# castorini/howl

Measured on AMD Instinct MI355X. Metric: utterances/sec/node (res8 end-to-end training step, 1s@16kHz, 40-mel), higher is better.
Workload: dtype f32; 1 GPU; res8 training step (frontend+fwd+xent+bwd+AdamW), 512 x 1 s utterances per GPU, 12 labels -- BASELINE configs[2] per-GPU share: res8 GSC-12, 512 x 1 s per GPU (4096 over 8); global_batch=512, samples_per_utterance=16000, labels=12, parallelism=single, frontend=eval

## Files before the change

### howl_amd/csrc/howl_common.hip.h

```cpp
#pragma once
#include <hip/hip_runtime.h>
#include <math.h>
#include <stdint.h>
#include <stdio.h>

typedef float f32x4 __attribute__((ext_vector_type(4)));
typedef __attribute__((address_space(3))) float lds_f32;

#if defined(HIPEMU)
#define HOWL_OPAQUE_V(x) ((void)(x))
#else
#define HOWL_OPAQUE_V(x) asm volatile("" : "+v"(x))
#endif
#define HOWL_OPAQUE_LDS(p) HOWL_OPAQUE_V(p)

#define HOWL_OK 0
#define HOWL_E_ARG (-1)
#define HOWL_E_LAUNCH (-2)
#define HOWL_E_WORKSPACE (-3)

void howl_set_error(const char* fmt, ...);
int howl_num_cus();
bool howl_prof_begin(const char* tag, hipStream_t stream, size_t* slot, double work);
void howl_prof_end(size_t slot, hipStream_t stream);

struct HowlSideLane {
    hipStream_t stream;
    hipEvent_t fork_ev, join_ev;
};
HowlSideLane* howl_side_lane();
bool howl_raise_lds(const void* kernel, size_t lds, size_t* granted, const char* what);
bool howl_take_pending_error();
inline void howl_lane_fork(HowlSideLane* l, hipStream_t main) {
    hipEventRecord(l->fork_ev, main);
    hipStreamWaitEvent(l->stream, l->fork_ev, 0);
}
inline void howl_lane_join(HowlSideLane* l, hipStream_t main) {
    hipEventRecord(l->join_ev, l->stream);
    hipStreamWaitEvent(main, l->join_ev, 0);
}

struct HowlProfScope {
    size_t slot = 0;
    bool on;
    hipStream_t stream;
    HowlProfScope(const char* tag, hipStream_t s, double work = 0.0) : stream(s) { on = howl_prof_begin(tag, s, &slot, work); }
    ~HowlProfScope() {
        if (on) howl_prof_end(slot, stream);
    }
};

struct HowlAdamWCoef {
    float lr, b1, b2, eps, wd, bc1, bc2_sqrt, gscale;
};
inline HowlAdamWCoef howl_adamw_coef(float lr, float beta1, float beta2, float eps, float weight_decay, int step, float grad_scale) {
    const double bc1 = 1.0 - pow((double)beta1, (double)step);
    const double bc2 = 1.0 - pow((double)beta2, (double)step);
    return HowlAdamWCoef{lr, beta1, beta2, eps, weight_decay, (float)bc1, (float)sqrt(bc2), grad_scale};
}
__device__ __forceinline__ void howl_adamw_element(float* __restrict__ p, float* __restrict__ m, float* __restrict__ v, size_t i, float g,
                                                   const HowlAdamWCoef& c) {
#pragma clang fp contract(off)
    const float gi = g * c.gscale;
    float pi = p[i] * (1.0f - c.lr * c.wd);
    const float mi = m[i] + (gi - m[i]) * (1.0f - c.b1);
    const float vi = c.b2 * v[i] + (1.0f - c.b2) * gi * gi;
    const float denom = sqrtf(vi) / c.bc2_sqrt + c.eps;
    pi -= (c.lr / c.bc1) * (mi / denom);
    p[i] = pi;
    m[i] = mi;
    v[i] = vi;
}

#define HOWL_REQUIRE(cond, ...)                 \
    do {                                        \
        if (!(cond)) {                          \
            howl_set_error(__VA_ARGS__);        \
            return HOWL_E_ARG;                  \
        }                                       \
    } while (0)

#define HOWL_CHECK_LAUNCH(name)                                                     \
    do {                                                                            \
        hipError_t e_ = hipGetLastError();                                          \
        if (howl_take_pending_error()) return HOWL_E_LAUNCH;   \
        if (e_ != hipSuccess) {                                                     \
            howl_set_error("%s: launch failed: %s", name, hipGetErrorString(e_));   \
            return HOWL_E_LAUNCH;                                                   \
        }                                                                           \
    } while (0)

__device__ __forceinline__ void wave_lds_sync() {
    __builtin_amdgcn_fence(__ATOMIC_RELEASE, "wavefront");
    __builtin_amdgcn_wave_barrier();
    __builtin_amdgcn_fence(__ATOMIC_ACQUIRE, "wavefront");
}

__device__ __forceinline__ float wave_sum(float v) {
    for (int m = 32; m >= 1; m >>= 1) v += __shfl_xor(v, m);
    return v;
}
__device__ __forceinline__ float wave_sum_rows(float v) {
    v += __int_as_float(__builtin_amdgcn_update_dpp(0, __float_as_int(v), 0xB1, 0xf, 0xf, true));
    v += __int_as_float(__builtin_amdgcn_update_dpp(0, __float_as_int(v), 0x4E, 0xf, 0xf, true));
    v += __int_as_float(__builtin_amdgcn_update_dpp(0, __float_as_int(v), 0x141, 0xf, 0xf, true));
    v += __int_as_float(__builtin_amdgcn_update_dpp(0, __float_as_int(v), 0x140, 0xf, 0xf, true));
    v += __shfl_xor(v, 16);
    v += __shfl_xor(v, 32);
    return v;
}
__device__ __forceinline__ double wave_sum_d(double v) {
    for (int m = 32; m >= 1; m >>= 1) v += __shfl_xor(v, m);
    return v;
}
```

### howl_amd/csrc/res8.hip

```cpp
#include "howl_common.hip.h"
#include "../../include/howl_hip.h"

namespace {

struct HowlPtrs6 {
    float* p[6];
};
constexpr int MAX_WINDOWS = 64;
struct HowlWinRows {
    int lo[MAX_WINDOWS], hi[MAX_WINDOWS];
};
struct HowlBnBuffers {
    float* running_mean;
    float* running_var;
    long long* num_batches;
};
struct BnFold {
    const float* part;
    int nparts;
    double count;
    float* stats_out;
    HowlBnBuffers bn;
};

// ... 18 lines not shown
__host__ __device__ inline int tile_floats(int H, bool own_rows = false) { return CP * chan_stride(H, own_rows) + 32; }
constexpr int WPW = 13;
constexpr int WNCOL = 16 * 26;
constexpr int WTAPS = 9 * NMAP;
__host__ __device__ inline int wgrad_rounds(int H) { return (H + 3) / 4; }

constexpr int PACK_ELEMS = 3 * KSTEPS * 64;
__device__ __forceinline__ void pack_weights_one(const HowlPtrs6& w, float* __restrict__ wp_fwd, float* __restrict__ wp_bwd,
                                                 int layer, int mode, int idx) {
    const int lane = idx & 63;
    const int ks = (idx >> 6) % KSTEPS;
    const int nt = idx / (64 * KSTEPS);
    int kk, tap;
    if (ks < 9 * KFULL) {
        const int c0 = ks / 9;
        tap = ks - 9 * c0;
        kk = 4 * c0 + (lane >> 4);
    } else {
        tap = 4 * (ks - 9 * KFULL) + (lane >> 4);
        kk = 4 * KFULL;
    }
    const int n = 16 * nt + (lane & 15);
    float v = 0.0f;
    if (kk < NMAP && n < NMAP && tap < 9) {
        const float* wl = w.p[layer];
        v = (mode == 0) ? wl[(n * NMAP + kk) * 9 + tap] : wl[(kk * NMAP + n) * 9 + (8 - tap)];
    }
    float* dst = (mode == 0 ? wp_fwd : wp_bwd) + (size_t)layer * (3 * KSTEPS * 64);
    dst[idx] = v;
}

__device__ __forceinline__ void zero_lds(float* p, int n, int tid, int nthreads) {
    const int n4 = n >> 2;
    for (int i = tid; i < n4; i += nthreads) reinterpret_cast<float4*>(p)[i] = make_float4(0.0f, 0.0f, 0.0f, 0.0f);
    for (int i = 4 * n4 + tid; i < n; i += nthreads) p[i] = 0.0f;
}

__host__ __device__ inline int part_stride(int nparts) { return (nparts + 3) & ~3; }
__device__ __forceinline__ double fold_part_column(const float* __restrict__ part, int nps, int nparts, int column, int lane) {
    const int slice = lane & 7;
    const float* src = part + (size_t)column * nps;
    double acc = 0.0;
    for (int r0 = 4 * slice; r0 < nparts; r0 += 8 * 32) {
        float4 v[8];
#pragma unroll
        for (int j = 0; j < 8; ++j) {
            const int r = r0 + 32 * j;
            v[j] = *reinterpret_cast<const float4*>(src + (r < nps ? r : 0));
        }
#pragma unroll
        for (int j = 0; j < 8; ++j) {
            const int r = r0 + 32 * j;
            acc += (r + 0 < nparts) ? (double)v[j].x : 0.0;
            acc += (r + 1 < nparts) ? (double)v[j].y : 0.0;
            acc += (r + 2 < nparts) ? (double)v[j].z : 0.0;
            acc += (r + 3 < nparts) ? (double)v[j].w : 0.0;
        }
    }
    acc += __shfl_xor(acc, 1);
    acc += __shfl_xor(acc, 2);
    acc += __shfl_xor(acc, 4);
    return acc;
}

template <int NTW>
struct KCursor {
    const lds_f32* ap[NTW];
    const lds_f32* bp;
    float a[NTW], b;
};

template <int NTW>
__device__ __forceinline__ void k_prime(KCursor<NTW>& k) {
#pragma unroll
    for (int i = 0; i < NTW; ++i) k.a[i] = k.ap[i][0];
    k.b = k.bp[0];
}

template <int NTW, int TS>
__device__ __forceinline__ void k_begin(KCursor<NTW>& k, f32x4 (&acc)[NTW], const lds_f32* tile, const lds_f32* wl,
                                        int CS, int P, int t0, int lane) {
    constexpr int ts = TS;
#pragma unroll
    for (int i = 0; i < NTW; ++i) {
        int m = 16 * (t0 + ts * i) + (lane & 15);
        m = m < P ? m : P - 1;
        const int h = m / PW;
        k.ap[i] = tile + (lane >> 4) * CS + h * WP + (m - h * PW);
        HOWL_OPAQUE_LDS(k.ap[i]);
        acc[i] = {0.0f, 0.0f, 0.0f, 0.0f};
    }
    k.bp = wl + lane;
    HOWL_OPAQUE_LDS(k.bp);
}

template <int NTW>
__device__ __forceinline__ void k_run(KCursor<NTW>& k, f32x4 (&acc)[NTW], int CS, int groups) {
#pragma unroll 2
    for (int g = 0; g < groups; ++g) {
#pragma unroll
        for (int tap = 0; tap < 9; ++tap) {
            float na[NTW], nb;
            if (tap < 8) {
                const int off = ((tap + 1) / 3) * WP + ((tap + 1) % 3);
#pragma unroll
                for (int i = 0; i < NTW; ++i) na[i] = k.ap[i][off];
                nb = k.bp[(tap + 1) * 64];
            } else {
                k.bp += 9 * 64;
#pragma unroll
                for (int i = 0; i < NTW; ++i) k.ap[i] += 4 * CS;
#pragma unroll
                for (int i = 0; i < NTW; ++i) na[i] = k.ap[i][0];
                nb = k.bp[0];
            }
#pragma unroll
            for (int i = 0; i < NTW; ++i) acc[i] = __builtin_amdgcn_mfma_f32_16x16x4f32(k.a[i], k.b, acc[i], 0, 0, 0);
#pragma unroll
            for (int i = 0; i < NTW; ++i) k.a[i] = na[i];
            k.b = nb;
        }
    }
}

template <int NTW>
__device__ __forceinline__ void k_tail(KCursor<NTW>& k, f32x4 (&acc)[NTW], const int (&dl)[3]) {
#pragma unroll
    for (int s3 = 0; s3 < 3; ++s3) {
        const float b = k.bp[s3 * 64];
#pragma unroll
        for (int i = 0; i < NTW; ++i) acc[i] = __builtin_amdgcn_mfma_f32_16x16x4f32(k.ap[i][dl[s3]], b, acc[i], 0, 0, 0);
    }
}

constexpr int SPLIT_C = 24;
constexpr int KG_A = SPLIT_C / 4;
constexpr int KG_B = KFULL - KG_A;
constexpr int NS0 = 5, NS1 = 4;
static_assert(CONV_THREADS * NS0 >= SPLIT_C * MAX_H * PW / 2 && CONV_THREADS * NS1 >= (NMAP - SPLIT_C) * MAX_H * PW / 2, "slots");
static_assert(KG_A == 6 && KG_B == 5, "the segment schedule of conv_loop is written for 6 + 5 K groups");

#define HOWL_STAIR(p_) __builtin_amdgcn_s_setprio(p_)

struct StageCfg {
    const float* a;
    const float* s;
    const float* k;
    float* ds;
    const float* dpool;
    float invP;
    bool fused;
    bool even;
    bool affine;
};

struct SlotVal {
    float2 a, s, k;
};

template <int NSL>
__device__ __forceinline__ void region_slots(int (&pk)[NSL], int c0, int nch, int P, int CS, int tid) {
    const float invP = 1.0f / (float)P;
#pragma unroll
    for (int j = 0; j < NSL; ++j) {
        const int e = 2 * (tid + j * CONV_THREADS);
        const int c = (int)(((float)e + 0.5f) * invP);
        const int p = e - c * P;
        const int h = (int)(((float)p + 0.5f) * 0.1f);
        const int w = p - h * PW;
        pk[j] = (e < nch * P) ? (((c0 + c) * CS + (h + 1) * WP + (w + 1)) | ((c0 + c) << 20)) : -1;
    }
}
template <int NSL>
__device__ __forceinline__ void region_slots_pad(int (&pk)[NSL], int c0, int nch, int P, int CS, int tid, int hv, unsigned& padbits) {
    region_slots<NSL>(pk, c0, nch, P, CS, tid);
#pragma unroll
    for (int j = 0; j < NSL; ++j) {
        const int e = 2 * (tid + j * CONV_THREADS);
        const int p = e % P;
        if (pk[j] >= 0 && p / PW >= hv) padbits |= 1u << j;
    }
}

template <int MODE, int HALO = 0>
__device__ __forceinline__ void slot_load(SlotVal& v, const StageCfg& cfg, size_t base, int i2, int pkj, int b) {
    HOWL_OPAQUE_V(pkj);
    const unsigned off = pkj >= 0 ? 8u * (unsigned)i2 : 0u;
    if (MODE == 1 && cfg.fused) {
        if (cfg.a != nullptr) {
            v.a = *reinterpret_cast<const float2*>(reinterpret_cast<const char*>(cfg.a + base) + off);
        } else {
            const unsigned c4 = pkj >= 0 ? 4u * (unsigned)(pkj >> 20) : 0u;
            const float g = *reinterpret_cast<const float*>(reinterpret_cast<const char*>(cfg.dpool + (size_t)(HALO == 1 ? b >> 1 : b) * CP) + c4) * cfg.invP;
            v.a = make_float2(g, g);
        }
        v.s = *reinterpret_cast<const float2*>(reinterpret_cast<const char*>(cfg.s + base) + off);
        v.k = cfg.k != nullptr ? *reinterpret_cast<const float2*>(reinterpret_cast<const char*>(cfg.k + base) + off)
                               : make_float2(0.0f, 0.0f);
    } else {
        v.a = *reinterpret_cast<const float2*>(reinterpret_cast<const char*>(cfg.a + base) + off);
    }
}

__device__ __forceinline__ void bn_relu_bwd_pair(const SlotVal& v, const float* lmc, bool even, float2& ds, float2& dz) {
    const float A = lmc[0], Bc = lmc[CP], Cc = lmc[2 * CP];
    ds.x = fmaf(A, v.a.x, fmaf(Bc, fabsf(v.s.x), Cc)) + v.k.x;
    ds.y = fmaf(A, v.a.y, fmaf(Bc, fabsf(v.s.y), Cc)) + v.k.y;
    const float t0 = even ? -v.s.x : v.s.x, t1 = even ? -v.s.y : v.s.y;
    dz.x = t0 > 0.0f ? ds.x : 0.0f;
    dz.y = t1 > 0.0f ? ds.y : 0.0f;
}

template <int MODE>
__device__ __forceinline__ void slot_write(const SlotVal& v, const StageCfg& cfg, size_t base, int i2, int pkj, float* tile,
                                           const float* lm, bool zero = false ) {
    HOWL_OPAQUE_V(pkj);
    if (pkj < 0) return;
    const int c = pkj >> 20;
    float v0 = v.a.x, v1 = v.a.y;
    if (MODE == 0) {
        v0 = fabsf(v0);
        v1 = fabsf(v1);
        if (cfg.affine) {
            const float sh = lm[c], r = lm[CP + c];
            v0 = fmaf(v0, r, sh);
            v1 = fmaf(v1, r, sh);
        }
    } else if (cfg.fused) {
        float2 ds, dz;
        bn_relu_bwd_pair(v, lm + c, cfg.even, ds, dz);
        if (cfg.ds != nullptr)
            *reinterpret_cast<float2*>(reinterpret_cast<char*>(cfg.ds + base) + 8u * (unsigned)i2) = ds;
        v0 = dz.x;
        v1 = dz.y;
    }
    if (zero) v0 = v1 = 0.0f;
    float* d = tile + (pkj & 0xFFFFF);
    d[0] = v0;
    d[1] = v1;
}

struct HaloSlot {
    int pk;
    int g;
};
__device__ __forceinline__ HaloSlot halo_slot(int c0, int nch, int H, int P, int CS, int tid) {
    const int c = tid / H, h = tid - c * H;
    HaloSlot hs;
    hs.pk = (tid < nch * H) ? (((c0 + c) * CS + (h + 1) * WP) | ((c0 + c) << 20)) : -1;
    hs.g = (tid < nch * H) ? (c0 + c) * P + h * PW : 0;
    return hs;
}
template <int MODE>
__device__ __forceinline__ void halo_load(SlotVal& v, const StageCfg& cfg, size_t nbase, const HaloSlot& hs, int gcol, int b) {
    const unsigned off = hs.pk >= 0 ? 4u * (unsigned)(hs.g + gcol) : 0u;
    v.s = v.k = make_float2(0.0f, 0.0f);
    if (MODE == 1 && cfg.fused) {
        if (cfg.a != nullptr) {
            v.a.x = *reinterpret_cast<const float*>(reinterpret_cast<const char*>(cfg.a + nbase) + off);
        } else {
            const unsigned c4 = hs.pk >= 0 ? 4u * (unsigned)(hs.pk >> 20) : 0u;
            v.a.x = *reinterpret_cast<const float*>(reinterpret_cast<const char*>(cfg.dpool + (size_t)(b >> 1) * CP) + c4) * cfg.invP;
        }
        v.s.x = *reinterpret_cast<const float*>(reinterpret_cast<const char*>(cfg.s + nbase) + off);
        if (cfg.k != nullptr) v.k.x = *reinterpret_cast<const float*>(reinterpret_cast<const char*>(cfg.k + nbase) + off);
    } else {
        v.a.x = *reinterpret_cast<const float*>(reinterpret_cast<const char*>(cfg.a + nbase) + off);
    }
    v.a.y = v.a.x;
}
template <int MODE>
__device__ __forceinline__ void halo_write(const SlotVal& v, const StageCfg& cfg, const HaloSlot& hs, int lcol, float* tile,
                                           const float* lm) {
    if (hs.pk < 0) return;
    const int c = hs.pk >> 20;
    float v0 = v.a.x;
    if (MODE == 0) {
        v0 = fabsf(v0);
        if (cfg.affine) v0 = fmaf(v0, lm[CP + c], lm[c]);
    } else if (cfg.fused) {
        float2 ds, dz;
        bn_relu_bwd_pair(v, lm + c, cfg.even, ds, dz);
        v0 = dz.x;
    }
    tile[(hs.pk & 0xFFFFF) + lcol] = v0;
}

struct StripGeom {
    int nr, ns, hv_last;
};
struct StripPos {
    int r, c, hv, bu;
};
__device__ __forceinline__ StripPos strip_pos(const StripGeom& g, int v, int H) {
    StripPos p;
    const int q = v / g.ns;
    p.c = v - q * g.ns;
    p.bu = q / g.nr;
    p.r = q - p.bu * g.nr;
    p.hv = (p.r == g.nr - 1) ? g.hv_last : H;
    return p;
}
struct EdgeSlot {
    int pk;
    int g;
    int aux;
};
// ... 16 lines not shown
    if (MODE == 1 && cfg.fused) {
        v.a.x = cfg.a != nullptr ? cfg.a[idx] : cfg.dpool[(size_t)bu * CP + chan] * cfg.invP;
        v.s.x = cfg.s[idx];
        if (cfg.k != nullptr) v.k.x = cfg.k[idx];
    } else {
        v.a.x = cfg.a[idx];
    }
    v.a.y = v.a.x;
}
template <int MODE>
__device__ __forceinline__ void edge_write(const SlotVal& v, const StageCfg& cfg, int pk, int lds_extra, bool valid, float* tile,
                                           const float* lm) {
    if (pk < 0) return;
    const int c = pk >> 20;
    float v0 = v.a.x;
    if (MODE == 0) {
        v0 = fabsf(v0);
        if (cfg.affine) v0 = fmaf(v0, lm[CP + c], lm[c]);
    } else if (cfg.fused) {
        float2 ds, dz;
        bn_relu_bwd_pair(v, lm + c, cfg.even, ds, dz);
        v0 = dz.x;
    }
    tile[(pk & 0xFFFFF) + lds_extra] = valid ? v0 : 0.0f;
}
struct GridCtx {
    StripGeom sg;
    EdgeSlot col[2], row[2];
    unsigned pad[2];
};
template <int MODE>
__device__ __forceinline__ void grid_load(SlotVal (&e)[3], const StageCfg& cfg, const GridCtx& gx, int reg, int v, int H, int P) {
    const StripPos p = strip_pos(gx.sg, v, H);
    {
        const EdgeSlot& es = gx.col[reg];
        const bool valid = gx.sg.ns == 2 && es.pk >= 0 && es.aux < p.hv;
        edge_load<MODE>(e[0], cfg, v ^ 1, es.g + (p.c ? PW - 1 : 0), valid, es.pk >= 0 ? es.pk >> 20 : 0, p.bu, P);
    }
    const EdgeSlot& rs = gx.row[reg];
    const int cc = p.c + rs.aux;
    const bool colok = rs.pk >= 0 && cc >= 0 && cc < gx.sg.ns;
    const int chan = rs.pk >= 0 ? rs.pk >> 20 : 0;
    edge_load<MODE>(e[1], cfg, v - gx.sg.ns + rs.aux, rs.g + (H - 1) * PW, colok && p.r > 0, chan, p.bu, P);
    edge_load<MODE>(e[2], cfg, v + gx.sg.ns + rs.aux, rs.g, colok && p.r < gx.sg.nr - 1, chan, p.bu, P);
}
template <int MODE>
__device__ __forceinline__ void grid_write(const SlotVal (&e)[3], const StageCfg& cfg, const GridCtx& gx, int reg, int v, int H,
                                           float* tile, const float* lm) {
    const StripPos p = strip_pos(gx.sg, v, H);
    if (gx.sg.ns == 2) {
        const EdgeSlot& es = gx.col[reg];
        edge_write<MODE>(e[0], cfg, es.pk, p.c ? 0 : WP - 1, es.aux < p.hv, tile, lm);
    }
    const EdgeSlot& rs = gx.row[reg];
    const int cc = p.c + rs.aux;
    const bool colok = cc >= 0 && cc < gx.sg.ns;
    edge_write<MODE>(e[1], cfg, rs.pk, 0, colok && p.r > 0, tile, lm);
    edge_write<MODE>(e[2], cfg, rs.pk, (H + 1) * WP, colok && p.r < gx.sg.nr - 1, tile, lm);
}

struct ConvEpilogue {
    const float* res;
    float* out;
    const float* xs;
    float xshift, xrstd;
    int cout, P;
    bool cvalid;
    bool xadd;
    float* pool;
    int npg, pg;
};

template <int NTW, int TS>
struct EpiAddr {
    unsigned boff, bmax;
    static constexpr unsigned tstep = 64u * TS;
    __device__ __forceinline__ EpiAddr(const ConvEpilogue& e, int t0, int lane) {
        const unsigned crow = (unsigned)((e.cvalid ? e.cout : NMAP - 1) * e.P);
        boff = 4u * (crow + 16u * t0 + 4u * (lane >> 4));
        bmax = 4u * (crow + e.P - 2);
    }
    __device__ __forceinline__ unsigned off(int i, int hh) const {
        unsigned o = boff + tstep * i + 8u * hh;
        if (i == NTW - 1) o = o < bmax ? o : bmax;
        return o;
    }
};

template <int MODE, int NTW, int TS, int HALO = 0>
__device__ __forceinline__ void conv_epilogue(const f32x4 (&acc)[NTW], const float2 (&ev)[NTW > 0 ? NTW : 1][2], const ConvEpilogue& e,
                                              size_t ubase, int t0, int lane, float& st0, float& st1, int b,
                                              int pv = 0 ) {
    const EpiAddr<NTW, TS> ea(e, t0, lane);
    constexpr int ts = TS;
    char* obase = reinterpret_cast<char*>(e.out + ubase);
    float u0 = 0.0f, u1 = 0.0f;
#pragma unroll
    for (int i = 0; i < NTW; ++i) {
        const int mbase = 16 * (t0 + ts * i) + 4 * (lane >> 4);
#pragma unroll
        for (int hh = 0; hh < 2; ++hh) {
            const int m = mbase + 2 * hh;
            if (e.cvalid && (i < NTW - 1 || m < e.P)) {
                float v0 = acc[i][2 * hh], v1 = acc[i][2 * hh + 1];
                if (MODE == 0) {
                    v0 = fmaxf(v0, 0.0f);
                    v1 = fmaxf(v1, 0.0f);
                    if (e.res != nullptr) {
                        const float2 r = ev[i][hh];
                        const bool k0 = v0 > 0.0f, k1 = v1 > 0.0f;
                        v0 += fabsf(r.x);
                        v1 += fabsf(r.y);
                        if (HALO != 2 || m < pv) {
                            u0 += v0 + v1;
                            u1 += v0 * v0 + v1 * v1;
                        }
                        v0 = k0 ? -v0 : v0;
                        v1 = k1 ? -v1 : v1;
                    } else if (HALO != 2 || m < pv) {
                        u0 += v0 + v1;
                        u1 += v0 * v0 + v1 * v1;
                    }
                } else if (e.xs != nullptr) {
                    const float2 sv = ev[i][hh];
                    if (e.xadd) {
                        v0 += sv.x;
                        v1 += sv.y;
                    } else if (HALO != 2 || m < pv) {
                        u0 += v0 + v1;
                        u1 += v0 * fmaf(fabsf(sv.x), e.xrstd, e.xshift) + v1 * fmaf(fabsf(sv.y), e.xrstd, e.xshift);
                    }
                }
                *reinterpret_cast<float2*>(obase + (ea.boff + ea.tstep * i + 8u * hh)) = make_float2(v0, v1);
            }
        }
    }
    st0 += u0;
    st1 += u1;
    if (MODE == 0 && e.pool != nullptr) {
        float up = u0;
        up += __shfl_xor(up, 16);
        up += __shfl_xor(up, 32);
        if (lane < 16 && e.cvalid) e.pool[((size_t)b * e.npg + e.pg) * CP + e.cout] = up;
    }
}

struct ConvLoop {
    const lds_f32* ltile;
    const lds_f32* wnt;
    float* tile;
    const float* lm;
    int B, CS, t0, lane, tid;
    int nblk;
};


template <int MODE, int NTW, int TS, int HALO = 0>
__device__ __forceinline__ void conv_loop(const ConvLoop& c, const ConvEpilogue& epi, const StageCfg& cfg, const int (&pk0)[NS0],
                                          const int (&pk1)[NS1], int b, float& st0, float& st1,
                                          const HaloSlot (&hs)[2] = {HaloSlot{-1, 0}, HaloSlot{-1, 0}},
                                          const GridCtx& gx = GridCtx{}) {
    const int P = epi.P, tid = c.tid, lane = c.lane;
    const int wave = tid >> 6;
    const size_t r1 = (size_t)SPLIT_C * P;
    const float* eop = (MODE == 0) ? epi.res : epi.xs;
    constexpr int NTV = NTW > 0 ? NTW : 1;
    int dl[3];
#pragma unroll
    for (int s3 = 0; s3 < 3; ++s3) {
        const int tap = min(4 * s3 + (lane >> 4), 8);
        dl[s3] = (tap / 3) * WP + tap % 3 - (lane >> 4) * c.CS;
    }
    const int gcol = (b & 1) ? PW - 1 : 0, lcol = (b & 1) ? 0 : WP - 1;
    for (; b < c.B; b += c.nblk) {
        const size_t ubase = (size_t)b * NMAP * P;
        const int bn = b + c.nblk;
        const bool more = bn < c.B;
        const size_t nbase = (size_t)bn * NMAP * P;
        SlotVal v[3];
        SlotVal ge[3];
        int bsl = b, bnsl = bn, pv = P;
        bool zb = false, zn = false;
        if constexpr (HALO == 2) {
            const StripPos pb = strip_pos(gx.sg, b, P / PW), pn = strip_pos(gx.sg, more ? bn : b, P / PW);
            bsl = pb.bu, bnsl = pn.bu, pv = pb.hv * PW;
            zb = pb.hv < P / PW, zn = pn.hv < P / PW;
        }
        f32x4 acc[NTV];
        KCursor<NTV> k;
        if constexpr (NTW > 0) k_begin<NTW, TS>(k, acc, c.ltile, c.wnt, c.CS, P, c.t0, lane);
        if constexpr (NTW > 0) k_prime<NTW>(k);
        constexpr bool STAGE = true;
        const int a0 = 2, a1 = 2, a2 = KG_A - 4, b0 = 2, b1 = 2, b2 = KG_B - 4;
#define HOWL_WINO_CHUNK() ((void)0)
#define HOWL_WINO_BAR() ((void)0)
        if constexpr (STAGE) {
            slot_load<MODE, HALO>(v[0], cfg, ubase + r1, tid, pk1[0], bsl);
            slot_load<MODE, HALO>(v[1], cfg, ubase + r1, tid + CONV_THREADS, pk1[1], bsl);
            if constexpr (HALO == 1) halo_load<MODE>(v[2], cfg, (size_t)(b ^ 1) * NMAP * P, hs[1], gcol, b);
            if constexpr (HALO == 2) grid_load<MODE>(ge, cfg, gx, 1, b, P / PW, P);
        }
        HOWL_STAIR(3);
        HOWL_WINO_CHUNK();
        if constexpr (NTW > 0) k_run<NTW>(k, acc, c.CS, a0);
        HOWL_WINO_BAR();
        if constexpr (STAGE) {
            slot_write<MODE>(v[0], cfg, ubase + r1, tid, pk1[0], c.tile, c.lm, HALO == 2 && zb && ((gx.pad[1] >> 0) & 1));
            slot_write<MODE>(v[1], cfg, ubase + r1, tid + CONV_THREADS, pk1[1], c.tile, c.lm, HALO == 2 && zb && ((gx.pad[1] >> 1) & 1));
            if constexpr (HALO == 1) halo_write<MODE>(v[2], cfg, hs[1], lcol, c.tile, c.lm);
            if constexpr (HALO == 2) grid_write<MODE>(ge, cfg, gx, 1, b, P / PW, c.tile, c.lm);
            slot_load<MODE, HALO>(v[0], cfg, ubase + r1, tid + 2 * CONV_THREADS, pk1[2], bsl);
            slot_load<MODE, HALO>(v[1], cfg, ubase + r1, tid + 3 * CONV_THREADS, pk1[3], bsl);
        }
        HOWL_STAIR(2);
        HOWL_WINO_CHUNK();
        if constexpr (NTW > 0) k_run<NTW>(k, acc, c.CS, a1);
        HOWL_WINO_BAR();
        if constexpr (STAGE) {
            slot_write<MODE>(v[0], cfg, ubase + r1, tid + 2 * CONV_THREADS, pk1[2], c.tile, c.lm, HALO == 2 && zb && ((gx.pad[1] >> 2) & 1));
            slot_write<MODE>(v[1], cfg, ubase + r1, tid + 3 * CONV_THREADS, pk1[3], c.tile, c.lm, HALO == 2 && zb && ((gx.pad[1] >> 3) & 1));
        }
        HOWL_STAIR(1);
        HOWL_WINO_CHUNK();
        if constexpr (NTW > 0) k_run<NTW>(k, acc, c.CS, a2);
        HOWL_WINO_BAR();
        HOWL_STAIR(0);
        __syncthreads();
        if constexpr (NTW > 0) k_prime<NTW>(k);
        if (STAGE && more) {
            slot_load<MODE, HALO>(v[0], cfg, nbase, tid, pk0[0], bnsl);
            slot_load<MODE, HALO>(v[1], cfg, nbase, tid + CONV_THREADS, pk0[1], bnsl);
            slot_load<MODE, HALO>(v[2], cfg, nbase, tid + 2 * CONV_THREADS, pk0[2], bnsl);
            if constexpr (HALO == 2) grid_load<MODE>(ge, cfg, gx, 0, bn, P / PW, P);
        }
        HOWL_STAIR(3);
        HOWL_WINO_CHUNK();
        if constexpr (NTW > 0) k_run<NTW>(k, acc, c.CS, b0);
        HOWL_WINO_BAR();
        if (STAGE && more) {
            slot_write<MODE>(v[0], cfg, nbase, tid, pk0[0], c.tile, c.lm, HALO == 2 && zn && ((gx.pad[0] >> 0) & 1));
            slot_write<MODE>(v[1], cfg, nbase, tid + CONV_THREADS, pk0[1], c.tile, c.lm, HALO == 2 && zn && ((gx.pad[0] >> 1) & 1));
            slot_write<MODE>(v[2], cfg, nbase, tid + 2 * CONV_THREADS, pk0[2], c.tile, c.lm, HALO == 2 && zn && ((gx.pad[0] >> 2) & 1));
            if constexpr (HALO == 2) grid_write<MODE>(ge, cfg, gx, 0, bn, P / PW, c.tile, c.lm);
            slot_load<MODE, HALO>(v[0], cfg, nbase, tid + 3 * CONV_THREADS, pk0[3], bnsl);
            slot_load<MODE, HALO>(v[1], cfg, nbase, tid + 4 * CONV_THREADS, pk0[4], bnsl);
            if constexpr (HALO == 1) halo_load<MODE>(v[2], cfg, (size_t)(bn ^ 1) * NMAP * P, hs[0], gcol, bn);
        }
        HOWL_STAIR(2);
        HOWL_WINO_CHUNK();
        if constexpr (NTW > 0) k_run<NTW>(k, acc, c.CS, b1);
        HOWL_WINO_BAR();
        if (STAGE && more) {
            slot_write<MODE>(v[0], cfg, nbase, tid + 3 * CONV_THREADS, pk0[3], c.tile, c.lm, HALO == 2 && zn && ((gx.pad[0] >> 3) & 1));
            slot_write<MODE>(v[1], cfg, nbase, tid + 4 * CONV_THREADS, pk0[4], c.tile, c.lm, HALO == 2 && zn && ((gx.pad[0] >> 4) & 1));
            if constexpr (HALO == 1) halo_write<MODE>(v[2], cfg, hs[0], lcol, c.tile, c.lm);
        }
        float2 ev[NTV][2];
        if constexpr (NTW > 0) {
            if (eop != nullptr) {
                const EpiAddr<NTW, TS> ea(epi, c.t0, lane);
                const char* ebase = reinterpret_cast<const char*>(eop + ubase);
#pragma unroll
                for (int i = 0; i < NTW; ++i)
#pragma unroll
                    for (int hh = 0; hh < 2; ++hh) ev[i][hh] = *reinterpret_cast<const float2*>(ebase + ea.off(i, hh));
            }
            HOWL_STAIR(1);
            k_run<NTW>(k, acc, c.CS, b2);
            k_tail<NTW>(k, acc, dl);
            HOWL_STAIR(0);
        }
        if constexpr (NTW > 0) conv_epilogue<MODE, NTW, TS, HALO>(acc, ev, epi, ubase, c.t0, lane, st0, st1, b, pv);
        __syncthreads();
    }
}

struct BwdFold {
    const float* stats;
    const float* m12;
    const float* part;
    int nparts;
    double count;
};
__device__ __forceinline__ void bwd_consts_to_lds(float* lm, int ch, float mean, float rstd, float m1, float m2) {
    lm[ch] = rstd;
    lm[CP + ch] = -rstd * rstd * m2;
    lm[2 * CP + ch] = rstd * (mean * rstd * m2 - m1);
}
__device__ __forceinline__ void bwd_fold_to_lds(float* lm, const BwdFold& f, int tid, int nthreads) {
    const int lane = tid & 63, wave = tid >> 6;
    if (f.part == nullptr) {
        if (tid < CP) bwd_consts_to_lds(lm, tid, f.stats[tid], f.stats[CP + tid], f.m12[tid], f.m12[CP + tid]);
    } else {
        const int c8 = lane >> 3;
        for (int ch0 = 4 * wave; ch0 < CP; ch0 += 4 * (nthreads >> 6)) {
            const int ch = ch0 + (c8 & 3);
            const float mean = f.stats[ch], rstd = f.stats[CP + ch];
            const double acc = fold_part_column(f.part, part_stride(f.nparts), f.nparts, (c8 < 4 ? 0 : CP) + ch, lane);
            const double second = __shfl_xor(acc, 32);
            if (c8 < 4 && (lane & 7) == 0)
                bwd_consts_to_lds(lm, ch, mean, rstd, (float)(acc / f.count), (float)(second / f.count));
        }
    }
}

struct WFold {
    const float* part;
    int nparts;
    float* out;
};

template <int MODE, int SLICES, int HALO = 0>
__device__ __forceinline__ void conv3x3_body(
    StageCfg cfg,
    const float* __restrict__ in_stats,
    const float* __restrict__ wp,
    const float* __restrict__ res,
    float* __restrict__ out,
    const float* __restrict__ xs,
    const float* __restrict__ xs_stats,
    float* __restrict__ part,
    float* __restrict__ pool,
    int B, int H, int bid, int nblk,
    int slice,
    const BnFold& fold,
    const BwdFold& bfold,
    const WFold& wf = WFold{nullptr, 0, nullptr},
    const StripGeom& sg = StripGeom{1, 1, 0}) {
    HIP_DYNAMIC_SHARED(float, lds)
    const int P = H * PW;
    const int CS = chan_stride(H, HALO == 2);
    const int TF = tile_floats(H, HALO == 2);
    float* wl = lds;
    float* tile = lds + 3 * KSTEPS * 64;
    float* lm = tile + TF;
    float* red = lm + 4 * CP;

    const int tid = threadIdx.x;
    const int lane = tid & 63;
    const int wave = tid >> 6;
    const int nt = __builtin_amdgcn_readfirstlane(wave % 3);
    const int mg = __builtin_amdgcn_readfirstlane(wave / 3);
    const int ntiles = (P + 15) / 16;
    constexpr int slices = SLICES, ts = 4 * SLICES;
    const int t0 = mg + 4 * slice;
    const int ntw = t0 < ntiles ? (ntiles - t0 + ts - 1) / ts : 0;
    const bool folding = MODE == 0 && fold.part != nullptr;
    cfg.affine = MODE == 0 && (in_stats != nullptr || folding);
    if (slice != 0) cfg.ds = nullptr;

    int pk0[NS0], pk1[NS1];
    GridCtx gx{};
    HaloSlot hs[2] = {HaloSlot{-1, 0}, HaloSlot{-1, 0}};
    if constexpr (HALO == 2) {
        gx.sg = sg;
        gx.pad[0] = gx.pad[1] = 0u;
        region_slots_pad<NS0>(pk0, 0, SPLIT_C, P, CS, tid, sg.hv_last, gx.pad[0]);
        region_slots_pad<NS1>(pk1, SPLIT_C, NMAP - SPLIT_C, P, CS, tid, sg.hv_last, gx.pad[1]);
        gx.col[0] = col_edge_slot(0, SPLIT_C, H, P, CS, tid);
        gx.col[1] = col_edge_slot(SPLIT_C, NMAP - SPLIT_C, H, P, CS, tid);
        gx.row[0] = row_edge_slot(0, SPLIT_C, P, CS, tid);
        gx.row[1] = row_edge_slot(SPLIT_C, NMAP - SPLIT_C, P, CS, tid);
    } else {
        region_slots<NS0>(pk0, 0, SPLIT_C, P, CS, tid);
        region_slots<NS1>(pk1, SPLIT_C, NMAP - SPLIT_C, P, CS, tid);
    }
    if constexpr (HALO == 1) {
        hs[0] = halo_slot(0, SPLIT_C, H, P, CS, tid);
        hs[1] = halo_slot(SPLIT_C, NMAP - SPLIT_C, H, P, CS, tid);
    }

    int b = bid;
    SlotVal first[NS0];
    if (b < B) {
#pragma unroll
        for (int j = 0; j < NS0; ++j)
            slot_load<MODE, HALO>(first[j], cfg, (size_t)b * NMAP * P, tid + j * CONV_THREADS, pk0[j],
                                  HALO == 2 ? strip_pos(sg, b, H).bu : b);
    }
    SlotVal firsth;
    SlotVal firstg[3];
    if constexpr (HALO == 1) {
        if (b < B) halo_load<MODE>(firsth, cfg, (size_t)(b ^ 1) * NMAP * P, hs[0], (b & 1) ? PW - 1 : 0, b);
    }
    if constexpr (HALO == 2) {
        if (b < B) grid_load<MODE>(firstg, cfg, gx, 0, b, H, P);
    }
    {
        float4 wv[7];
#pragma unroll
        for (int j = 0; j < 7; ++j) {
            const int i = tid + j * CONV_THREADS;
            wv[j] = (i < 3 * KSTEPS * 16) ? reinterpret_cast<const float4*>(wp)[i] : make_float4(0.f, 0.f, 0.f, 0.f);
        }
        if (MODE == 0 && folding) {
            const int c8 = lane >> 3;
            const int ch = 4 * wave + (c8 & 3);
            const double acc = fold_part_column(fold.part, part_stride(fold.nparts), fold.nparts, (c8 < 4 ? 0 : CP) + ch, lane);
            const double sq = __shfl_xor(acc, 32);
            if (c8 < 4 && (lane & 7) == 0) {
                const double mean = acc / fold.count;
                double var = sq / fold.count - mean * mean;
                var = var < 0.0 ? 0.0 : var;
                const float fm = (ch < NMAP) ? (float)mean : 0.0f;
                const float fr = (ch < NMAP) ? (float)(1.0 / sqrt(var + (double)BN_EPS)) : 0.0f;
                lm[ch] = -fm * fr;
                lm[CP + ch] = fr;
                if (bid == 0 && slice == 0) {
                    fold.stats_out[ch] = fm;
                    fold.stats_out[CP + ch] = fr;
                    if (ch < NMAP && fold.bn.running_mean != nullptr) {
                        const double unbiased = fold.count > 1.0 ? var * fold.count / (fold.count - 1.0) : var;
                        fold.bn.running_mean[ch] = (1.0f - BN_MOMENTUM) * fold.bn.running_mean[ch] + BN_MOMENTUM * (float)mean;
                        fold.bn.running_var[ch] = (1.0f - BN_MOMENTUM) * fold.bn.running_var[ch] + BN_MOMENTUM * (float)unbiased;
                    }
                    if (ch == 0 && fold.bn.num_batches != nullptr) fold.bn.num_batches[0] += 1;
                }
            }
        }
        if (MODE == 1 && cfg.fused) bwd_fold_to_lds(lm, bfold, tid, CONV_THREADS);
        zero_lds(tile, TF, tid, CONV_THREADS);
#pragma unroll
        for (int j = 0; j < 7; ++j) {
            const int i = tid + j * CONV_THREADS;
            if (i < 3 * KSTEPS * 16) reinterpret_cast<float4*>(wl)[i] = wv[j];
        }
    }
    if (MODE == 0 && !folding && tid < CP) {
        lm[tid] = cfg.affine ? -in_stats[tid] * in_stats[CP + tid] : 0.0f;
        lm[CP + tid] = cfg.affine ? in_stats[CP + tid] : 1.0f;
    }
    const int cout = 16 * nt + (lane & 15);
    const bool cvalid = cout < NMAP;
    float xshift = 0.0f, xrstd = 1.0f;
    if (MODE == 1 && xs != nullptr && xs_stats != nullptr && cvalid) {
        xrstd = xs_stats[CP + cout];
        xshift = -xs_stats[cout] * xrstd;
    }
    float st0 = 0.0f, st1 = 0.0f;
    const ConvEpilogue epi{res, out, xs, xshift, xrstd, cout, P, cvalid, MODE == 1 && xs != nullptr && xs_stats == nullptr,
                           pool, 4 * slices, t0};
    __syncthreads();
    if (b < B) {
#pragma unroll
        for (int j = 0; j < NS0; ++j)
            slot_write<MODE>(first[j], cfg, (size_t)b * NMAP * P, tid + j * CONV_THREADS, pk0[j], tile, lm,
                             HALO == 2 && strip_pos(sg, b, H).hv < H && ((gx.pad[0] >> j) & 1));
        if constexpr (HALO == 1) halo_write<MODE>(firsth, cfg, hs[0], (b & 1) ? 0 : WP - 1, tile, lm);
        if constexpr (HALO == 2) grid_write<MODE>(firstg, cfg, gx, 0, b, H, tile, lm);
    }
    __syncthreads();

    const ConvLoop cl{(const lds_f32*)tile, (const lds_f32*)wl + nt * KSTEPS * 64, tile, lm, B, CS, t0, lane, tid, nblk};
    switch (ntw) {
        case 5: conv_loop<MODE, 5, ts, HALO>(cl, epi, cfg, pk0, pk1, b, st0, st1, hs, gx); break;
        case 4: conv_loop<MODE, 4, ts, HALO>(cl, epi, cfg, pk0, pk1, b, st0, st1, hs, gx); break;
        case 3: conv_loop<MODE, 3, ts, HALO>(cl, epi, cfg, pk0, pk1, b, st0, st1, hs, gx); break;
        case 2: conv_loop<MODE, 2, ts, HALO>(cl, epi, cfg, pk0, pk1, b, st0, st1, hs, gx); break;
        case 1: conv_loop<MODE, 1, ts, HALO>(cl, epi, cfg, pk0, pk1, b, st0, st1, hs, gx); break;
        default: conv_loop<MODE, 0, ts, HALO>(cl, epi, cfg, pk0, pk1, b, st0, st1, hs, gx); break;
    }

    if (part != nullptr) {
        st0 += __shfl_xor(st0, 16);
        st0 += __shfl_xor(st0, 32);
        st1 += __shfl_xor(st1, 16);
        st1 += __shfl_xor(st1, 32);
        if (lane < 16) {
            red[(wave * 2 + 0) * 16 + lane] = st0;
            red[(wave * 2 + 1) * 16 + lane] = st1;
        }
        __syncthreads();
        if (tid < 2 * CP) {
            const int which = tid / CP, c = tid - which * CP;
            const int t3 = c >> 4, cl = c & 15;
            float s = 0.0f;
#pragma unroll
            for (int g = 0; g < 4; ++g) s += red[((g * 3 + t3) * 2 + which) * 16 + cl];
            part[((size_t)which * CP + c) * part_stride(nblk * slices) + bid * slices + slice] = s;
        }
    }
    if (MODE == 1 && wf.part != nullptr) {
        constexpr int NCOL2 = CP * WNCOL / 2;
        const int nwg = nblk * slices, wg = bid * slices + slice;
        const int per = (NCOL2 + nwg - 1) / nwg;
        const int q0 = wg * per, q1 = (q0 + per < NCOL2) ? q0 + per : NCOL2;
        const int pl = tid % 96, rg = tid / 96;
        float2* scratch = reinterpret_cast<float2*>(tile);
        for (int qb = q0; qb < q1; qb += 96) {
            const int q = qb + pl;
            float2 acc = make_float2(0.0f, 0.0f);
            if (q < q1) {
                const float2* src = reinterpret_cast<const float2*>(wf.part) + q;
                for (int g0 = rg; g0 < wf.nparts; g0 += 8 * 16) {
                    float2 v[16];
#pragma unroll
                    for (int u = 0; u < 16; ++u) {
                        const int g = g0 + 8 * u;
                        v[u] = src[(size_t)(g < wf.nparts ? g : wf.nparts - 1) * NCOL2];
                    }
#pragma unroll
                    for (int u = 0; u < 16; ++u)
                        if (g0 + 8 * u < wf.nparts) {
                            acc.x += v[u].x;
                            acc.y += v[u].y;
                        }
                }
            }
            scratch[rg * 96 + pl] = acc;
            __syncthreads();
            if (rg == 0 && q < q1) {
                float2 tot = scratch[pl];
#pragma unroll
                for (int r = 1; r < 8; ++r) {
                    tot.x += scratch[r * 96 + pl].x;
                    tot.y += scratch[r * 96 + pl].y;
                }
                const int col = 2 * q;
                const int co = col / WNCOL, i0 = col - co * WNCOL;
                if (co < NMAP && i0 < WTAPS) wf.out[(co * NMAP + i0 % NMAP) * 9 + i0 / NMAP] = tot.x;
                if (co < NMAP && i0 + 1 < WTAPS) wf.out[(co * NMAP + (i0 + 1) % NMAP) * 9 + (i0 + 1) / NMAP] = tot.y;
            }
            __syncthreads();
        }
    }
}

template <int MODE, int SLICES, int HALO = 0>
__global__ __launch_bounds__(CONV_THREADS) void conv3x3_mfma_kernel(StageCfg cfg, const float* __restrict__ in_stats,
                                                                    const float* __restrict__ wp,
                                                                    const float* __restrict__ res, float* __restrict__ out,
                                                                    const float* __restrict__ xs,
                                                                    const float* __restrict__ xs_stats,
                                                                    float* __restrict__ part, float* __restrict__ pool, int B,
                                                                    int H, int nblk, BnFold fold, BwdFold bfold, WFold wf,
                                                                    StripGeom sg) {
    const int x = blockIdx.x & 7, y = blockIdx.x >> 3;
    const int slice = y % SLICES, bid = (y / SLICES) * 8 + x;
    if (bid >= nblk) return;
    conv3x3_body<MODE, SLICES, HALO>(cfg, in_stats, wp, res, out, xs, xs_stats, part, pool, B, H, bid, nblk, slice, fold, bfold, wf, sg);
}


constexpr int WPZ = 11;
constexpr int WNT = 4, WNB = 5;
__host__ __device__ inline int wgrad_r1(int H) { return wgrad_rounds(H) / 2; }
__host__ __device__ inline int chan_stride_z(int H) {
    const int cs = 4 * wgrad_rounds(H) * WPZ;
    return cs + (2 - (cs % 32) + 32) % 32;
}
__host__ __device__ inline int chan_stride_x(int H) {
    const int cs = (4 * wgrad_rounds(H) + 4) * WPW;
    return cs + (2 - (cs % 32) + 32) % 32;
}
__host__ __device__ inline int tile_floats_z(int H) { return CP * chan_stride_z(H) + 32; }
__host__ __device__ inline int tile_floats_x(int H) { return CP * chan_stride_x(H) + 96; }

template <int NB>
struct WCursor {
    const lds_f32* ap[3];
    const lds_f32* bp[NB];
    const lds_f32* ape;
    const lds_f32* bpe;
};

template <int NB, bool EX>
__device__ __forceinline__ void wgrad_k_run(WCursor<NB>& c, f32x4 (&acc)[NB][3], f32x4& acce, float (&az)[3], float (&bx)[NB],
                                            float& aze, float& bxe, int rounds) {
#pragma nounroll
    for (int r = 0; r < rounds; ++r) {
#pragma unroll
        for (int w = 0; w < PW; ++w) {
            const int noz = (w + 1 < PW) ? (w + 1) : 4 * WPZ;
            const int nox = (w + 1 < PW) ? (w + 1) : 4 * WPW;
            float nz[3], nx[NB], nze = 0.0f, nxe = 0.0f;
#pragma unroll
            for (int mt = 0; mt < 3; ++mt) nz[mt] = c.ap[mt][noz];
#pragma unroll
            for (int i = 0; i < NB; ++i) nx[i] = c.bp[i][nox];
            if constexpr (EX) {
                nze = c.ape[noz];
                nxe = c.bpe[nox];
            }
#pragma unroll
            for (int i = 0; i < NB; ++i)
#pragma unroll
                for (int mt = 0; mt < 3; ++mt) {
                    acc[i][mt] = __builtin_amdgcn_mfma_f32_16x16x4f32(az[mt], bx[i], acc[i][mt], 0, 0, 0);
                }
            if constexpr (EX) acce = __builtin_amdgcn_mfma_f32_16x16x4f32(aze, bxe, acce, 0, 0, 0);
#pragma unroll
            for (int mt = 0; mt < 3; ++mt) az[mt] = nz[mt];
#pragma unroll
            for (int i = 0; i < NB; ++i) bx[i] = nx[i];
            if constexpr (EX) {
                aze = nze;
                bxe = nxe;
            }
        }
#pragma unroll
        for (int mt = 0; mt < 3; ++mt) c.ap[mt] += 4 * WPZ;
#pragma unroll
        for (int i = 0; i < NB; ++i) c.bp[i] += 4 * WPW;
        if constexpr (EX) {
            c.ape += 4 * WPZ;
            c.bpe += 4 * WPW;
// ... 26 lines not shown
    const int nper = PW * (h1 > h0 ? h1 - h0 : 0), nsafe = nper > 0 ? nper : 1;
#pragma unroll
    for (int j = 0; j < NSL; ++j) {
        const int e = 2 * (tid + j * CONV_THREADS);
        const int h = h0 + (e % nsafe) / PW;
        if (pk[j] >= 0 && h >= hv) padbits |= 1u << j;
    }
}

struct WStage {
    StageCfg z;
    const float* x;
    bool xaffine;
};

struct WSlot {
    SlotVal z;
    float2 x;
};

template <int HALO = 0>
__device__ __forceinline__ void wz_load(SlotVal& v, const StageCfg& cfg, size_t ubase, int pkj, int chj, int b) {
    HOWL_OPAQUE_V(pkj);
    HOWL_OPAQUE_V(chj);
    const unsigned g = pkj >= 0 ? (unsigned)(pkj >> 15) : 0u;
    const unsigned off = 4u * g;
    if (cfg.fused) {
        if (cfg.a != nullptr) {
            v.a = *reinterpret_cast<const float2*>(reinterpret_cast<const char*>(cfg.a + ubase) + off);
        } else {
            const unsigned c4 = 4u * (unsigned)(chj & 0xFF);
            const float gg = *reinterpret_cast<const float*>(reinterpret_cast<const char*>(cfg.dpool + (size_t)(HALO == 1 ? b >> 1 : b) * CP) + c4) * cfg.invP;
            v.a = make_float2(gg, gg);
        }
        v.s = *reinterpret_cast<const float2*>(reinterpret_cast<const char*>(cfg.s + ubase) + off);
        v.k = cfg.k != nullptr ? *reinterpret_cast<const float2*>(reinterpret_cast<const char*>(cfg.k + ubase) + off)
                               : make_float2(0.0f, 0.0f);
    } else {
        v.a = *reinterpret_cast<const float2*>(reinterpret_cast<const char*>(cfg.a + ubase) + off);
    }
}
__device__ __forceinline__ void wz_write(const SlotVal& v, const StageCfg& cfg, int pkj, int chj, float* tz, const float* lm,
                                         bool zero = false) {
    HOWL_OPAQUE_V(pkj);
    HOWL_OPAQUE_V(chj);
    if (pkj < 0) return;
    float v0 = v.a.x, v1 = v.a.y;
    if (cfg.fused) {
        const int c = chj & 0xFF;
        float2 ds, dz;
        bn_relu_bwd_pair(v, lm + c, cfg.even, ds, dz);
        v0 = dz.x;
        v1 = dz.y;
    }
    if (zero) v0 = v1 = 0.0f;
    float* d = tz + (pkj & 0x7FFF);
    d[0] = v0;
    d[1] = v1;
}
__device__ __forceinline__ void wx_load(float2& v, const float* x, size_t ubase, int pkj) {
    HOWL_OPAQUE_V(pkj);
    const unsigned off = pkj >= 0 ? 4u * (unsigned)(pkj >> 15) : 0u;
    v = *reinterpret_cast<const float2*>(reinterpret_cast<const char*>(x + ubase) + off);
}
__device__ __forceinline__ void wx_write(const float2& v, bool affine, int pkj, int chj, float* tx, const float* lm,
                                         bool zero = false) {
    HOWL_OPAQUE_V(pkj);
    HOWL_OPAQUE_V(chj);
    if (pkj < 0) return;
    float v0 = fabsf(v.x), v1 = fabsf(v.y);
    if (affine) {
        const int c = (chj >> 8) & 0xFF;
        const float sh = lm[4 * CP + c], r = lm[5 * CP + c];
        v0 = fmaf(v0, r, sh);
        v1 = fmaf(v1, r, sh);
    }
    if (zero) v0 = v1 = 0.0f;
    float* d = tx + (pkj & 0x7FFF);
    d[0] = v0;
    d[1] = v1;
}

struct WHalo {
    int pk;
    int g;
    int c;
    int h;
};
__device__ __forceinline__ WHalo whalo_slot(int h0, int h1, int P, int CSX, int row0, int tid) {
    const int nper = h1 > h0 ? h1 - h0 : 0, nsafe = nper > 0 ? nper : 1;
    const int c = tid / nsafe, hh = tid - c * nsafe, h = h0 + hh;
    const bool ok = tid < NMAP * nper;
    return WHalo{ok ? c * CSX + (h + row0) * WPW : -1, ok ? c * P + h * PW : 0, ok ? c : 0, ok ? h : 0};
}
__device__ __forceinline__ float whalo_load(const float* x, size_t nbase, const WHalo& wh, int gcol) {
    if (wh.pk < 0) return 0.0f;
    return *reinterpret_cast<const float*>(reinterpret_cast<const char*>(x + nbase) + 4u * (unsigned)(wh.g + gcol));
}
__device__ __forceinline__ void whalo_write(float v, bool affine, const WHalo& wh, int lcol, float* tx, const float* lm,
                                            int hv = 1 << 20) {
    if (wh.pk < 0) return;
    float v0 = fabsf(v);
    if (affine) v0 = fmaf(v0, lm[5 * CP + wh.c], lm[4 * CP + wh.c]);
    tx[wh.pk + lcol] = wh.h < hv ? v0 : 0.0f;
}

struct WRowSlot {
    int pk;
    int g;
    int c;
    int dc;
};
__device__ __forceinline__ WRowSlot wrow_slot(int P, int CSX, int tid) {
    const int c = tid / WP, w = tid - c * WP;
    const bool ok = tid < NMAP * WP;
    const int dc = w == 0 ? -1 : (w == WP - 1 ? 1 : 0);
    const int col = w == 0 ? PW - 1 : (w == WP - 1 ? 0 : w - 1);
    return WRowSlot{ok ? c * CSX + w : -1, ok ? c * P + col : 0, ok ? c : 0, ok ? dc : 0};
}
struct WGridCtx {
    StripGeom sg;
    WRowSlot row;
    unsigned pzt, pxt, pzb, pxb;
};
__device__ __forceinline__ float wrow_load(const float* x, const WGridCtx& gx, int v, int H, int P, bool below) {
    const StripPos p = strip_pos(gx.sg, v, H);
    const int cc = p.c + gx.row.dc;
    const bool valid = gx.row.pk >= 0 && cc >= 0 && cc < gx.sg.ns && (below ? p.r < gx.sg.nr - 1 : p.r > 0);
    const int blk = below ? v + gx.sg.ns + gx.row.dc : v - gx.sg.ns + gx.row.dc;
    const size_t idx = valid ? (size_t)blk * NMAP * P + (size_t)(gx.row.g + (below ? 0 : (H - 1) * PW)) : 0;
    return valid ? x[idx] : 0.0f;
}
__device__ __forceinline__ void wrow_write(float v, bool affine, const WGridCtx& gx, int vstrip, int H, bool below, float* tx,
                                           const float* lm) {
    if (gx.row.pk < 0) return;
    const StripPos p = strip_pos(gx.sg, vstrip, H);
    const int cc = p.c + gx.row.dc;
    const bool valid = cc >= 0 && cc < gx.sg.ns && (below ? p.r < gx.sg.nr - 1 : p.r > 0);
    float v0 = fabsf(v);
    if (affine) v0 = fmaf(v0, lm[5 * CP + gx.row.c], lm[4 * CP + gx.row.c]);
    tx[gx.row.pk + (below ? (H + 3) * WPW : 0)] = valid ? v0 : 0.0f;
}

struct WgradArgs {
    WStage st;
    float* part;
    float* tz;
    float* tx;
    const float* lm;
    int B, P, CSZ, CSX, R, R1, tid, lane, wave;
    int bid, nblk;
    int gw;
    int qe, mte;
};

__device__ __forceinline__ int wgrad_boff(int q, int n, int g, int CSX) {
    const int idx = 16 * q + n;
    const int tap = idx < WTAPS ? idx / NMAP : 0;
    const int cin = idx < WTAPS ? idx - tap * NMAP : NMAP;
    return cin * CSX + (g + tap / 3) * WPW + (tap % 3);
}

template <int NB, bool EX, int GWS, int HALO = 0>
__device__ __forceinline__ void wgrad_loop(const WgradArgs& a, const int (&zt)[WNT], const int (&xt)[WNT], const int (&ct)[WNT],
                                           const int (&zb)[WNB], const int (&xb)[WNB], const int (&cb)[WNB], int b,
                                           const WHalo (&wh)[2] = {WHalo{-1, 0, 0, 0}, WHalo{-1, 0, 0, 0}},
                                           const WGridCtx& gx = WGridCtx{}) {
    const int lane = a.lane, wave = a.wave;
    const int g = lane >> 4, n = lane & 15;
    f32x4 acc[NB][3];
#pragma unroll
    for (int i = 0; i < NB; ++i)
#pragma unroll
        for (int mt = 0; mt < 3; ++mt) acc[i][mt] = {0.0f, 0.0f, 0.0f, 0.0f};
    int boff[NB];
#pragma unroll
    for (int i = 0; i < NB; ++i) boff[i] = wgrad_boff(a.gw + GWS * i, n, g, a.CSX);
    const int boffe = EX ? wgrad_boff(a.qe, n, g, a.CSX) : 0;
    f32x4 acce = {0.0f, 0.0f, 0.0f, 0.0f};
    const int aoff = n * a.CSZ + g * WPZ;
    const int R1 = a.R1, R2 = a.R - a.R1;
    const int gcol = (b & 1) ? PW - 1 : 0, lcol = (b & 1) ? 0 : PW + 1;
    for (; b < a.B; b += a.nblk) {
        const size_t ubase = (size_t)b * NMAP * a.P;
        const int bn = b + a.nblk;
        const bool more = bn < a.B;
        const size_t nbase = (size_t)bn * NMAP * a.P;
        WCursor<NB> c;
#pragma unroll
        for (int mt = 0; mt < 3; ++mt) c.ap[mt] = (const lds_f32*)a.tz + aoff + 16 * mt * a.CSZ;
#pragma unroll
        for (int i = 0; i < NB; ++i) c.bp[i] = (const lds_f32*)a.tx + boff[i];
        c.ape = (const lds_f32*)a.tz + aoff + 16 * a.mte * a.CSZ;
        c.bpe = (const lds_f32*)a.tx + boffe;
        float az[3], bx[NB], aze = 0.0f, bxe = 0.0f;
        WSlot v[2];
        int bsl = b, bnsl = bn, hvb = 1 << 20, hvn = 1 << 20;
        bool zb_ = false, zn_ = false;
        if constexpr (HALO == 2) {
            const int Hs = a.P / PW;
            const StripPos pb = strip_pos(gx.sg, b, Hs), pn = strip_pos(gx.sg, more ? bn : b, Hs);
            bsl = pb.bu, bnsl = pn.bu, hvb = pb.hv, hvn = pn.hv;
            zb_ = pb.hv < Hs, zn_ = pn.hv < Hs;
        }
#pragma unroll
        for (int mt = 0; mt < 3; ++mt) az[mt] = c.ap[mt][0];
#pragma unroll
        for (int i = 0; i < NB; ++i) bx[i] = c.bp[i][0];
        if constexpr (EX) {
            aze = c.ape[0];
            bxe = c.bpe[0];
        }
        static_assert(WNB == 5 && WNT == 4, "the staging schedule below is written for 5 + 4 slot pairs");
#define HOWL_W_LOAD(slot_, j_, zpk_, xpk_, cpk_, ub_, bb_)                    \
    do {                                                                     \
        wz_load<HALO>(v[slot_].z, a.st.z, ub_, zpk_[j_], cpk_[j_], bb_);     \
        wx_load(v[slot_].x, a.st.x, ub_, xpk_[j_]);                          \
    } while (0)
#define HOWL_W_WRITE(slot_, j_, zpk_, xpk_, cpk_, zf_, zp_, xp_)                                                             \
    do {                                                                                                                   \
        wz_write(v[slot_].z, a.st.z, zpk_[j_], cpk_[j_], a.tz, a.lm, HALO == 2 && (zf_) && (((zp_) >> (j_)) & 1));         \
        wx_write(v[slot_].x, a.st.xaffine, xpk_[j_], cpk_[j_], a.tx, a.lm, HALO == 2 && (zf_) && (((xp_) >> (j_)) & 1));   \
    } while (0)
        HOWL_W_LOAD(0, 0, zb, xb, cb, ubase, bsl);
        HOWL_W_LOAD(1, 1, zb, xb, cb, ubase, bsl);
        float xh = 0.0f, xr = 0.0f;
        if constexpr (HALO != 0) xh = whalo_load(a.st.x, (size_t)(b ^ 1) * NMAP * a.P, wh[1], gcol);
        if constexpr (HALO == 2) xr = wrow_load(a.st.x, gx, b, a.P / PW, a.P, true);
        HOWL_STAIR(3);
        if (R1 > 0) wgrad_k_run<NB, EX>(c, acc, acce, az, bx, aze, bxe, 1);
        HOWL_W_WRITE(0, 0, zb, xb, cb, zb_, gx.pzb, gx.pxb);
        HOWL_W_WRITE(1, 1, zb, xb, cb, zb_, gx.pzb, gx.pxb);
        if constexpr (HALO != 0) whalo_write(xh, a.st.xaffine, wh[1], lcol, a.tx, a.lm, hvb);
        if constexpr (HALO == 2) wrow_write(xr, a.st.xaffine, gx, b, a.P / PW, true, a.tx, a.lm);
        HOWL_W_LOAD(0, 2, zb, xb, cb, ubase, bsl);
        HOWL_W_LOAD(1, 3, zb, xb, cb, ubase, bsl);
        HOWL_STAIR(2);
        if (R1 > 1) wgrad_k_run<NB, EX>(c, acc, acce, az, bx, aze, bxe, 1);
        HOWL_W_WRITE(0, 2, zb, xb, cb, zb_, gx.pzb, gx.pxb);
        HOWL_W_WRITE(1, 3, zb, xb, cb, zb_, gx.pzb, gx.pxb);
        HOWL_W_LOAD(0, 4, zb, xb, cb, ubase, bsl);
        HOWL_STAIR(1);
        if (R1 > 2) wgrad_k_run<NB, EX>(c, acc, acce, az, bx, aze, bxe, R1 - 2);
        HOWL_STAIR(0);
        HOWL_W_WRITE(0, 4, zb, xb, cb, zb_, gx.pzb, gx.pxb);
        __syncthreads();
#pragma unroll
        for (int i = 0; i < NB; ++i) c.bp[i] += 2 * WPW;
        c.bpe += 2 * WPW;
#pragma unroll
        for (int mt = 0; mt < 3; ++mt) az[mt] = c.ap[mt][0];
#pragma unroll
        for (int i = 0; i < NB; ++i) bx[i] = c.bp[i][0];
        if constexpr (EX) {
            aze = c.ape[0];
            bxe = c.bpe[0];
        }
        if (more) {
            HOWL_W_LOAD(0, 0, zt, xt, ct, nbase, bnsl);
            HOWL_W_LOAD(1, 1, zt, xt, ct, nbase, bnsl);
            if constexpr (HALO != 0) xh = whalo_load(a.st.x, (size_t)(bn ^ 1) * NMAP * a.P, wh[0], gcol);
            if constexpr (HALO == 2) xr = wrow_load(a.st.x, gx, bn, a.P / PW, a.P, false);
        }
        HOWL_STAIR(3);
        wgrad_k_run<NB, EX>(c, acc, acce, az, bx, aze, bxe, 1);
        if (more) {
            HOWL_W_WRITE(0, 0, zt, xt, ct, zn_, gx.pzt, gx.pxt);
            HOWL_W_WRITE(1, 1, zt, xt, ct, zn_, gx.pzt, gx.pxt);
            if constexpr (HALO != 0) whalo_write(xh, a.st.xaffine, wh[0], lcol, a.tx, a.lm, hvn);
            if constexpr (HALO == 2) wrow_write(xr, a.st.xaffine, gx, bn, a.P / PW, false, a.tx, a.lm);
            HOWL_W_LOAD(0, 2, zt, xt, ct, nbase, bnsl);
            HOWL_W_LOAD(1, 3, zt, xt, ct, nbase, bnsl);
        }
        HOWL_STAIR(2);
        if (R2 > 1) wgrad_k_run<NB, EX>(c, acc, acce, az, bx, aze, bxe, 1);
        if (more) {
            HOWL_W_WRITE(0, 2, zt, xt, ct, zn_, gx.pzt, gx.pxt);
            HOWL_W_WRITE(1, 3, zt, xt, ct, zn_, gx.pzt, gx.pxt);
        }
        HOWL_STAIR(1);
        if (R2 > 2) wgrad_k_run<NB, EX>(c, acc, acce, az, bx, aze, bxe, R2 - 2);
        HOWL_STAIR(0);
#undef HOWL_W_LOAD
#undef HOWL_W_WRITE
        __syncthreads();
    }
    float* dst = a.part + (size_t)a.bid * CP * WNCOL;
#pragma unroll
    for (int i = 0; i < NB; ++i) {
        const int q = a.gw + GWS * i;
#pragma unroll
        for (int mt = 0; mt < 3; ++mt)
#pragma unroll
            for (int r = 0; r < 4; ++r) dst[(16 * mt + 4 * g + r) * WNCOL + 16 * q + n] = acc[i][mt][r];
    }
    if constexpr (EX) {
#pragma unroll
        for (int r = 0; r < 4; ++r) dst[(16 * a.mte + 4 * g + r) * WNCOL + 16 * a.qe + n] = acce[r];
    }
}

template <int SLICES, int HALO = 0>
__device__ __forceinline__ void wgrad_body(
    WStage st, const float* __restrict__ in_stats , const BwdFold& bfold,
    float* __restrict__ part , int B, int H, int bid, int nblk, int slice,
    const StripGeom& sg = StripGeom{1, 1, 0} ) {
    HIP_DYNAMIC_SHARED(float, lds)
    const int P = H * PW;
    const int CSZ = chan_stride_z(H), CSX = chan_stride_x(H);
    float* tz = lds;
    float* tx = lds + tile_floats_z(H);
    float* lm = tx + tile_floats_x(H);

    const int tid = threadIdx.x;
    const int lane = tid & 63;
    const int wave = __builtin_amdgcn_readfirstlane(tid >> 6);
    const int R = wgrad_rounds(H), R1 = wgrad_r1(H);
    st.xaffine = in_stats != nullptr;
    st.z.ds = nullptr;

    const int zsplit = 4 * R1 < H ? 4 * R1 : H;
    const int xtop = R1 > 0 ? (4 * R1 + 1 < H ? 4 * R1 + 1 : H) : 0;
    const int xbot = 4 * R1 - 1 > 0 ? 4 * R1 - 1 : 0;
    int zt[WNT], xt[WNT], zb[WNB], xb[WNB], ct[WNT] = {}, cb[WNB] = {};
    WGridCtx gx{};
    if constexpr (HALO == 2) {
        gx.sg = sg;
        gx.row = wrow_slot(P, CSX, tid);
        row_region_slots_pad<WNT>(zt, ct, 0, 0, zsplit, P, CSZ, WPZ, 0, 0, tid, sg.hv_last, gx.pzt);
        row_region_slots_pad<WNT>(xt, ct, 1, 0, xtop, P, CSX, WPW, 1, 1, tid, sg.hv_last, gx.pxt);
        row_region_slots_pad<WNB>(zb, cb, 0, zsplit, H, P, CSZ, WPZ, 0, 0, tid, sg.hv_last, gx.pzb);
        row_region_slots_pad<WNB>(xb, cb, 1, xbot, H, P, CSX, WPW, 3, 1, tid, sg.hv_last, gx.pxb);
    } else {
        row_region_slots<WNT>(zt, ct, 0, 0, zsplit, P, CSZ, WPZ, 0, 0, tid);
        row_region_slots<WNT>(xt, ct, 1, 0, xtop, P, CSX, WPW, 1, 1, tid);
        row_region_slots<WNB>(zb, cb, 0, zsplit, H, P, CSZ, WPZ, 0, 0, tid);
        row_region_slots<WNB>(xb, cb, 1, xbot, H, P, CSX, WPW, 3, 1, tid);
    }
    WHalo wh[2] = {WHalo{-1, 0, 0, 0}, WHalo{-1, 0, 0, 0}};
    if (HALO == 1 || (HALO == 2 && sg.ns == 2)) {
        wh[0] = whalo_slot(0, xtop, P, CSX, 1, tid);
        wh[1] = whalo_slot(xbot, H, P, CSX, 3, tid);
    }
    const int b = bid;
    WSlot first[WNT];
    if (b < B) {
#pragma unroll
        for (int j = 0; j < WNT; ++j) {
            wz_load<HALO>(first[j].z, st.z, (size_t)b * NMAP * P, zt[j], ct[j], HALO == 2 ? strip_pos(sg, b, H).bu : b);
            wx_load(first[j].x, st.x, (size_t)b * NMAP * P, xt[j]);
        }
    }
    float firsth = 0.0f, firstr = 0.0f;
    if constexpr (HALO != 0) {
        if (b < B) firsth = whalo_load(st.x, (size_t)(b ^ 1) * NMAP * P, wh[0], (b & 1) ? PW - 1 : 0);
    }
    if constexpr (HALO == 2) {
        if (b < B) firstr = wrow_load(st.x, gx, b, H, P, false);
    }
    zero_lds(lds, tile_floats_z(H) + tile_floats_x(H), tid, CONV_THREADS);
    if (st.z.fused) {
        bwd_fold_to_lds(lm, bfold, tid, CONV_THREADS);
    }
    if (tid < CP) {
        lm[4 * CP + tid] = st.xaffine ? -in_stats[tid] * in_stats[CP + tid] : 0.0f;
        lm[5 * CP + tid] = st.xaffine ? in_stats[CP + tid] : 1.0f;
    }
    __syncthreads();
    if (b < B) {
#pragma unroll
        for (int j = 0; j < WNT; ++j) {
            const bool padded = HALO == 2 && strip_pos(sg, b, H).hv < H;
            wz_write(first[j].z, st.z, zt[j], ct[j], tz, lm, padded && ((gx.pzt >> j) & 1));
            wx_write(first[j].x, st.xaffine, xt[j], ct[j], tx, lm, padded && ((gx.pxt >> j) & 1));
        }
        if constexpr (HALO != 0) whalo_write(firsth, st.xaffine, wh[0], (b & 1) ? 0 : PW + 1, tx, lm, HALO == 2 ? strip_pos(sg, b, H).hv : 1 << 20);
        if constexpr (HALO == 2) wrow_write(firstr, st.xaffine, gx, b, H, false, tx, lm);
    }
    __syncthreads();
    constexpr int GWS = 12 * SLICES;
    const int gw = wave + 12 * slice;
    if constexpr (SLICES == 1) {
        int qe = 0, mte = 0;
        bool ex = true;
        switch (wave) {
            case 0: qe = 24, mte = 0; break;
            case 4: qe = 24, mte = 1; break;
            case 1: qe = 24, mte = 2; break;
            case 5: qe = 25, mte = 0; break;
            case 2: qe = 25, mte = 1; break;
            case 3: qe = 25, mte = 2; break;
            default: ex = false; break;
        }
        const WgradArgs a{st, part, tz, tx, lm, B, P, CSZ, CSX, R, R1, tid, lane, wave, bid, nblk, gw, qe, mte};
        if (ex)
            wgrad_loop<2, true, GWS, HALO>(a, zt, xt, ct, zb, xb, cb, b, wh, gx);
        else
            wgrad_loop<2, false, GWS, HALO>(a, zt, xt, ct, zb, xb, cb, b, wh, gx);
    } else {
        static_assert(SLICES == 2, "the weight gradient is sliced two ways");
        const bool ex = wave < 3;
        const WgradArgs a{st, part, tz, tx, lm, B, P, CSZ, CSX, R, R1, tid, lane, wave, bid, nblk, gw, 24 + slice, ex ? wave : 0};
        if (ex)
            wgrad_loop<1, true, GWS, HALO>(a, zt, xt, ct, zb, xb, cb, b, wh, gx);
        else
            wgrad_loop<1, false, GWS, HALO>(a, zt, xt, ct, zb, xb, cb, b, wh, gx);
    }
}

template <int SLICES, int HALO = 0>
__global__ __launch_bounds__(CONV_THREADS) void wgrad_mfma_kernel(WStage st, const float* __restrict__ in_stats, BwdFold bfold,
                                                                  float* __restrict__ part, int B, int H, int nblk, StripGeom sg) {
    const int x = blockIdx.x & 7, y = blockIdx.x >> 3;
    const int slice = y % SLICES, bid = (y / SLICES) * 8 + x;
    if (bid >= nblk) return;
    wgrad_body<SLICES, HALO>(st, in_stats, bfold, part, B, H, bid, nblk, slice, sg);
}

template <int SD, int SW, int HALO = 0>
__global__ __launch_bounds__(CONV_THREADS) void bwd_pair_kernel(
    StageCfg zc, BwdFold bfold, const float* __restrict__ wp, float* __restrict__ dx, const float* __restrict__ xs,
    const float* __restrict__ xs_stats, float* __restrict__ spart, const float* __restrict__ s_prev,
    const float* __restrict__ in_stats, float* __restrict__ wpart, int B, int H, int nblk, WFold wf, StripGeom sg) {
    const int x = blockIdx.x & 7, y = blockIdx.x >> 3;
    const int r = y % (SD + SW);
    const int j = (y / (SD + SW)) * 8 + x;
    if (j >= nblk) return;
    if (r < SD)
        conv3x3_body<1, SD, HALO>(zc, nullptr, wp, nullptr, dx, xs, xs_stats, spart, nullptr, B, H, j, nblk, r, BnFold{}, bfold, wf, sg);
    else
        wgrad_body<SW, HALO>(WStage{zc, s_prev, false}, in_stats, bfold, wpart, B, H, j, nblk, r - SD, sg);
}

struct RowsAdamW {
    float* p;
    const float* g0;
    float* m;
    float* v;
    HowlAdamWCoef c;
    long rest_lo, rest_hi;
    int on;
};
__device__ __forceinline__ void reduce_rows_body(const float* __restrict__ part, int nparts, int ncols, int mode,
                                                 float* __restrict__ out, const RowsAdamW& opt) {
    __shared__ float red[16][64];
    const int lane = threadIdx.x & 63, rg = threadIdx.x >> 6, nrg = blockDim.x >> 6;
    const int col = blockIdx.x * 64 + lane;
    float s = 0.0f;
    if (col < ncols) {
        const float* src = part + col;
        for (int g = rg; g < nparts; g += 8 * nrg) {
            float v[8];
#pragma unroll
            for (int u = 0; u < 8; ++u) {
                const int r = g + u * nrg;
                v[u] = src[(size_t)(r < nparts ? r : nparts - 1) * ncols];
            }
#pragma unroll
            for (int u = 0; u < 8; ++u) s += (g + u * nrg < nparts) ? v[u] : 0.0f;
        }
    }
    red[rg][lane] = s;
    __syncthreads();
    if (rg == 0 && col < ncols) {
        float tot = red[0][lane];
        for (int r = 1; r < nrg; ++r) tot += red[r][lane];
        long d = -1;
        if (mode == 0) {
            d = col;
        } else {
            const int co = col / WNCOL, idx = col - co * WNCOL;
            if (co < NMAP && idx < WTAPS) d = (co * NMAP + idx % NMAP) * 9 + idx / NMAP;
        }
        if (d >= 0) {
            out[d] = tot;
            if (opt.on) howl_adamw_element(opt.p, opt.m, opt.v, (size_t)((out - opt.g0) + d), tot, opt.c);
        }
    }
}

__global__ __launch_bounds__(1024) void reduce_rows_all_kernel(const float* __restrict__ part, size_t layer_stride, int nparts,
                                                              HowlPtrs6 out, const float* __restrict__ c0part, int c0parts,
                                                              float* __restrict__ c0out, int y0, int yskip, int nrows, RowsAdamW opt) {
    if ((int)blockIdx.y >= nrows) {
        for (long i = opt.rest_lo + (long)blockIdx.x * blockDim.x + threadIdx.x; i < opt.rest_hi; i += (long)gridDim.x * blockDim.x)
            howl_adamw_element(opt.p, opt.m, opt.v, (size_t)i, opt.g0[i], opt.c);
        return;
    }
    const int y = y0 + (int)blockIdx.y * (1 + yskip);
    if (y < 6) {
        reduce_rows_body(part + y * layer_stride, nparts, CP * WNCOL, 1, out.p[y], opt);
    } else if (blockIdx.x * 64 < NMAP * 9) {
        reduce_rows_body(c0part, c0parts, NMAP * 9, 0, c0out, opt);
    }
}

__global__ void bn_eval_stats_kernel(HowlPtrs6 rmean, HowlPtrs6 rvar, float* __restrict__ stats) {
    const int layer = blockIdx.x, c = threadIdx.x;
    if (c >= CP) return;
    float* st = stats + (size_t)layer * 2 * CP;
    st[c] = (c < NMAP) ? rmean.p[layer][c] : 0.0f;
    st[CP + c] = (c < NMAP) ? 1.0f / sqrtf(rvar.p[layer][c] + BN_EPS) : 0.0f;
}

constexpr int BRB_THREADS = 1024;
__global__ __launch_bounds__(BRB_THREADS) void bn_relu_bwd_kernel(
    const float* __restrict__ dx,
    const float* __restrict__ dpool,
    const float* __restrict__ s, const float* __restrict__ stats, const float* __restrict__ m12,
    const float* __restrict__ part, int nparts, double count,
    const float* __restrict__ dskip,
    int even,
    float* __restrict__ ds_out,
    float* __restrict__ dz_out, int B, int P) {
    __shared__ float lm[4 * CP];
    const int tid = threadIdx.x, lane = tid & 63, wave = tid >> 6;
    if (tid < CP) {
        lm[tid] = stats[tid];
        lm[CP + tid] = stats[CP + tid];
        if (part == nullptr) {
            lm[2 * CP + tid] = m12[tid];
            lm[3 * CP + tid] = m12[CP + tid];
        }
    }
    if (part != nullptr) {
        const int c8 = lane >> 3;
        const int ch = 3 * wave + (c8 & 3);
        const bool used = (c8 & 3) < 3;
        const double acc = fold_part_column(part, part_stride(nparts), nparts, (c8 < 4 ? 0 : CP) + (used ? ch : 0), lane);
        const double second = __shfl_xor(acc, 32);
        if (c8 < 3 && (lane & 7) == 0) {
            lm[2 * CP + ch] = (float)(acc / count);
            lm[3 * CP + ch] = (float)(second / count);
        }
    }
    __syncthreads();
    const unsigned n2 = (unsigned)((size_t)B * NMAP * P / 2);
    const float invP = 1.0f / (float)P;
    const unsigned stride = gridDim.x * BRB_THREADS;
    auto finish = [&](float2 g, float2 sv, float2 kk, unsigned c, float2& ds, float2& dz) {
        const float mean = lm[c], rstd = lm[CP + c], m1 = lm[2 * CP + c], m2 = lm[3 * CP + c];
        ds.x = rstd * (g.x - m1 - ((fabsf(sv.x) - mean) * rstd) * m2) + kk.x;
        ds.y = rstd * (g.y - m1 - ((fabsf(sv.y) - mean) * rstd) * m2) + kk.y;
        const bool k0 = even ? (sv.x < 0.0f) : (sv.x > 0.0f), k1 = even ? (sv.y < 0.0f) : (sv.y > 0.0f);
        dz = make_float2(k0 ? ds.x : 0.0f, k1 ? ds.y : 0.0f);
    };
    const unsigned n4 = n2 / 2;
    for (unsigned i0 = blockIdx.x * BRB_THREADS + tid; i0 < n4; i0 += 2 * stride) {
        unsigned idx[2];
        bool ok[2];
        float4 g[2], sv[2], kk[2];
        unsigned cc[2][2];
#pragma unroll
        for (int u = 0; u < 2; ++u) {
            const unsigned i = i0 + u * stride;
            ok[u] = i < n4;
            idx[u] = ok[u] ? i : i0;
            float gb[2] = {0.0f, 0.0f};
#pragma unroll
            for (int h = 0; h < 2; ++h) {
                const unsigned bc = (4u * idx[u] + 2u * h) / (unsigned)P;
                const unsigned bb = bc / NMAP;
                cc[u][h] = bc - bb * NMAP;
                if (dx == nullptr) gb[h] = dpool[bb * CP + cc[u][h]] * invP;
            }
            g[u] = dx != nullptr ? reinterpret_cast<const float4*>(dx)[idx[u]] : make_float4(gb[0], gb[0], gb[1], gb[1]);
            sv[u] = reinterpret_cast<const float4*>(s)[idx[u]];
            kk[u] = dskip != nullptr ? reinterpret_cast<const float4*>(dskip)[idx[u]] : make_float4(0.0f, 0.0f, 0.0f, 0.0f);
        }
#pragma unroll
        for (int u = 0; u < 2; ++u) {
            float2 dsa, dza, dsb, dzb;
            finish(make_float2(g[u].x, g[u].y), make_float2(sv[u].x, sv[u].y), make_float2(kk[u].x, kk[u].y), cc[u][0], dsa, dza);
            finish(make_float2(g[u].z, g[u].w), make_float2(sv[u].z, sv[u].w), make_float2(kk[u].z, kk[u].w), cc[u][1], dsb, dzb);
            if (ok[u]) {
                if (ds_out != nullptr) reinterpret_cast<float4*>(ds_out)[idx[u]] = make_float4(dsa.x, dsa.y, dsb.x, dsb.y);
                reinterpret_cast<float4*>(dz_out)[idx[u]] = make_float4(dza.x, dza.y, dzb.x, dzb.y);
            }
        }
    }
    if ((n2 & 1u) && blockIdx.x == 0 && tid == 0) {
        const unsigned i = n2 - 1;
        const unsigned bc = (2u * i) / (unsigned)P;
        const unsigned bb = bc / NMAP, c = bc - bb * NMAP;
        float2 g;
        if (dx != nullptr) {
            g = reinterpret_cast<const float2*>(dx)[i];
        } else {
            const float v = dpool[bb * CP + c] * invP;
            g = make_float2(v, v);
        }
        const float2 sv = reinterpret_cast<const float2*>(s)[i];
        const float2 kk = dskip != nullptr ? reinterpret_cast<const float2*>(dskip)[i] : make_float2(0.0f, 0.0f);
        float2 ds, dz;
        finish(g, sv, kk, c, ds, dz);
        if (ds_out != nullptr) reinterpret_cast<float2*>(ds_out)[i] = ds;
        reinterpret_cast<float2*>(dz_out)[i] = dz;
    }
}


template <bool EXACT = false>
__device__ __forceinline__ void load_feat_tile(float* tin, const float* feat, long sb, long st, long sm, int b, int T,
                                               int M, int tid, int nthreads, int t_lo = 0, int t_hi = 0) {
    const int pitch = M + 4;
    const int n = (T + 2) * pitch;
    for (int i0 = tid; i0 < n; i0 += 8 * nthreads) {
        float v[8];
#pragma unroll
        for (int j = 0; j < 8; ++j) {
            const int i = i0 + j * nthreads;
            const int t = i / pitch - 1, m = i % pitch - 1;
            const bool ok = i < n && (EXACT ? t >= t_lo && t < t_hi : t >= 0 && t < T) && m >= 0 && m < M;
            v[j] = feat[b * sb + (ok ? t * st + m * sm : 0)];
        }
#pragma unroll
        for (int j = 0; j < 8; ++j) {
            const int i = i0 + j * nthreads;
            const int t = i / pitch - 1, m = i % pitch - 1;
            const bool ok = (EXACT ? t >= t_lo && t < t_hi : t >= 0 && t < T) && m >= 0 && m < M;
            if (i < n) tin[i] = ok ? v[j] : 0.0f;
        }
    }
}

constexpr int C0M_THREADS = 512;

template <int NS = 1, bool EXACT = false>
__global__ __launch_bounds__(C0M_THREADS) void conv0_fwd_mfma_kernel(const float* __restrict__ feat, long sb, long st,
                                                                    long sm, const float* __restrict__ w0,
                                                                    float* __restrict__ s0, unsigned short* __restrict__ mask0,
                                                                    int B, int T, int M, int H, int nconv, HowlPtrs6 cw,
                                                                    float* __restrict__ wp_fwd, float* __restrict__ wp_bwd,
                                                                    int nwin, int win_step, int win_last, int slices) {
    if ((int)blockIdx.x >= nconv) {
        const int e = ((int)blockIdx.x - nconv) * C0M_THREADS + (int)threadIdx.x;
        if (e < 2 * 6 * PACK_ELEMS) pack_weights_one(cw, wp_fwd, wp_bwd, (e / PACK_ELEMS) % 6, e / (6 * PACK_ELEMS), e % PACK_ELEMS);
        return;
    }
    HIP_DYNAMIC_SHARED(float, lds)
    float* tin = lds;
    const int tid = threadIdx.x, lane = tid & 63, wave = tid >> 6;
    const int pitch = M + 4;
    const int P = H * PW;
    const int g = lane >> 4, n = lane & 15;
    float bw[3][3];
#pragma unroll
    for (int ks = 0; ks < 3; ++ks)
#pragma unroll
        for (int nt = 0; nt < 3; ++nt) {
            const int tap = 4 * ks + g, c = 16 * nt + n;
            bw[ks][nt] = (tap < 9 && c < NMAP) ? w0[c * 9 + tap] : 0.0f;
        }
    int aoff[3];
#pragma unroll
    for (int ks = 0; ks < 3; ++ks) {
        const int tap = min(4 * ks + g, 8);
        aoff[ks] = (tap / 3) * pitch + tap % 3 + (n & 7) + (n >> 3) * 3 * pitch;
    }
    for (int i = tid; i < 3 * pitch + 16; i += C0M_THREADS) tin[(T + 2) * pitch + i] = 0.0f;
    for (int item = blockIdx.x; item < B * slices; item += nconv) {
        const int b = item / slices, sl = item - b * slices;
        const int ph0 = (sl * H) / slices, ph1 = ((sl + 1) * H) / slices;
        __syncthreads();
        const int clip = b / nwin, wi = b - clip * nwin;
        const int t0 = EXACT ? wi * win_step : min(wi * win_step, win_last);
        load_feat_tile<EXACT>(tin, feat + (long)clip * sb + (long)t0 * st, 0, st, sm, 0, T, M, tid, C0M_THREADS, -t0, win_last - t0);
        __syncthreads();
        constexpr int NJ = 5 * NS;
        for (int u = wave; u < NJ * ((ph1 - ph0 + 1) / 2); u += C0M_THREADS / 64) {
            const int pp = u / NJ, j8 = u - NJ * pp;
            const float* rowp = tin + 3 * (ph0 + 2 * pp) * pitch + 8 * j8;
            {
                f32x4 acc[3][3];
#pragma unroll
                for (int tl = 0; tl < 3; ++tl)
#pragma unroll
                    for (int nt = 0; nt < 3; ++nt) acc[tl][nt] = {0.0f, 0.0f, 0.0f, 0.0f};
#pragma unroll
                for (int tl = 0; tl < 3; ++tl)
#pragma unroll
                    for (int ks = 0; ks < 3; ++ks) {
                        const float a = rowp[aoff[ks] + tl * pitch];
#pragma unroll
                        for (int nt = 0; nt < 3; ++nt)
                            acc[tl][nt] = __builtin_amdgcn_mfma_f32_16x16x4f32(a, bw[ks][nt], acc[tl][nt], 0, 0, 0);
                    }
                const int pw = 2 * j8 + (g & 1), ph = ph0 + 2 * pp + (g >> 1);
#pragma unroll
                for (int nt = 0; nt < 3; ++nt) {
                    float sum = 0.0f;
                    unsigned bits = 0;
#pragma unroll
                    for (int tl = 0; tl < 3; ++tl)
#pragma unroll
                        for (int r = 0; r < 4; ++r) {
                            const int rb = max(__float_as_int(acc[tl][nt][r]), 0);
                            sum += __int_as_float(rb);
                            bits |= min((unsigned)rb, 1u) << (4 * tl + r);
                        }
                    const int c = 16 * nt + n;
                    if (ph < ph1 && c < NMAP) {
                        const int strip = NS > 1 ? pw / PW : 0;
                        const size_t o = (((size_t)b * NS + strip) * NMAP + c) * P + (size_t)ph * PW + (pw - strip * PW);
                        s0[o] = sum * (1.0f / 12.0f);
                        if (mask0 != nullptr) mask0[o] = (unsigned short)bits;
                    }
                }
            }
        }
    }
}

constexpr int C0G_WAVES = 15, C0G_THREADS = 64 * C0G_WAVES, C0G_CPW = NMAP / C0G_WAVES;
static_assert(C0G_CPW * C0G_WAVES == NMAP, "channels split evenly over the waves");

__device__ __forceinline__ void load_patch(float (&x)[5][6], const float* tin, int pitch, int ph, int pw) {
    const float* base = tin + 3 * ph * pitch + 4 * pw;
#pragma unroll
    for (int r = 0; r < 5; ++r) {
        const float4 a = *reinterpret_cast<const float4*>(base + r * pitch);
        const float2 c = *reinterpret_cast<const float2*>(base + r * pitch + 4);
        x[r][0] = a.x, x[r][1] = a.y, x[r][2] = a.z, x[r][3] = a.w, x[r][4] = c.x, x[r][5] = c.y;
    }
}

template <int NS = 1, bool EXACT = false>
__global__ __launch_bounds__(C0G_THREADS) void conv0_wgrad_valu_kernel(const float* __restrict__ feat, long sb, long st, long sm,
                                                                      const unsigned short* __restrict__ mask0,
                                                                      const float* __restrict__ ga, const float* __restrict__ gb,
                                                                      float* __restrict__ part, int B, int T, int M, int H,
                                                                      int slices, StripGeom sg, int t_total) {
    HIP_DYNAMIC_SHARED(float, lds)
    float* tin = lds;
    const int tid = threadIdx.x, lane = tid & 63;
    const int wave = __builtin_amdgcn_readfirstlane(tid >> 6);
    const int pitch = M + 4;
    const int P = H * PW;
    float acc[C0G_CPW][9];
#pragma unroll
    for (int j = 0; j < C0G_CPW; ++j)
#pragma unroll
        for (int t = 0; t < 9; ++t) acc[j][t] = 0.0f;
    const int nrs = EXACT ? sg.nr : 1;
    for (int item = blockIdx.x; item < B * nrs * NS * slices; item += gridDim.x) {
        const int vb = item / slices, sl = item - vb * slices;
        const int vq = NS > 1 ? vb / NS : vb, strip = NS > 1 ? vb - vq * NS : 0;
        const int b = EXACT ? vq / nrs : vq, rs = EXACT ? vq - b * nrs : 0;
        const int Pv = (EXACT && rs == nrs - 1) ? sg.hv_last * PW : P;
        const int cell0 = (sl * Pv) / slices, cell1 = ((sl + 1) * Pv) / slices;
        __syncthreads();
        if constexpr (EXACT)
            load_feat_tile<true>(tin, feat + (long)rs * T * st, sb, st, sm, b, T, M, tid, C0G_THREADS, -rs * T, t_total - rs * T);
        else
            load_feat_tile(tin, feat, sb, st, sm, b, T, M, tid, C0G_THREADS);
        __syncthreads();
        const float* gab = ga + ((size_t)vb * NMAP + C0G_CPW * wave) * P;
        const float* gbb = gb != nullptr ? gb + ((size_t)vb * NMAP + C0G_CPW * wave) * P : nullptr;
        const unsigned short* mb = mask0 + ((size_t)vb * NMAP + C0G_CPW * wave) * P;
        for (int cb = cell0; cb < cell1; cb += 64) {
            const int cell = cb + lane;
            const bool valid = cell < cell1;
            const unsigned cc = (unsigned)(valid ? cell : cell1 - 1);
            float gv[C0G_CPW];
            unsigned mv[C0G_CPW];
#pragma unroll
            for (int j = 0; j < C0G_CPW; ++j) {
                const unsigned o = (unsigned)(j * P) + cc;
                gv[j] = gab[o] + (gbb != nullptr ? gbb[o] : 0.0f);
                mv[j] = mb[o];
            }
            const int ph = (int)cc / PW, pw = (int)cc - ph * PW;
            float x[5][6];
            load_patch(x, tin, pitch, ph, pw + strip * PW);
#pragma unroll
            for (int j = 0; j < C0G_CPW; ++j) {
                const int gbits = valid ? __float_as_int(gv[j] * (1.0f / 12.0f)) : 0;
#pragma unroll
                for (int tl = 0; tl < 3; ++tl)
#pragma unroll
                    for (int fl = 0; fl < 4; ++fl) {
                        const int k = 4 * tl + fl;
                        const int sel = ((int)(mv[j] << (31 - k))) >> 31;
                        const float dy = __int_as_float(sel & gbits);
#pragma unroll
                        for (int tap = 0; tap < 9; ++tap) acc[j][tap] = fmaf(dy, x[tl + tap / 3][fl + tap % 3], acc[j][tap]);
                    }
            }
// ... 172 lines not shown
    }
}

__global__ void head_bwd_pool_kernel(const float* __restrict__ dlogits, const float* __restrict__ wout,
                                     float* __restrict__ dpool, int B, int C) {
    const int idx = blockIdx.x * blockDim.x + threadIdx.x;
    if (idx >= B * CP) return;
    const int b = idx / CP, c = idx - b * CP;
    float acc = 0.0f;
    if (c < NMAP)
        for (int k = 0; k < C; ++k) acc = fmaf(dlogits[(size_t)b * C + k], wout[k * NMAP + c], acc);
    dpool[idx] = acc;
}

__global__ __launch_bounds__(1024) void head_bwd_param_kernel(const float* __restrict__ dlogits,
                                                              const float* __restrict__ pooled,
                                                              const float* __restrict__ dpool, float* __restrict__ dwout,
                                                              float* __restrict__ dbout, float* __restrict__ m12, int B,
                                                              int C, int P, const float* __restrict__ nll,
                                                              float* __restrict__ loss) {
    __shared__ double red[2][16][64];
    if ((int)blockIdx.x == C + 1) {
        double acc = 0.0;
        for (int b = threadIdx.x; b < B; b += 1024) acc += (double)nll[b];
        acc = wave_sum_d(acc);
        if ((threadIdx.x & 63) == 0) red[0][threadIdx.x >> 6][0] = acc;
        __syncthreads();
        if (threadIdx.x == 0) {
            double tot = 0.0;
            for (int w = 0; w < 16; ++w) tot += red[0][w][0];
            loss[0] = (float)(tot / (double)B);
        }
        return;
    }
    const int k = blockIdx.x, c = threadIdx.x & 63, bg = threadIdx.x >> 6;
    double a0 = 0.0, a1 = 0.0;
    constexpr int HR = 16;
    const int cc = c < CP ? c : CP - 1;
    if (k < C) {
        for (int b = bg; b < B; b += 16 * HR) {
            float d[HR], pv[HR];
#pragma unroll
            for (int j = 0; j < HR; ++j) {
                const int bb = b + 16 * j < B ? b + 16 * j : B - 1;
                d[j] = dlogits[(size_t)bb * C + k];
                pv[j] = pooled[(size_t)bb * CP + cc];
            }
#pragma unroll
            for (int j = 0; j < HR; ++j) {
                const bool ok = b + 16 * j < B;
                a1 += ok ? (double)d[j] : 0.0;
                a0 += (ok && c < CP) ? (double)d[j] * (double)pv[j] : 0.0;
            }
        }
    } else if (c < CP) {
        for (int b = bg; b < B; b += 16 * HR) {
            float d[HR], pv[HR];
#pragma unroll
            for (int j = 0; j < HR; ++j) {
                const int bb = b + 16 * j < B ? b + 16 * j : B - 1;
                d[j] = dpool[(size_t)bb * CP + c];
                pv[j] = pooled[(size_t)bb * CP + c];
            }
#pragma unroll
            for (int j = 0; j < HR; ++j) {
                const bool ok = b + 16 * j < B;
                a0 += ok ? (double)d[j] : 0.0;
                a1 += ok ? (double)d[j] * (double)pv[j] : 0.0;
            }
        }
    }
    red[0][bg][c] = a0;
    red[1][bg][c] = a1;
    __syncthreads();
    if (bg != 0) return;
    double s0 = 0.0, s1 = 0.0;
    for (int g = 0; g < 16; ++g) {
        s0 += red[0][g][c];
        s1 += red[1][g][c];
    }
    if (k < C) {
        if (c < NMAP) dwout[k * NMAP + c] = (float)s0;
        if (c == 0) dbout[k] = (float)s1;
    } else if (c < CP) {
        const double n = (double)B * (double)P;
        m12[c] = (float)(s0 / n);
        m12[CP + c] = (float)(s1 / n);
    }
}

__global__ __launch_bounds__(1024) void xent_kernel(const float* __restrict__ logits, const long long* __restrict__ labels,
                                                    int B, int C, float* __restrict__ loss, float* __restrict__ dlogits) {
    __shared__ double red[16];
    double acc = 0.0;
    const float invB = 1.0f / (float)B;
    constexpr int XC = 32;
    for (int b = threadIdx.x; b < B; b += 1024) {
        const float* row = logits + (size_t)b * C;
        const int y = (int)labels[b];
        if (C <= XC) {
            float v[XC];
#pragma unroll
            for (int k = 0; k < XC; ++k) v[k] = row[k < C ? k : C - 1];
            float mx = v[0];
#pragma unroll
            for (int k = 1; k < XC; ++k) mx = k < C ? fmaxf(mx, v[k]) : mx;
            float se = 0.0f;
#pragma unroll
            for (int k = 0; k < XC; ++k) se += k < C ? expf(v[k] - mx) : 0.0f;
            const float lse = mx + logf(se);
            float vy = v[0];
#pragma unroll
            for (int k = 1; k < XC; ++k) vy = k == y ? v[k] : vy;
            acc += (double)(lse - vy);
            if (dlogits != nullptr) {
#pragma unroll
                for (int k = 0; k < XC; ++k)
                    if (k < C) dlogits[(size_t)b * C + k] = (expf(v[k] - lse) - (k == y ? 1.0f : 0.0f)) * invB;
            }
            continue;
        }
        float mx = row[0];
        for (int k = 1; k < C; ++k) mx = fmaxf(mx, row[k]);
        float se = 0.0f;
        for (int k = 0; k < C; ++k) se += expf(row[k] - mx);
        const float lse = mx + logf(se);
        acc += (double)(lse - row[y]);
        if (dlogits != nullptr)
            for (int k = 0; k < C; ++k)
                dlogits[(size_t)b * C + k] = (expf(row[k] - lse) - (k == y ? 1.0f : 0.0f)) * invB;
    }
    acc = wave_sum_d(acc);
    if ((threadIdx.x & 63) == 0) red[threadIdx.x >> 6] = acc;
    __syncthreads();
    if (threadIdx.x == 0) {
        double tot = 0.0;
        for (int w = 0; w < 16; ++w) tot += red[w];
        loss[0] = (float)(tot / (double)B);
    }
}

__global__ void adamw_kernel(float* __restrict__ p, const float* __restrict__ g, float* __restrict__ m,
                             float* __restrict__ v, size_t n, HowlAdamWCoef c) {
    for (size_t i = (size_t)blockIdx.x * blockDim.x + threadIdx.x; i < n; i += (size_t)gridDim.x * blockDim.x)
        howl_adamw_element(p, m, v, i, g[i], c);
}

}

namespace {

size_t conv0_tile_floats(int T, int M) { return (size_t)(T + 2) * (M + 4) + 3 * (M + 4) + 16; }
size_t conv_lds_bytes(int H, bool own_rows) {
    return (size_t)(3 * KSTEPS * 64 + tile_floats(H, own_rows) + 4 * CP + 12 * 2 * 16) * sizeof(float);
}
size_t wgrad_lds_bytes(int H) { return (size_t)(tile_floats_z(H) + tile_floats_x(H) + 6 * CP) * sizeof(float); }

struct Ws {
    float* wp_fwd;
    float* wp_bwd;
    float* part;
    float* part2;
    float* stats;
    float* m12;
    float* dpool;
    float* pool;
    float* bufa;
    float* bufb;
    float* dz;
    float* dz2;
    float* dsa;
    float* dsb;
    float* wpart;
    float* c0part;
};

size_t ws_layout(Ws* w, char* base, int B, int H, int G, int cus, size_t* fwd_eval_bytes) {
    size_t off = 0;
    auto take = [&](size_t floats) {
        float* p = base ? reinterpret_cast<float*>(base + off) : nullptr;
        off += ((floats * sizeof(float) + 255) / 256) * 256;
        return p;
    };
    const size_t act = (size_t)B * NMAP * H * PW;
    w->wp_fwd = take((size_t)6 * 3 * KSTEPS * 64);
    w->wp_bwd = take((size_t)6 * 3 * KSTEPS * 64);
    const int max_parts = G > cus ? G : cus;
    w->part = take((size_t)part_stride(max_parts) * 2 * CP);
    w->part2 = take((size_t)part_stride(max_parts) * 2 * CP);
    w->stats = take((size_t)6 * 2 * CP);
    w->m12 = take(2 * CP);
    w->dpool = take((size_t)B * CP);
    w->pool = take((size_t)B * 16 * CP);
    *fwd_eval_bytes = off;
    w->bufa = take(act);
    w->bufb = take(act);
    w->dz = take(act);
    w->dz2 = take(act);
    w->dsa = take(act);
    w->dsb = take(act);
    w->wpart = take((size_t)6 * G * CP * WNCOL);
    w->c0part = take((size_t)max_parts * NMAP * 9);
    return off;
}

int mel_strips(int M) { return M == 40 ? 1 : (M == 80 ? 2 : 0); }
int even_grid(int g, int strips) { return strips > 1 ? ((g & ~1) > 2 ? (g & ~1) : 2) : g; }
int launch_blocks(int nblk, int per_group) { return 8 * per_group * ((nblk + 7) / 8); }
int conv_slices(int nblk, int H, int budget) {
    const int ntiles = (H * PW + 15) / 16;
    for (int sl = 4; sl > 1; sl >>= 1)
        if (nblk * sl <= budget && 4 * sl <= ntiles) return sl;
    return 1;
}
void pair_slices(int nblk, int H, int cus, int* sd, int* sw) {
    const int ntiles = (H * PW + 15) / 16;
    const int opts[3][2] = {{4, 2}, {2, 2}, {2, 1}};
    *sd = *sw = 1;
    for (const auto& o : opts)
        if (nblk * (o[0] + o[1]) <= cus && 4 * o[0] <= ntiles) {
            *sd = o[0];
            *sw = o[1];
            return;
        }
}
int conv0_slices(int B, int cus) {
    const int sl = cus / (B > 0 ? B : 1);
    return sl < 1 ? 1 : (sl > 8 ? 8 : sl);
}
bool env_off(const char* name) {
    const char* e = getenv(name);
    return e != nullptr && e[0] == '0';
}

constexpr int WIN_H = MAX_H, WIN_MARGIN = 7, WIN_STEP = WIN_H - 2 * WIN_MARGIN;
int long_windows(int H) { return H <= WIN_H ? 1 : (H - WIN_H + WIN_STEP - 1) / WIN_STEP + 1; }

struct Res8Plan {
    int B, T, M, ns, nr, Hs, hv_last, Bv, halo;
    StripGeom sg;
    int P, Pt;
    bool slicing, merged, fused;
    int G, SL;
    size_t lds_conv;
    int Bw, Tw, S0, G0, c0_nwin, c0_step, c0_last;
    bool c0_exact;
    size_t lds_conv0;
    int Gh, SD, SW, ew_grid;
    bool fold_in_pair;
    size_t wpart_stride, lds_wgrad, lds_pair;
    int S0w, G0w;
    size_t lds_conv0w;
    size_t saved_floats, train_bytes, eval_bytes;
    size_t long_map_bytes, long_bytes;
    Ws ws;
};

void plan_launches(Res8Plan& p, bool slice_conv0, char* ws_base) {
    const int cus = howl_num_cus(), H = p.Hs;
    p.P = H * PW;
    p.Pt = (p.T / 3) * PW * p.ns;
    p.saved_floats = (size_t)p.Bv * NMAP * p.P;
    p.slicing = !env_off("HOWL_RES8_SLICES");
    p.merged = !env_off("HOWL_RES8_BWD_PAIR");
    p.fused = p.halo != 0 || !env_off("HOWL_RES8_BWD_FUSED");

    p.G = even_grid(p.Bv < cus ? p.Bv : cus, p.ns);
    p.SL = p.halo == 0 && p.slicing ? conv_slices(p.G, H, cus) : 1;
    p.lds_conv = conv_lds_bytes(H, p.halo == 2);
    p.S0 = slice_conv0 && p.slicing ? conv0_slices(p.Bw, cus) : 1;
    p.G0 = p.Bw * p.S0 < 2 * cus ? p.Bw * p.S0 : 2 * cus;
    p.lds_conv0 = conv0_tile_floats(p.Tw, p.M) * sizeof(float);

    const int half = cus / 2 > 0 ? cus / 2 : 1;
    p.Gh = even_grid(p.Bv < half ? p.Bv : half, p.ns);
    p.SD = p.SW = 1;
    if (p.halo == 0 && p.slicing) pair_slices(p.Gh, H, cus, &p.SD, &p.SW);
    p.fold_in_pair = p.Gh * p.SD >= 64;
    p.wpart_stride = (size_t)p.Gh * CP * WNCOL;
    p.lds_wgrad = wgrad_lds_bytes(H);
    p.lds_pair = p.lds_conv > p.lds_wgrad ? p.lds_conv : p.lds_wgrad;
    const size_t quads = (p.saved_floats / 4 + BRB_THREADS - 1) / BRB_THREADS;
    p.ew_grid = quads < 1 ? 1 : (quads > (size_t)(2 * cus) ? 2 * cus : (int)quads);
    p.S0w = p.slicing ? conv0_slices(p.Bv, cus) : 1;
    p.G0w = p.Bv * p.S0w < cus ? p.Bv * p.S0w : cus;
    p.lds_conv0w = ((size_t)(p.Tw + 2) * (p.M + 4) + 16) * sizeof(float);

    p.train_bytes = ws_layout(&p.ws, ws_base, p.Bv, H, p.G, cus, &p.eval_bytes);
}

Res8Plan res8_plan(int B, int T, int M, void* ws = nullptr) {
    Res8Plan p{};
    const int H = T / 3;
    p.B = B, p.T = T, p.M = M;
    p.ns = mel_strips(M) > 0 ? mel_strips(M) : 1;
    p.nr = H <= MAX_H ? 1 : (H + MAX_H - 1) / MAX_H;
    p.Hs = (H + p.nr - 1) / p.nr;
    p.hv_last = H - (p.nr - 1) * p.Hs;
    p.Bv = B * p.nr * p.ns;
    p.halo = p.nr > 1 ? 2 : (p.ns > 1 ? 1 : 0);
    p.sg = StripGeom{p.nr, p.ns, p.hv_last};
    p.c0_exact = p.halo == 2;
    p.Bw = B * p.nr;
    p.Tw = p.c0_exact ? 3 * p.Hs : T;
    p.c0_nwin = p.c0_exact ? p.nr : 1;
    p.c0_step = p.c0_exact ? 3 * p.Hs : 0;
    p.c0_last = p.c0_exact ? T : 0;
    plan_launches(p, true, static_cast<char*>(ws));
    return p;
}

Res8Plan res8_long_plan(int B, int T, int M, void* ws = nullptr) {
    Res8Plan p{};
    const int H = T / 3, nw = long_windows(H);
    p.B = B, p.T = T, p.M = M;
    p.ns = mel_strips(M) > 0 ? mel_strips(M) : 1;
    p.nr = 1, p.Hs = p.hv_last = WIN_H;
    p.Bv = B * nw * p.ns;
    p.halo = p.ns > 1 ? 1 : 0;
    p.sg = StripGeom{1, 1, 0};
    p.Bw = B * nw;
    p.Tw = 3 * WIN_H + T % 3;
    p.c0_nwin = nw, p.c0_step = 3 * WIN_STEP, p.c0_last = 3 * (H - WIN_H);
    static_assert((6 * 2 * CP * sizeof(float)) % 256 == 0, "statistics block keeps the 256-byte alignment");
    p.long_map_bytes = ((size_t)p.Bv * NMAP * WIN_H * PW * sizeof(float) + 255) / 256 * 256;
    const size_t front = 3 * p.long_map_bytes + 6 * 2 * CP * sizeof(float) + 256;
    plan_launches(p, false, ws ? static_cast<char*>(ws) + front : nullptr);
    p.long_bytes = front + p.train_bytes;
    return p;
}

int check_workspace(const char* who, size_t have, size_t need) {
    if (have >= need) return HOWL_OK;
    howl_set_error("%s: workspace %zu < %zu bytes", who, have, need);
    return HOWL_E_WORKSPACE;
}
template <class T>
HowlPtrs6 ptrs6(T* const (&a)[6]) {
    HowlPtrs6 r;
    for (int i = 0; i < 6; ++i) r.p[i] = const_cast<float*>(a[i]);
    return r;
}
StageCfg plain_tile(const float* t) { return StageCfg{t, nullptr, nullptr, nullptr, nullptr, 0.0f, false, false, false}; }

template <auto Kernel>
void raise_lds_limit(size_t lds) {
    static thread_local size_t granted[16] = {};
    howl_raise_lds(reinterpret_cast<const void*>(Kernel), lds, granted, "res8 kernel");
}
template <int HALO>
StripGeom geom_arg(const Res8Plan& p) { return HALO == 2 ? p.sg : StripGeom{1, 1, 0}; }

struct Conv3x3Launch {
    StageCfg in;
    const float* in_stats = nullptr;
    const float* wp = nullptr;
    const float* res = nullptr;
    float* out = nullptr;
    const float* xs = nullptr;
    const float* xs_stats = nullptr;
    float* part = nullptr;
    float* pool = nullptr;
    BnFold fold{};
    BwdFold bfold{};
    WFold wf{nullptr, 0, nullptr};
};
template <int MODE, int SLICES, int HALO>
void launch_conv3x3_inst(const Res8Plan& p, hipStream_t stream, const Conv3x3Launch& a) {
    const int nblk = MODE == 0 ? p.G : p.Gh;
    raise_lds_limit<conv3x3_mfma_kernel<MODE, SLICES, HALO>>(p.lds_conv);
    hipLaunchKernelGGL((conv3x3_mfma_kernel<MODE, SLICES, HALO>), dim3(launch_blocks(nblk, SLICES)), dim3(CONV_THREADS), p.lds_conv,
                       stream, a.in, a.in_stats, a.wp, a.res, a.out, a.xs, a.xs_stats, a.part, a.pool, p.Bv, p.Hs, nblk, a.fold,
                       a.bfold, a.wf, geom_arg<HALO>(p));
}
template <int MODE>
void launch_conv3x3(const Res8Plan& p, hipStream_t stream, const Conv3x3Launch& a) {
    const int slices = MODE == 0 ? p.SL : p.SD;
    if (p.halo == 2)
        launch_conv3x3_inst<MODE, 1, 2>(p, stream, a);
    else if (p.halo == 1)
        launch_conv3x3_inst<MODE, 1, 1>(p, stream, a);
    else if (slices == 4)
        launch_conv3x3_inst<MODE, 4, 0>(p, stream, a);
    else if (slices == 2)
        launch_conv3x3_inst<MODE, 2, 0>(p, stream, a);
    else
        launch_conv3x3_inst<MODE, 1, 0>(p, stream, a);
}

struct BwdLayerLaunch {
    StageCfg zc;
    BwdFold bfold;
    const float* wp;
    float* dx;
    const float* xs;
    const float* xs_stats;
    float* spart;
    const float* s_prev;
    const float* in_stats;
    float* wpart;
    WFold wf;
};
template <int SD, int SW, int HALO>
void launch_pair_inst(const Res8Plan& p, hipStream_t stream, const BwdLayerLaunch& a) {
    raise_lds_limit<bwd_pair_kernel<SD, SW, HALO>>(p.lds_pair);
    hipLaunchKernelGGL((bwd_pair_kernel<SD, SW, HALO>), dim3(launch_blocks(p.Gh, SD + SW)), dim3(CONV_THREADS), p.lds_pair, stream, a.zc,
                       a.bfold, a.wp, a.dx, a.xs, a.xs_stats, a.spart, a.s_prev, a.in_stats, a.wpart, p.Bv, p.Hs, p.Gh, a.wf,
                       geom_arg<HALO>(p));
}
void launch_pair(const Res8Plan& p, hipStream_t stream, const BwdLayerLaunch& a) {
    if (p.halo == 2)
        launch_pair_inst<1, 1, 2>(p, stream, a);
    else if (p.halo == 1)
        launch_pair_inst<1, 1, 1>(p, stream, a);
    else if (p.SD == 4 && p.SW == 2)
        launch_pair_inst<4, 2, 0>(p, stream, a);
    else if (p.SD == 2 && p.SW == 2)
        launch_pair_inst<2, 2, 0>(p, stream, a);
    else if (p.SD == 2 && p.SW == 1)
        launch_pair_inst<2, 1, 0>(p, stream, a);
    else
        launch_pair_inst<1, 1, 0>(p, stream, a);
}
template <int SW, int HALO>
void launch_wgrad_inst(const Res8Plan& p, hipStream_t stream, const BwdLayerLaunch& a) {
    StageCfg zw = a.zc;
    zw.ds = nullptr;
    raise_lds_limit<wgrad_mfma_kernel<SW, HALO>>(p.lds_wgrad);
    hipLaunchKernelGGL((wgrad_mfma_kernel<SW, HALO>), dim3(launch_blocks(p.Gh, SW)), dim3(CONV_THREADS), p.lds_wgrad, stream,
                       WStage{zw, a.s_prev, false}, a.in_stats, a.bfold, a.wpart, p.Bv, p.Hs, p.Gh, geom_arg<HALO>(p));
}
void launch_wgrad(const Res8Plan& p, hipStream_t stream, const BwdLayerLaunch& a) {
    if (p.halo == 2)
        launch_wgrad_inst<1, 2>(p, stream, a);
    else if (p.halo == 1)
        launch_wgrad_inst<1, 1>(p, stream, a);
    else if (p.SW == 2)
        launch_wgrad_inst<2, 0>(p, stream, a);
    else
        launch_wgrad_inst<1, 0>(p, stream, a);
}

struct Feat {
    const float* x;
    long sb, st, sm;
};
template <int NS, bool EXACT>
void launch_conv0_fwd_inst(const Res8Plan& p, hipStream_t stream, const Feat& f, const HowlRes8Params* prm, float* s0,
                           unsigned short* mask0) {
    const int npack = (2 * 6 * PACK_ELEMS + C0M_THREADS - 1) / C0M_THREADS;
    hipLaunchKernelGGL((conv0_fwd_mfma_kernel<NS, EXACT>), dim3(p.G0 + npack), dim3(C0M_THREADS), p.lds_conv0, stream, f.x, f.sb, f.st,
                       f.sm, prm->conv0_w, s0, mask0, p.Bw, p.Tw, p.M, p.Hs, p.G0, ptrs6(prm->conv_w), p.ws.wp_fwd, p.ws.wp_bwd,
                       p.c0_nwin, p.c0_step, p.c0_last, p.S0);
}
void launch_conv0_fwd(const Res8Plan& p, hipStream_t stream, const Feat& f, const HowlRes8Params* prm, float* s0,
                      unsigned short* mask0) {
    if (p.c0_exact && p.ns == 2)
        launch_conv0_fwd_inst<2, true>(p, stream, f, prm, s0, mask0);
    else if (p.c0_exact)
        launch_conv0_fwd_inst<1, true>(p, stream, f, prm, s0, mask0);
    else if (p.ns == 2)
        launch_conv0_fwd_inst<2, false>(p, stream, f, prm, s0, mask0);
    else
        launch_conv0_fwd_inst<1, false>(p, stream, f, prm, s0, mask0);
}
template <int NS, bool EXACT>
void launch_conv0_wgrad_inst(const Res8Plan& p, hipStream_t stream, const Feat& f, const unsigned short* mask0, const float* g0) {
    hipLaunchKernelGGL((conv0_wgrad_valu_kernel<NS, EXACT>), dim3(p.G0w), dim3(C0G_THREADS), p.lds_conv0w, stream, f.x, f.sb, f.st, f.sm,
                       mask0, g0, (const float*)nullptr, p.ws.c0part, p.B, p.Tw, p.M, p.Hs, p.S0w, p.sg, p.T);
}
void launch_conv0_wgrad(const Res8Plan& p, hipStream_t stream, const Feat& f, const unsigned short* mask0, const float* g0) {
    if (p.c0_exact && p.ns == 2)
        launch_conv0_wgrad_inst<2, true>(p, stream, f, mask0, g0);
    else if (p.c0_exact)
        launch_conv0_wgrad_inst<1, true>(p, stream, f, mask0, g0);
    else if (p.ns == 2)
        launch_conv0_wgrad_inst<2, false>(p, stream, f, mask0, g0);
    else
        launch_conv0_wgrad_inst<1, false>(p, stream, f, mask0, g0);
}

int res8_fwd_impl(const HowlRes8Params* prm, const Feat& feat, int B, int T, int M, int C, int training, const HowlRes8Saved* sv,
                  float* logits, void* ws, size_t ws_bytes, const long long* labels, float* nll, float* dlogits, hipStream_t stream) {
    HOWL_REQUIRE(prm && feat.x && sv && logits && ws, "howl_res8_fwd: null pointer");
    HOWL_REQUIRE(labels == nullptr || (nll != nullptr && dlogits != nullptr && C <= HEAD_XC),
                 "howl_res8_fwd_xent: nll / dlogits missing or more than %d classes (C=%d)", HEAD_XC, C);
    HOWL_REQUIRE(mel_strips(M) > 0, "howl_res8_fwd: res8 pools (3,4) over 40 or 80 mel bins; got M=%d", M);
    HOWL_REQUIRE(B >= 1 && T / 3 >= 1, "howl_res8_fwd: B=%d T=%d unsupported (T >= 3)", B, T);
    HOWL_REQUIRE(C >= 1, "howl_res8_fwd: C must be positive");
    const Res8Plan p = res8_plan(B, T, M, ws);
    HOWL_REQUIRE(p.hv_last >= 1 && p.nr <= MAX_ROW_STRIPS, "howl_res8_fwd: T=%d frames unsupported (%d row strips)", T, p.nr);
    if (int rc = check_workspace("howl_res8_fwd", ws_bytes, training ? p.train_bytes : p.eval_bytes)) return rc;
    const Ws& w = p.ws;
    if (!training)
        hipLaunchKernelGGL(bn_eval_stats_kernel, dim3(6), dim3(64), 0, stream, ptrs6(prm->bn_running_mean), ptrs6(prm->bn_running_var),
                           sv->bn_stats);
    {
        HowlProfScope prof("conv0_fwd", stream);
        launch_conv0_fwd(p, stream, feat, prm, sv->s[0], sv->mask0);
    }
    const double count = (double)B * (double)p.Pt;
    const auto fold_of = [&](int layer, float* part) {
        return BnFold{part, p.G * p.SL, count, sv->bn_stats + (size_t)(layer - 1) * 2 * CP,
                      HowlBnBuffers{prm->bn_running_mean[layer - 1], prm->bn_running_var[layer - 1], prm->bn_num_batches[layer - 1]}};
    };
    for (int i = 1; i <= 6; ++i) {
        Conv3x3Launch a;
        a.in = plain_tile(sv->s[i - 1]);
        a.wp = w.wp_fwd + (size_t)(i - 1) * 3 * KSTEPS * 64;
        a.res = (i % 2) == 0 ? sv->s[i - 2] : nullptr;
        a.out = sv->s[i];
        a.part = training ? ((i & 1) ? w.part : w.part2) : nullptr;
        a.pool = i == 6 ? w.pool : nullptr;
        if (i > 1 && training)
            a.fold = fold_of(i - 1, (i & 1) ? w.part2 : w.part);
        else if (i > 1)
            a.in_stats = sv->bn_stats + (size_t)(i - 2) * 2 * CP;
        HowlProfScope prof("conv3x3_fwd", stream);
        launch_conv3x3<0>(p, stream, a);
    }
    const int groups = 4 * p.SL;
    hipLaunchKernelGGL(head_fwd_kernel, dim3(B < 1024 ? B : 1024), dim3(HEAD_THREADS), 0, stream, sv->s[6],
                       sv->bn_stats + (size_t)5 * 2 * CP, prm->out_w, prm->out_b, sv->pooled, logits, B, p.Pt, C, labels, nll, dlogits,
                       w.dpool, 1.0f / (float)B, (const float*)w.pool, groups, groups < (p.P + 15) / 16 ? groups : (p.P + 15) / 16,
                       training ? fold_of(6, w.part2) : BnFold{}, p.nr * p.ns);
    HOWL_CHECK_LAUNCH("howl_res8_fwd");
    return HOWL_OK;
}

int res8_bwd_impl(const HowlRes8Params* prm, const Feat& feat, int B, int T, int M, int C, const HowlRes8Saved* sv, const float* dlogits,
                  const HowlRes8Grads* gr, void* ws, size_t ws_bytes, int part, const float* nll, float* loss, hipStream_t stream,
                  const HowlAdamW* adamw = nullptr) {
    HOWL_REQUIRE(prm && feat.x && sv && dlogits && gr && ws, "howl_res8_bwd: null pointer");
    HOWL_REQUIRE(adamw == nullptr || (part == 0 && adamw->p && adamw->g && adamw->m && adamw->v && adamw->n >= 1 && adamw->step >= 1),
                 "howl_res8_bwd: HowlAdamW needs the whole pass (part 0) and complete buffers");
    HOWL_REQUIRE(part >= 0 && part <= 2, "howl_res8_bwd_part: part must be 0 (all), 1 or 2");
    const bool run_layers = part != 2, run_conv0 = part != 1;
    HOWL_REQUIRE(mel_strips(M) > 0, "howl_res8_bwd: M must be 40 or 80 (got %d)", M);
    HOWL_REQUIRE(B >= 1 && T / 3 >= 1, "howl_res8_bwd: B=%d T=%d unsupported", B, T);
    const Res8Plan p = res8_plan(B, T, M, ws);
    HOWL_REQUIRE(p.hv_last >= 1 && p.nr <= MAX_ROW_STRIPS, "howl_res8_bwd: T=%d frames unsupported (%d row strips)", T, p.nr);
    if (int rc = check_workspace("howl_res8_bwd", ws_bytes, p.train_bytes)) return rc;
    HOWL_REQUIRE(p.saved_floats / 2 < (size_t)1 << 31, "howl_res8_bwd: B=%d too large for the 32-bit element index of the elementwise pass", B);
    const Ws& w = p.ws;
    const double count = (double)B * (double)p.Pt;

    if (run_layers) {
        if (nll == nullptr)
            hipLaunchKernelGGL(head_bwd_pool_kernel, dim3((B * CP + 255) / 256), dim3(256), 0, stream, dlogits, prm->out_w, w.dpool,
                               B, C);
        hipLaunchKernelGGL(head_bwd_param_kernel, dim3(C + (nll != nullptr ? 2 : 1)), dim3(1024), 0, stream, dlogits, sv->pooled,
                           w.dpool, gr->out_w, gr->out_b, w.m12, B, C, p.Pt, nll, loss);
    }
    float* dx_cur = nullptr;
    float* dx_next = w.bufa;
    float* ds_prev = nullptr;
    float* ds_free = w.dsa;
    for (int i = 6; i >= 1; --i) {
        const bool even = (i % 2) == 0;
        const float* stats_i = sv->bn_stats + (size_t)(i - 1) * 2 * CP;
        float* ds_out = even ? ds_free : nullptr;
        float* dz = even ? w.dz : w.dz2;
        float* part_in = p.fused ? ((i & 1) ? w.part2 : w.part) : w.part;
        float* part_out = p.fused ? ((i & 1) ? w.part : w.part2) : w.part;
        BwdLayerLaunch a;
        a.bfold = BwdFold{stats_i, w.m12, i == 6 ? (const float*)nullptr : (const float*)part_in, p.Gh * p.SD, count};
        a.zc = plain_tile(dz);
        if (p.fused)
            a.zc = StageCfg{dx_cur, sv->s[i], even ? (const float*)ds_prev : (const float*)nullptr, ds_out, w.dpool,
                            1.0f / (float)p.Pt, true, even, false};
        else if (run_layers)
            hipLaunchKernelGGL(bn_relu_bwd_kernel, dim3(p.ew_grid), dim3(BRB_THREADS), 0, stream, (const float*)dx_cur, w.dpool, sv->s[i],
                               stats_i, w.m12, a.bfold.part, p.Gh * p.SD, count, even ? (const float*)ds_prev : (const float*)nullptr,
                               even ? 1 : 0, ds_out, dz, B, p.P);
        if (even) {
            float* t = ds_prev ? ds_prev : w.dsb;
            ds_prev = ds_out;
            ds_free = t;
        }
        const bool need_stats = i > 1;
        a.s_prev = sv->s[i - 1];
        a.in_stats = need_stats ? sv->bn_stats + (size_t)(i - 2) * 2 * CP : nullptr;
        a.wp = w.wp_bwd + (size_t)(i - 1) * 3 * KSTEPS * 64;
        a.dx = dx_next;
        a.xs = need_stats ? sv->s[i - 1] : (const float*)ds_prev;
        a.xs_stats = a.in_stats;
        a.spart = need_stats ? part_out : nullptr;
        a.wpart = w.wpart + (size_t)(i - 1) * p.wpart_stride;
        a.wf = (p.fold_in_pair && i < 6) ? WFold{w.wpart + (size_t)i * p.wpart_stride, p.Gh, gr->conv_w[i]} : WFold{nullptr, 0, nullptr};
        if (!run_layers) {
        } else if (p.merged) {
            HowlProfScope prof("bwd_pair", stream);
            launch_pair(p, stream, a);
        } else {
            {
                HowlProfScope prof("conv3x3_dgrad", stream);
                Conv3x3Launch d;
                d.in = a.zc, d.wp = a.wp, d.out = a.dx, d.xs = a.xs, d.xs_stats = a.xs_stats, d.part = a.spart;
                d.bfold = a.bfold, d.wf = a.wf;
                launch_conv3x3<1>(p, stream, d);
            }
            HowlProfScope prof("wgrad", stream);
            launch_wgrad(p, stream, a);
        }
        dx_cur = dx_next;
        dx_next = (dx_next == w.bufa) ? w.bufb : w.bufa;
    }
    HOWL_REQUIRE(sv->mask0 != nullptr, "howl_res8_bwd: saved->mask0 is required");
    const HowlPtrs6 gw = ptrs6(gr->conv_w);
    const RowsAdamW no_opt{nullptr, nullptr, nullptr, nullptr, HowlAdamWCoef{}, 0, 0, 0};
    const auto reduce_rows = [&](int cols, int first, int skip, int nrows, const RowsAdamW& opt) {
        hipLaunchKernelGGL(reduce_rows_all_kernel, dim3((cols + 63) / 64, nrows + (opt.on ? 1 : 0)), dim3(1024), 0, stream,
                           (const float*)w.wpart, p.wpart_stride, p.Gh, gw, (const float*)w.c0part, p.G0w, gr->conv0_w, first, skip,
                           nrows, opt);
    };
    if (part == 1)
        reduce_rows(CP * WNCOL, 0, 0, p.fold_in_pair ? 1 : 6, no_opt);
    if (run_conv0) {
        {
            HowlProfScope prof("conv0_wgrad", stream);
            launch_conv0_wgrad(p, stream, feat, sv->mask0, dx_cur);
        }
        if (part == 0) {
            RowsAdamW opt = no_opt;
            bool own_launch = adamw != nullptr;
            if (adamw != nullptr && getenv("HOWL_NO_FOLD_ADAMW") == nullptr) {
                const float* g0 = adamw->g;
                bool flat = gr->conv0_w == g0 && gr->out_b == gr->out_w + (size_t)NMAP * C &&
                            adamw->n == (size_t)NMAP * 9 + (size_t)6 * NMAP * NMAP * 9 + (size_t)NMAP * C + (size_t)C &&
                            gr->out_w == g0 + (size_t)NMAP * 9 + (size_t)6 * NMAP * NMAP * 9;
                for (int i = 0; i < 6; ++i) flat = flat && gr->conv_w[i] == g0 + (size_t)NMAP * 9 + (size_t)i * NMAP * NMAP * 9;
                if (flat) {
                    opt = RowsAdamW{adamw->p, g0, adamw->m, adamw->v,
                                    howl_adamw_coef(adamw->lr, adamw->beta1, adamw->beta2, adamw->eps, adamw->weight_decay, adamw->step,
                                                    adamw->grad_scale),
                                    (long)((p.fold_in_pair ? gr->conv_w[1] : gr->out_w) - g0), (long)adamw->n, 1};
                    own_launch = false;
                }
            }
            reduce_rows(CP * WNCOL, 0, p.fold_in_pair ? 5 : 0, p.fold_in_pair ? 2 : 7, opt);
            if (own_launch) {
                const int rc = howl_adamw_step(adamw->p, adamw->g, adamw->m, adamw->v, adamw->n, adamw->lr, adamw->beta1, adamw->beta2,
                                               adamw->eps, adamw->weight_decay, adamw->step, adamw->grad_scale, stream);
                if (rc != HOWL_OK) return rc;
            }
        } else {
            reduce_rows(NMAP * 9, 6, 0, 1, no_opt);
        }
    }
    HOWL_CHECK_LAUNCH("howl_res8_bwd");
    return HOWL_OK;
}

}

extern "C" {

size_t howl_res8_workspace_bytes(int B, int T) { return res8_plan(B, T, 40).train_bytes; }
size_t howl_res8_workspace_bytes_mels(int B, int T, int M) { return res8_plan(B, T, M).train_bytes; }
size_t howl_res8_saved_floats(int B, int T, int M) { return res8_plan(B, T, M).saved_floats; }
size_t howl_res8_eval_workspace_bytes_mels(int B, int T, int M) { return res8_plan(B, T, M).eval_bytes; }
int howl_res8_row_strips(int T) { return res8_plan(1, T, 40).nr; }

int howl_res8_fwd(const HowlRes8Params* prm, const float* feat, long sb, long st, long sm, int B, int T, int M, int C,
                  int training, const HowlRes8Saved* sv, float* logits, void* ws, size_t ws_bytes, hipStream_t stream) {
    return res8_fwd_impl(prm, Feat{feat, sb, st, sm}, B, T, M, C, training, sv, logits, ws, ws_bytes, nullptr, nullptr, nullptr, stream);
}

size_t howl_res8_long_workspace_bytes(int B, int T) { return res8_long_plan(B, T, 40).long_bytes; }
size_t howl_res8_long_workspace_bytes_mels(int B, int T, int M) { return res8_long_plan(B, T, M).long_bytes; }

int howl_res8_fwd_long(const HowlRes8Params* prm, const float* feat, long sb, long st, long sm, int B, int T, int M, int C,
                       float* logits, void* ws, size_t ws_bytes, hipStream_t stream) {
    HOWL_REQUIRE(prm && feat && logits && ws, "howl_res8_fwd_long: null pointer");
    HOWL_REQUIRE(mel_strips(M) > 0, "howl_res8_fwd_long: res8 pools (3,4) over 40 or 80 mel bins; got M=%d", M);
    const int H = T / 3;
    HOWL_REQUIRE(B >= 1 && H > WIN_H && C >= 1, "howl_res8_fwd_long: for T > 83 frames (got B=%d T=%d); shorter inputs use howl_res8_fwd", B, T);
    const int nw = long_windows(H);
    HOWL_REQUIRE(nw <= MAX_WINDOWS, "howl_res8_fwd_long: T=%d needs %d windows (max %d)", T, nw, MAX_WINDOWS);
    const Res8Plan p = res8_long_plan(B, T, M, ws);
    if (int rc = check_workspace("howl_res8_fwd_long", ws_bytes, p.long_bytes)) return rc;
    char* base = static_cast<char*>(ws);
    float* buf[3];
    for (int i = 0; i < 3; ++i) buf[i] = reinterpret_cast<float*>(base + i * p.long_map_bytes);
    float* stats = reinterpret_cast<float*>(base + 3 * p.long_map_bytes);
    HowlWinRows rows;
    for (int i = 0; i < nw; ++i) {
        const int a = i * WIN_STEP < H - WIN_H ? i * WIN_STEP : H - WIN_H;
        const int a_next = (i + 1) * WIN_STEP < H - WIN_H ? (i + 1) * WIN_STEP : H - WIN_H;
        const int g_lo = i == 0 ? 0 : a + WIN_MARGIN;
        const int g_hi = i == nw - 1 ? H : a_next + WIN_MARGIN;
        rows.lo[i] = g_lo - a;
        rows.hi[i] = g_hi - a;
    }
    hipLaunchKernelGGL(bn_eval_stats_kernel, dim3(6), dim3(64), 0, stream, ptrs6(prm->bn_running_mean), ptrs6(prm->bn_running_var), stats);
    launch_conv0_fwd(p, stream, Feat{feat, sb, st, sm}, prm, buf[0], nullptr);
    int cur = 0, skip = 0;
    for (int i = 1; i <= 6; ++i) {
        const bool even = (i % 2) == 0;
        int out = 0;
        while (out == cur || out == skip) ++out;
        Conv3x3Launch a;
        a.in = plain_tile(buf[cur]);
        a.in_stats = i == 1 ? nullptr : stats + (size_t)(i - 2) * 2 * CP;
        a.wp = p.ws.wp_fwd + (size_t)(i - 1) * 3 * KSTEPS * 64;
        a.res = even ? buf[skip] : nullptr;
        a.out = buf[out];
        launch_conv3x3<0>(p, stream, a);
        if (even) skip = out;
        cur = out;
    }
    hipLaunchKernelGGL(head_fwd_windows_kernel, dim3(B < 1024 ? B : 1024), dim3(256), 0, stream, (const float*)buf[cur],
                       (const float*)(stats + (size_t)5 * 2 * CP), prm->out_w, prm->out_b, logits, B, nw, WIN_H, rows,
                       1.0f / ((float)H * PW * p.ns), C, p.ns);
    HOWL_CHECK_LAUNCH("howl_res8_fwd_long");
    return HOWL_OK;
}

int howl_res8_bwd(const HowlRes8Params* prm, const float* feat, long sb, long st, long sm, int B, int T, int M, int C,
                  const HowlRes8Saved* sv, const float* dlogits, const HowlRes8Grads* gr, void* ws, size_t ws_bytes,
                  hipStream_t stream) {
    return res8_bwd_impl(prm, Feat{feat, sb, st, sm}, B, T, M, C, sv, dlogits, gr, ws, ws_bytes, 0, nullptr, nullptr, stream);
}

int howl_res8_bwd_part(const HowlRes8Params* prm, const float* feat, long sb, long st, long sm, int B, int T, int M, int C,
                       const HowlRes8Saved* sv, const float* dlogits, const HowlRes8Grads* gr, void* ws, size_t ws_bytes,
                       int part, hipStream_t stream) {
    return res8_bwd_impl(prm, Feat{feat, sb, st, sm}, B, T, M, C, sv, dlogits, gr, ws, ws_bytes, part, nullptr, nullptr, stream);
}

int howl_res8_fwd_xent(const HowlRes8Params* prm, const float* feat, long sb, long st, long sm, int B, int T, int M, int C,
                       const HowlRes8Saved* sv, const long long* labels, float* logits, float* nll, float* dlogits, void* ws,
                       size_t ws_bytes, hipStream_t stream) {
    HOWL_REQUIRE(labels && nll && dlogits, "howl_res8_fwd_xent: null pointer");
    return res8_fwd_impl(prm, Feat{feat, sb, st, sm}, B, T, M, C, 1, sv, logits, ws, ws_bytes, labels, nll, dlogits, stream);
}

int howl_res8_bwd_xent(const HowlRes8Params* prm, const float* feat, long sb, long st, long sm, int B, int T, int M, int C,
                       const HowlRes8Saved* sv, const float* dlogits, const float* nll, float* loss, const HowlRes8Grads* gr,
                       void* ws, size_t ws_bytes, int part, const HowlAdamW* adamw, hipStream_t stream) {
    HOWL_REQUIRE(nll && loss, "howl_res8_bwd_xent: null pointer");
    return res8_bwd_impl(prm, Feat{feat, sb, st, sm}, B, T, M, C, sv, dlogits, gr, ws, ws_bytes, part, nll, loss, stream, adamw);
}

int howl_xent_fwd_bwd(const float* logits, const long long* labels, int B, int C, float* loss, float* dlogits,
                      hipStream_t stream) {
    HOWL_REQUIRE(logits && labels && loss, "howl_xent_fwd_bwd: null pointer");
    HOWL_REQUIRE(B >= 1 && C >= 1, "howl_xent_fwd_bwd: bad shape");
    hipLaunchKernelGGL(xent_kernel, dim3(1), dim3(1024), 0, stream, logits, labels, B, C, loss, dlogits);
    HOWL_CHECK_LAUNCH("howl_xent_fwd_bwd");
    return HOWL_OK;
}

int howl_adamw_step(float* p, const float* g, float* m, float* v, size_t n, float lr, float beta1, float beta2, float eps,
                    float weight_decay, int step, float grad_scale, hipStream_t stream) {
    HOWL_REQUIRE(p && g && m && v, "howl_adamw_step: null pointer");
    HOWL_REQUIRE(step >= 1, "howl_adamw_step: step counts from 1");
    if (n == 0) return HOWL_OK;
    size_t blocks = (n + 255) / 256;
    if (blocks > 2048) blocks = 2048;
    hipLaunchKernelGGL(adamw_kernel, dim3((unsigned)blocks), dim3(256), 0, stream, p, g, m, v, n,
                       howl_adamw_coef(lr, beta1, beta2, eps, weight_decay, step, grad_scale));
    HOWL_CHECK_LAUNCH("howl_adamw_step");
    return HOWL_OK;
}

}
```

### howl_amd/lib.py

```python
import ctypes
import os
from ctypes import POINTER, c_char_p, c_double, c_float, c_int, c_long, c_size_t, c_void_p
from pathlib import Path

LIB_PATH = Path(os.environ.get("HOWL_HIP_LIBRARY") or Path(__file__).resolve().parent / "libhowl_hip.so")
MAX_MELS = 96
FB_COLS = 48
FB_PACKED_FLOATS = 260 * FB_COLS + 17 * 64 * 4 + 17 * (FB_COLS // 4) * 64 + 32


def fb_packed_floats(n_mels: int) -> int:
    return FB_PACKED_FLOATS * (1 if n_mels <= FB_COLS else 2)


P = c_void_p
STREAM = c_void_p


class HowlMelPoints(ctypes.Structure):
    _fields_ = [("f", c_float * (MAX_MELS + 2))]


class HowlRes8Params(ctypes.Structure):
    _fields_ = [("conv0_w", P), ("conv_w", P * 6), ("bn_running_mean", P * 6), ("bn_running_var", P * 6),
                ("bn_num_batches", P * 6), ("out_w", P), ("out_b", P)]


class HowlRes8Grads(ctypes.Structure):
    _fields_ = [("conv0_w", P), ("conv_w", P * 6), ("out_w", P), ("out_b", P)]


class HowlRes8Saved(ctypes.Structure):
    _fields_ = [("s", P * 7), ("bn_stats", P), ("pooled", P), ("mask0", P)]


class HowlLstmParams(ctypes.Structure):
    _fields_ = [("w_ih", P), ("w_hh", P), ("b_ih", P), ("b_hh", P)]


class HowlLstmGrads(ctypes.Structure):
    _fields_ = [("w_ih", P), ("w_hh", P), ("b_ih", P), ("b_hh", P)]


class HowlHeadParams(ctypes.Structure):
    _fields_ = [("w1", P), ("b1", P), ("w2", P), ("b2", P)]


class HowlHeadGrads(ctypes.Structure):
    _fields_ = [("w1", P), ("b1", P), ("w2", P), ("b2", P)]


class HowlCtcMean(ctypes.Structure):
    _fields_ = [("nll", P), ("target_lengths", P), ("B", c_int), ("loss", P)]


class HowlLogmelArgs(ctypes.Structure):
    _fields_ = [("pcm", P), ("B", c_int), ("L", c_int), ("ld", c_long), ("fbp", P), ("M", c_int), ("log_eps", c_float), ("zmuv", P),
                ("out", P), ("layout", c_int)]


class HowlAdamW(ctypes.Structure):
    _fields_ = [("p", P), ("g", P), ("m", P), ("v", P), ("n", c_size_t), ("lr", c_float), ("beta1", c_float), ("beta2", c_float),
                ("eps", c_float), ("weight_decay", c_float), ("step", c_int), ("grad_scale", c_float)]


class HowlLstmSaved(ctypes.Structure):
    _fields_ = [("gx", P), ("gates", P), ("c", P), ("hseq", P), ("dgates", P), ("t_out", c_int), ("x_frames", c_int)]


class HowlMbLayer(ctypes.Structure):
    _fields_ = [(n, c_int) for n in ("kind", "cin", "cout", "stride", "pad_h", "pad_w", "act", "bias", "pool", "res_src",
                                     "feat", "sub", "wrapped")] + \
               [(n, ctypes.c_longlong) for n in ("w_off", "b_off", "gamma_off", "beta_off", "rmean_off", "rvar_off")]


class HowlMbWsLayer(ctypes.Structure):
    _fields_ = [(n, ctypes.c_longlong) for n in ("z", "g", "y", "ss", "bc", "b_ss", "f_yout", "pooled", "pooled_d", "dz1",
                                                 "total_floats")] + \
               [(n, c_int) for n in ("hin", "win", "ho", "wo", "hy", "wy", "f_tile", "f_cx", "f_ry", "d_tile", "d_ry", "d_chunks",
                                     "nslab", "group_rows")]


class HowlDecideConfig(ctypes.Structure):
    _fields_ = [("mode", c_int), ("C", c_int), ("blank", c_int), ("negative", c_int), ("threshold", c_double), ("smoothing_ms", c_double),
                ("window_ms", c_double), ("tolerance_ms", c_double), ("seq_len", c_int), ("sequence", c_int * 16), ("weights", P),
                ("color", P)]


SIGNATURES = {
    "howl_version": [POINTER(c_int), POINTER(c_int)],
    "howl_profile_enable": [c_int],
    "howl_profile_read": [c_char_p, POINTER(c_double), POINTER(c_int), c_int],
    "howl_profile_read_work": [c_char_p, POINTER(c_double), POINTER(c_int), POINTER(c_double), c_int],
    "howl_shutdown": [],
    "howl_fb_pack": [P, c_int, P, STREAM],
    "howl_fb_from_points": [POINTER(HowlMelPoints), c_int, c_float, P, STREAM],
    "howl_logmel_fwd": [P, c_int, c_int, c_long, P, c_int, c_float, P, P, c_int, STREAM],
    "howl_deltas_fwd": [P, c_int, c_int, c_int, P, P, STREAM],
    "howl_zmuv_update": [P, c_size_t, P, P, P, P, STREAM],
    "howl_zmuv_update_masked": [P, P, c_size_t, c_double, P, P, P, P, STREAM],
    "howl_zmuv_pair": [P, P, P, STREAM],
    "howl_zmuv_apply": [P, c_size_t, P, P, STREAM],
    "howl_collate_augment": [P, c_long, P, P, P, P, P, P, ctypes.c_ulonglong, c_int, c_int, P, STREAM],
    "howl_collate_augment_mix": [P, c_long, P, P, P, P, P, P, ctypes.c_ulonglong, P, c_long, P, P, P, c_int, c_int, P, STREAM],
    "howl_collate_augment_window": [P, c_long, P, P, P, P, P, P, ctypes.c_ulonglong, P, c_long, P, P, P, P, c_int, c_int, P,
                                    STREAM],
    "howl_gather_windows": [P, c_long, P, P, P, P, c_int, c_int, P, STREAM],
    "howl_specaug_mask": [P, c_int, c_int, c_int, c_int, c_long, c_long, c_long, c_long, P, P, P, P, STREAM],
    "howl_res8_fwd": [POINTER(HowlRes8Params), P, c_long, c_long, c_long, c_int, c_int, c_int, c_int, c_int,
                      POINTER(HowlRes8Saved), P, P, c_size_t, STREAM],
    "howl_res8_fwd_long": [POINTER(HowlRes8Params), P, c_long, c_long, c_long, c_int, c_int, c_int, c_int, P, P, c_size_t, STREAM],
    "howl_res8_bwd": [POINTER(HowlRes8Params), P, c_long, c_long, c_long, c_int, c_int, c_int, c_int,
                      POINTER(HowlRes8Saved), P, POINTER(HowlRes8Grads), P, c_size_t, STREAM],
    "howl_res8_bwd_part": [POINTER(HowlRes8Params), P, c_long, c_long, c_long, c_int, c_int, c_int, c_int,
                           POINTER(HowlRes8Saved), P, POINTER(HowlRes8Grads), P, c_size_t, c_int, STREAM],
    "howl_res8_fwd_xent": [POINTER(HowlRes8Params), P, c_long, c_long, c_long, c_int, c_int, c_int, c_int,
                           POINTER(HowlRes8Saved), P, P, P, P, P, c_size_t, STREAM],
    "howl_res8_bwd_xent": [POINTER(HowlRes8Params), P, c_long, c_long, c_long, c_int, c_int, c_int, c_int,
                           POINTER(HowlRes8Saved), P, P, P, POINTER(HowlRes8Grads), P, c_size_t, c_int, POINTER(HowlAdamW), STREAM],
    "howl_dropout_mask": [P, c_size_t, c_float, ctypes.c_ulonglong, STREAM],
    "howl_xent_fwd_bwd": [P, P, c_int, c_int, P, P, STREAM],
    "howl_ctc_loss": [P, c_long, c_long, c_int, c_int, c_int, P, c_long, c_int, P, P, c_int, P, P, P, c_long, c_long, P, c_size_t,
                      STREAM],
    "howl_lstm_fwd": [POINTER(HowlLstmParams), P, c_int, c_int, c_int, P, P, P, POINTER(HowlLstmSaved), P, P, P, c_size_t,
                      STREAM],
    "howl_lstm_fwd_next": [POINTER(HowlLstmParams), P, c_int, c_int, c_int, P, P, P, POINTER(HowlLstmSaved), P, P, P, c_size_t,
                           POINTER(HowlLogmelArgs), STREAM],
    "howl_lstm_bwd": [POINTER(HowlLstmParams), P, c_int, c_int, c_int, P, P, POINTER(HowlLstmSaved), P, P, P,
                      POINTER(HowlLstmGrads), P, c_size_t, STREAM],
    "howl_head_fwd": [POINTER(HowlHeadParams), P, c_int, c_long, c_long, c_int, c_int, c_int, c_int, P, P, STREAM],
    "howl_head_bwd": [POINTER(HowlHeadParams), P, c_int, c_long, c_long, c_int, c_int, c_int, c_int, P, P, P, P,
                      POINTER(HowlHeadGrads), POINTER(HowlCtcMean), P, c_size_t, STREAM],
    "howl_seq_head_ctc": [POINTER(HowlHeadParams), P, c_long, c_long, c_int, c_int, c_int, c_int, c_int, P, c_long, c_int, P, P, c_int, P, P,
                          P, P, P, c_size_t, STREAM],
    "howl_seq_head_ctc_supported": [c_int, c_int, c_int, c_int, c_int, c_int],
    "howl_seq_lstm_bwd": [POINTER(HowlHeadParams), c_int, c_int, P, P, P, P, POINTER(HowlHeadGrads), POINTER(HowlCtcMean), P,
                          c_size_t, POINTER(HowlLstmParams), P, c_int, c_int, c_int, P, P, POINTER(HowlLstmSaved),
                          POINTER(HowlLstmGrads), P, c_size_t, POINTER(HowlAdamW), STREAM],
    "howl_adamw_step": [P, P, P, P, c_size_t, c_float, c_float, c_float, c_float, c_float, c_int, c_float, STREAM],
    "howl_mobilenet_layer": [c_int, POINTER(HowlMbLayer)],
    "howl_mobilenet_workspace_layer": [c_int, c_int, c_int, c_int, c_int, POINTER(HowlMbWsLayer)],
    "howl_mobilenet_fwd": [P, P, c_int, P, c_long, c_long, c_long, c_int, c_int, c_int, c_int, P, c_float, P, P, c_size_t,
                           STREAM],
    "howl_mobilenet_bwd": [P, c_int, P, c_long, c_long, c_long, c_int, c_int, c_int, P, c_float, P, P, P, c_size_t, STREAM],
}
SIZE_FUNCS = {"howl_fb_packed_floats": [c_int], "howl_res8_workspace_bytes": [c_int, c_int], "howl_res8_long_workspace_bytes": [c_int, c_int],
              "howl_res8_workspace_bytes_mels": [c_int, c_int, c_int], "howl_res8_saved_floats": [c_int, c_int, c_int],
              "howl_res8_eval_workspace_bytes_mels": [c_int, c_int, c_int], "howl_res8_row_strips": [c_int], "howl_res8_long_workspace_bytes_mels": [c_int, c_int, c_int], "howl_lstm_workspace_bytes": [c_int, c_int],
              "howl_lstm_needs_gx": [POINTER(HowlLstmParams), c_int, c_int, c_int, c_int],
              "howl_head_workspace_bytes": [c_int, c_int, c_int],
              "howl_mobilenet_num_layers": [],
              "howl_mobilenet_param_floats": [c_int], "howl_mobilenet_buffer_floats": [],
              "howl_mobilenet_workspace_bytes": [c_int, c_int, c_int, c_int],
              "howl_ctc_supported": [c_int, c_int, c_int], "howl_ctc_workspace_floats": [c_int, c_int]}


STREAM_SIGNATURES = {
    "howl_res8_stream_prepare": [POINTER(HowlRes8Params), c_int, P, c_size_t, STREAM],
    "howl_res8_stream_windows": [P, P, c_long, c_int, c_int, P, c_int, c_float, P, c_int, P, P, STREAM],
}
STREAM_SIZE_FUNCS = {"howl_res8_stream_supported": [c_int, c_int, c_int], "howl_res8_stream_state_bytes": [c_int]}

LSTM_STREAM_SIGNATURES = {
    "howl_lstm_stream_chunks": [POINTER(HowlLstmParams), POINTER(HowlHeadParams), P, c_long, c_int, c_int, P, P, P, c_int, c_float, P,
                                P, P, c_int, c_int, P, P, c_long, STREAM],
}
LSTM_STREAM_SIZE_FUNCS = {"howl_lstm_stream_supported": [c_int, c_int, c_int]}

DECIDE_SIGNATURES = {
    "howl_decide_clips": [POINTER(HowlDecideConfig), P, c_long, c_long, c_int, c_int, P, P, P, P, P, P, P, P, P, c_long, P, STREAM],
}
DECIDE_SIZE_FUNCS = {"howl_decide_supported": [POINTER(HowlDecideConfig), c_int]}


class HowlHipError(RuntimeError):
    pass


class Library:
    def __init__(self, path):
        path = Path(path)
        if not path.exists():
            raise HowlHipError(
                f"{path} not found: the HIP extension is not built. Run `python __graft_entry__.py` "
                "(build()) first; howl_amd has no CPU fallback.")
        self.path = path
        self.cdll = ctypes.CDLL(str(path))
        self.cdll.howl_last_error.restype = c_char_p
        self.cdll.howl_last_error.argtypes = []
        for name, argtypes in {**SIGNATURES, **STREAM_SIGNATURES, **LSTM_STREAM_SIGNATURES, **DECIDE_SIGNATURES}.items():
            fn = getattr(self.cdll, name)
            fn.restype = c_int
            fn.argtypes = argtypes
        for name, argtypes in {**SIZE_FUNCS, **STREAM_SIZE_FUNCS, **LSTM_STREAM_SIZE_FUNCS, **DECIDE_SIZE_FUNCS}.items():
            fn = getattr(self.cdll, name)
            fn.restype = c_size_t
            fn.argtypes = argtypes

    def call(self, name, *args):
        rc = getattr(self.cdll, name)(*args)
        if rc != 0:
            raise HowlHipError(f"{name} failed ({rc}): {self.cdll.howl_last_error().decode()}")


_LIB = None


def get() -> Library:
    global _LIB
    if _LIB is None:
        _LIB = Library(LIB_PATH)
        import atexit
        atexit.register(_LIB.cdll.howl_shutdown)
    return _LIB
```

### howl_amd/model/cnn.py

```python
import ctypes
import logging
from typing import Tuple

import torch
import torch.nn as nn

from howl_amd import lib as _lib
from howl_amd import ops, parallel
from howl_amd.settings import _EnvSettings

from .base import RegisteredModel

__all__ = ["Res8", "Res8Settings", "Res8StreamSession", "MobileNetClassifier"]


class Res8Settings(_EnvSettings):
    num_labels: int = 2
    pooling: Tuple[int, int] = (3, 4)
    num_maps: int = 45


def _vp(t):
    return t.data_ptr()

# ... 126 lines not shown
            logging.getLogger(__name__).warning(msg)
        self.conv0 = nn.Conv2d(1, n_maps, (3, 3), padding=(1, 1), bias=False)
        self.pool = nn.AvgPool2d(config.pooling)
        self.n_layers = n_layers = 6
        self.convs = [nn.Conv2d(n_maps, n_maps, (3, 3), padding=1, bias=False) for _ in range(n_layers)]
        for i, conv in enumerate(self.convs):
            self.add_module(f"bn{i + 1}", nn.BatchNorm2d(n_maps, affine=False))
            self.add_module(f"conv{i + 1}", conv)
        self.output = nn.Linear(n_maps, num_labels)
        self._buffers_cache = {}
        self._eval_cache = {}
        self._fwd_version = 0

    def hot_parameters(self):
        return [self.conv0.weight] + [getattr(self, f"conv{i}").weight for i in range(1, 7)] + \
               [self.output.weight, self.output.bias]

    def _params_struct(self):
        prm = _lib.HowlRes8Params()
        ps = self.hot_parameters()
        for p in ps:
            if not (ops.on_device(p) and p.is_contiguous() and p.dtype == torch.float32):
                raise _lib.HowlHipError("Res8 parameters must be contiguous fp32 tensors on a HIP device "
                                        "(call .to('cuda') first; there is no CPU fallback)")
        prm.conv0_w = _vp(ps[0])
        for i in range(6):
            bn = getattr(self, f"bn{i + 1}")
            prm.conv_w[i] = _vp(ps[1 + i])
            prm.bn_running_mean[i] = _vp(bn.running_mean)
            prm.bn_running_var[i] = _vp(bn.running_var)
            prm.bn_num_batches[i] = _vp(bn.num_batches_tracked)
        prm.out_w = _vp(ps[7])
        prm.out_b = _vp(ps[8])
        return prm

    def _get_buffers(self, B, T, device, M=40):
        key = (B, T, M, self.num_labels, str(device))
        buf = self._buffers_cache.pop(key, None)
        if buf is None:
            if len(self._buffers_cache) >= 6:
                self._buffers_cache.pop(next(iter(self._buffers_cache)))
            buf = _Res8Buffers(B, T, self.num_labels, device, M)
        self._buffers_cache[key] = buf
        return buf

    EVAL_CACHE_BYTES = 256 << 20

    def _get_eval_buffers(self, B, T, device, M=40):
        key = (B, T, M, self.num_labels, str(device))
        buf = self._eval_cache.pop(key, None)
        if buf is None:
            buf = _Res8EvalBuffers(B, T, self.num_labels, device, M)
        size = lambda b: b.ws.numel() + 4 * 3 * b.rot[0].numel() + 2 * b.mask0.numel()
        if size(buf) <= self.EVAL_CACHE_BYTES // 4:
            self._eval_cache[key] = buf
            while sum(size(b) for b in self._eval_cache.values()) > self.EVAL_CACHE_BYTES:
                self._eval_cache.pop(next(iter(self._eval_cache)))
        return buf

    @staticmethod
    def _feat_view(x):
        x0 = x[:, 0]
        if not ops.on_device(x0) or x0.dtype != torch.float32:
            raise _lib.HowlHipError("Res8 input must be an fp32 tensor on a HIP device (no CPU fallback)")
        if x0.shape[1] not in RES8_MELS:
            raise ValueError(f"Res8 on MI355X is built for NUM_MELS=40 (envs/res8.env) or 80 (stock default); got "
                             f"{x0.shape[1]} mel bins -- set NUM_MELS before howl_amd.settings is imported")
        if x0.shape[2] < 3:
            raise ValueError(f"Res8 needs at least 3 frames (one pooled row); got T={x0.shape[2]}")
        return x0, x0.stride(0), x0.stride(2), x0.stride(1)

    MAX_FRAMES = 83

    def _launch_forward_long(self, x0, sb, st, sm):
        B, M, T = x0.shape
        nbytes = _lib.get().cdll.howl_res8_long_workspace_bytes_mels(B, T, M)
        ws = torch.empty(nbytes, dtype=torch.uint8, device=x0.device)
        logits = torch.empty((B, self.num_labels), dtype=torch.float32, device=x0.device)
        prm = self._params_struct()
        _lib.get().call("howl_res8_fwd_long", ctypes.byref(prm), ctypes.c_void_p(x0.data_ptr()), sb, st, sm, B, T, M,
                        self.num_labels, ctypes.c_void_p(logits.data_ptr()), ctypes.c_void_p(ws.data_ptr()), ws.numel(),
                        ops._stream())
        return logits

    def _launch_forward(self, feat, grads_struct=None):
        x0, sb, st, sm = self._feat_view(feat)
        B, M, T = x0.shape
        if not self.training:
            buf = self._get_eval_buffers(B, T, x0.device, M)
        else:
            buf = self._get_buffers(B, T, x0.device, M)
        logits = torch.empty((B, self.num_labels), dtype=torch.float32, device=x0.device)
        prm = self._params_struct()
        self._fwd_version += 1
        _lib.get().call("howl_res8_fwd", ctypes.byref(prm), ctypes.c_void_p(x0.data_ptr()), sb, st, sm, B, T, M,
                        self.num_labels, int(self.training), ctypes.byref(buf.saved), ctypes.c_void_p(logits.data_ptr()),
                        ctypes.c_void_p(buf.ws.data_ptr()), buf.ws.numel(), ops._stream())
        return logits

    XENT_MAX_LABELS = 64

    def _launch_forward_xent(self, feat, labels):
        x0, sb, st, sm = self._feat_view(feat)
        B, M, T = x0.shape
        if not self.training or self.num_labels > self.XENT_MAX_LABELS:
            raise NotImplementedError("fused forward + cross-entropy: training mode, <= 64 labels")
        buf = self._get_buffers(B, T, x0.device, M)
        f32 = dict(dtype=torch.float32, device=x0.device)
        logits = torch.empty((B, self.num_labels), **f32)
        nll, dlogits = torch.empty((B,), **f32), torch.empty((B, self.num_labels), **f32)
        labels = labels.to(device=x0.device, dtype=torch.int64).contiguous()
        prm = self._params_struct()
        self._fwd_version += 1
        _lib.get().call("howl_res8_fwd_xent", ctypes.byref(prm), ctypes.c_void_p(x0.data_ptr()), sb, st, sm, B, T, M,
                        self.num_labels, ctypes.byref(buf.saved), _vp(labels), _vp(logits), _vp(nll), _vp(dlogits),
                        ctypes.c_void_p(buf.ws.data_ptr()), buf.ws.numel(), ops._stream())
        return logits, nll, dlogits

    LATE_GRAD_PARAMS = 1

    def _launch_backward(self, feat, dlogits, out_grads=None, part=0, xent=None, adamw=None):
        self.optimizer_step_done = False
        if not self.training:
            raise NotImplementedError("Res8 backward is implemented for training-mode BatchNorm (batch statistics), "
                                      "the only mode the reference trains in")
        x0, sb, st, sm = self._feat_view(feat)
        B, M, T = x0.shape
        buf = self._get_buffers(B, T, x0.device, M)
        ps = self.hot_parameters()
        grads = out_grads if out_grads is not None else [torch.empty_like(p) for p in ps]
        gr = _lib.HowlRes8Grads()
        gr.conv0_w = _vp(grads[0])
        for i in range(6):
            gr.conv_w[i] = _vp(grads[1 + i])
        gr.out_w = _vp(grads[7])
        gr.out_b = _vp(grads[8])
        prm = self._params_struct()
        if xent is not None:
            nll, loss = xent
            opt = None
            if adamw is not None and part == 0:
                flat, fgrad, m, v, lr, betas, eps, wd, step, gscale = adamw
                opt = ctypes.byref(_lib.HowlAdamW(_vp(flat), _vp(fgrad), _vp(m), _vp(v), flat.numel(), lr, betas[0], betas[1], eps, wd,
                                                  step, gscale))
            _lib.get().call("howl_res8_bwd_xent", ctypes.byref(prm), ctypes.c_void_p(x0.data_ptr()), sb, st, sm, B, T, M,
                            self.num_labels, ctypes.byref(buf.saved), ctypes.c_void_p(dlogits.data_ptr()), _vp(nll), _vp(loss),
                            ctypes.byref(gr), ctypes.c_void_p(buf.ws.data_ptr()), buf.ws.numel(), int(part), opt, ops._stream())
            self.optimizer_step_done = opt is not None
            return grads
        _lib.get().call("howl_res8_bwd_part", ctypes.byref(prm), ctypes.c_void_p(x0.data_ptr()), sb, st, sm, B, T, M,
                        self.num_labels, ctypes.byref(buf.saved), ctypes.c_void_p(dlogits.data_ptr()), ctypes.byref(gr),
                        ctypes.c_void_p(buf.ws.data_ptr()), buf.ws.numel(), int(part), ops._stream())
        return grads

    def forward(self, x, lengths=None):
        if torch.is_grad_enabled() and any(p.requires_grad for p in self.hot_parameters()):
            return _Res8Function.apply(self, x, *self.hot_parameters())
        return self._launch_forward(x)

    def stream_session(self, std, zmuv) -> Res8StreamSession:
        return Res8StreamSession(self, std, zmuv)


class _InvertedResidualParams(nn.Module):

    def __init__(self, inp, oup, stride, t):
        super().__init__()
        hidden = inp * t
        layers = []
        if t != 1:
            layers.append(nn.Sequential(nn.Conv2d(inp, hidden, 1, bias=False), nn.BatchNorm2d(hidden), nn.ReLU6()))
        layers.append(nn.Sequential(nn.Conv2d(hidden, hidden, 3, stride, 1, groups=hidden, bias=False), nn.BatchNorm2d(hidden),
                                    nn.ReLU6()))
        layers += [nn.Conv2d(hidden, oup, 1, bias=False), nn.BatchNorm2d(oup)]
        self.conv = nn.Sequential(*layers)


class _MobileNetV2Params(nn.Module):
    SETTING = [[1, 16, 1, 1], [6, 24, 2, 2], [6, 32, 3, 2], [6, 64, 4, 2], [6, 96, 3, 1], [6, 160, 3, 2], [6, 320, 1, 1]]

    def __init__(self, num_classes):
        super().__init__()
        feats = [nn.Sequential(nn.Conv2d(3, 32, 3, 2, 1, bias=False), nn.BatchNorm2d(32), nn.ReLU6())]
        inp = 32
        for t, c, n, s in self.SETTING:
            for i in range(n):
                feats.append(_InvertedResidualParams(inp, c, s if i == 0 else 1, t))
                inp = c
        feats.append(nn.Sequential(nn.Conv2d(inp, 1280, 1, bias=False), nn.BatchNorm2d(1280), nn.ReLU6()))
        self.features = nn.Sequential(*feats)
        self.classifier = nn.Sequential(nn.Dropout(0.2), nn.Linear(1280, num_classes))
        for m in self.modules():
            if isinstance(m, nn.Conv2d):
                nn.init.kaiming_normal_(m.weight, mode="fan_out")
            elif isinstance(m, nn.BatchNorm2d):
                nn.init.ones_(m.weight)
                nn.init.zeros_(m.bias)
            elif isinstance(m, nn.Linear):
                nn.init.normal_(m.weight, 0, 0.01)
                nn.init.zeros_(m.bias)


class _MobileNetFunction(torch.autograd.Function):
    @staticmethod
    def forward(ctx, module, feat, *params):
        logits = module._launch_forward(feat)
        ctx.module, ctx.feat, ctx.version = module, feat, module._fwd_version
        return logits

    @staticmethod
    def backward(ctx, dlogits):
        module = ctx.module
        if ctx.version != module._fwd_version:
            raise RuntimeError("MobileNetClassifier: backward called after a newer forward overwrote the saved activations")
        grads = module._launch_backward(ctx.feat, dlogits.contiguous())
        return (None, None) + tuple(grads)


class MobileNetClassifier(RegisteredModel, name="mobilenet"):

    def __init__(self, num_labels: int):
        super().__init__(num_labels)
        self.downsample = nn.Sequential(nn.Conv2d(1, 3, 3, padding=(1, 3)), nn.BatchNorm2d(3), nn.ReLU(),
                                        nn.MaxPool2d((1, 2)))
        self.model = _MobileNetV2Params(num_labels)
        self.dropout_p = 0.2
        self.forced_keep_mask = None
        self._table = None
        self._flat = self._bflat = None
        self._ws_cache = {}
        self._fwd_version = 0
        self._last_mask = None

    def _layer_modules(self):
        if self._table is None:
            lb = _lib.get()
            table = []
            for i in range(lb.cdll.howl_mobilenet_num_layers()):
                d = _lib.HowlMbLayer()
                lb.call("howl_mobilenet_layer", i, ctypes.byref(d))
                if d.feat < 0:
                    conv, bn = self.downsample[0], self.downsample[1]
                elif d.sub < 0:
                    conv, bn = self.model.features[d.feat][0], self.model.features[d.feat][1]
                elif d.wrapped:
                    conv, bn = self.model.features[d.feat].conv[d.sub][0], self.model.features[d.feat].conv[d.sub][1]
                else:
                    conv, bn = self.model.features[d.feat].conv[d.sub], self.model.features[d.feat].conv[d.sub + 1]
                table.append((conv, bn, d))
            self._table = table
        return self._table

    def hot_parameters(self):
        ps = []
        for conv, bn, d in self._layer_modules():
            ps.append(conv.weight)
            if d.bias:
                ps.append(conv.bias)
            ps += [bn.weight, bn.bias]
        lin = self.model.classifier[1]
        return ps + [lin.weight, lin.bias]

    def _stat_buffers(self):
        out = []
        for _, bn, _ in self._layer_modules():
            out += [bn.running_mean, bn.running_var]
        return out

    @staticmethod
    def _is_flat(tensors, flat):
        if flat is None or not ops.on_device(tensors[0]) or tensors[0].device != flat.device:
            return False
        off = 0
        for t in tensors:
            if t.data_ptr() != flat.data_ptr() + 4 * off or not t.is_contiguous():
                return False
            off += t.numel()
        return off == flat.numel()

    def _ensure_flat(self):
        ps = self.hot_parameters()
        for p in ps:
            if not (ops.on_device(p) and p.dtype == torch.float32):
                raise _lib.HowlHipError("MobileNetClassifier parameters must be fp32 tensors on a HIP device "
                                        "(call .to('cuda') first; there is no CPU fallback)")
        if not self._is_flat(ps, self._flat):
            base = ps[0]
            n = sum(p.numel() for p in ps)
            probe = None
            if base.is_contiguous() and base.untyped_storage().nbytes() >= 4 * (base.storage_offset() + n):
                probe = torch.as_strided(base.detach(), (n,), (1,), base.storage_offset())
            if probe is not None and self._is_flat(ps, probe):
                self._flat = probe
            else:
                flat = torch.empty(n, dtype=torch.float32, device=base.device)
                off = 0
                with torch.no_grad():
                    for p in ps:
                        flat[off:off + p.numel()].copy_(p.data.reshape(-1))
                        p.data = flat[off:off + p.numel()].view(p.shape)
                        off += p.numel()
                self._flat = flat
        bs = self._stat_buffers()
        if not self._is_flat(bs, self._bflat):
            n = sum(b.numel() for b in bs)
            bflat = torch.empty(n, dtype=torch.float32, device=bs[0].device)
# ... 93 lines not shown
```

### include/howl_hip.h

```cpp
#ifndef HOWL_HIP_H
#define HOWL_HIP_H

#include <stddef.h>
#include <stdint.h>

#ifdef __cplusplus
extern "C" {
#endif

typedef struct ihipStream_t* hipStream_t;

#define HOWL_FB_COLS 48
#define HOWL_MAX_MELS 96
#define HOWL_FB_PACKED_FLOATS (260 * HOWL_FB_COLS + 17 * 64 * 4 + 17 * (HOWL_FB_COLS / 4) * 64 + 32)

int howl_version(int* major, int* minor);
const char* howl_last_error(void);

int howl_profile_enable(int on);
int howl_profile_read(const char* tag, double* total_ms, int* count, int reset);
int howl_profile_read_work(const char* tag, double* total_ms, int* count, double* work, int reset);

int howl_shutdown(void);


size_t howl_fb_packed_floats(int M);
int howl_fb_pack(const float* fb, int M, float* fbp, hipStream_t stream);

typedef struct {
    float f[HOWL_MAX_MELS + 2];
} HowlMelPoints;
int howl_fb_from_points(const HowlMelPoints* pts , int M, float nyquist, float* fbp, hipStream_t stream);

int howl_logmel_fwd(const float* pcm, int B, int L, long ld, const float* fbp, int M, float log_eps,
                    const float* zmuv, float* out, int layout, hipStream_t stream);

int howl_deltas_fwd(const float* logmel, int B, int M, int T, const float* zmuv, float* out3, hipStream_t stream);

int howl_zmuv_update(const float* x, size_t n, float* total, float* mean, float* mean2, double* scratch2,
                     hipStream_t stream);
int howl_zmuv_update_masked(const float* x, const float* mask, size_t n, double count_scale, float* total, float* mean,
                            float* mean2, double* scratch3, hipStream_t stream);
int howl_zmuv_pair(const float* mean, const float* mean2, float* pair, hipStream_t stream);

int howl_zmuv_apply(const float* x, size_t n, const float* pair, float* out, hipStream_t stream);

int howl_collate_augment(const float* bank, long bank_ld, const int* idx, const int* src_len, const int* shift,
                         const int* from_head, const float* sigma, const float* sp_prob, unsigned long long seed, int B,
                         int Lout, float* out, hipStream_t stream);
int howl_collate_augment_mix(const float* bank, long bank_ld, const int* idx, const int* src_len, const int* shift,
                             const int* from_head, const float* sigma, const float* sp_prob, unsigned long long seed,
                             const float* bg, long bg_ld, const int* bg_idx, const int* bg_off, const float* alpha, int B,
                             int Lout, float* out, hipStream_t stream);

int howl_collate_augment_window(const float* bank, long bank_ld, const int* idx, const int* src_len, const int* shift,
                                const int* from_head, const float* sigma, const float* sp_prob, unsigned long long seed,
                                const float* bg, long bg_ld, const int* bg_idx, const int* bg_off, const float* alpha,
                                const int* dst_off, int B, int Lout, float* out, hipStream_t stream);

int howl_gather_windows(const float* bank, long bank_ld, const int* idx, const int* start, const int* len,
                        const int* dst_off, int B, int Lout, float* out, hipStream_t stream);

int howl_specaug_mask(float* x, int B, int C, int M, int T, long sb, long sc, long sm, long st, const int* f0,
                      const int* f, const int* t0, const int* t, hipStream_t stream);

typedef struct {
    const float* conv0_w;
    const float* conv_w[6];
    float* bn_running_mean[6];
    float* bn_running_var[6];
    long long* bn_num_batches[6];
    const float* out_w;
    const float* out_b;
} HowlRes8Params;

typedef struct {
    float* conv0_w;
    float* conv_w[6];
    float* out_w;
    float* out_b;
} HowlRes8Grads;

typedef struct {
    float* s[7];
    float* bn_stats;
    float* pooled;
    unsigned short* mask0;
} HowlRes8Saved;

size_t howl_res8_workspace_bytes(int B, int T);
size_t howl_res8_workspace_bytes_mels(int B, int T, int M);
size_t howl_res8_saved_floats(int B, int T, int M);
size_t howl_res8_eval_workspace_bytes_mels(int B, int T, int M);
int howl_res8_row_strips(int T);

int howl_res8_fwd(const HowlRes8Params* prm, const float* feat, long sb, long st, long sm, int B, int T, int M, int C,
                  int training, const HowlRes8Saved* saved, float* logits, void* ws, size_t ws_bytes,
                  hipStream_t stream);

size_t howl_res8_long_workspace_bytes(int B, int T);
size_t howl_res8_long_workspace_bytes_mels(int B, int T, int M);
int howl_res8_fwd_long(const HowlRes8Params* prm, const float* feat, long sb, long st, long sm, int B, int T, int M, int C,
                       float* logits, void* ws, size_t ws_bytes, hipStream_t stream);

int howl_res8_bwd(const HowlRes8Params* prm, const float* feat, long sb, long st, long sm, int B, int T, int M, int C,
                  const HowlRes8Saved* saved, const float* dlogits, const HowlRes8Grads* grads, void* ws,
                  size_t ws_bytes, hipStream_t stream);
int howl_res8_bwd_part(const HowlRes8Params* prm, const float* feat, long sb, long st, long sm, int B, int T, int M, int C,
                       const HowlRes8Saved* saved, const float* dlogits, const HowlRes8Grads* grads, void* ws,
                       size_t ws_bytes, int part, hipStream_t stream);

typedef struct {
    float* p;
    float* g;
    float* m;
    float* v;
    size_t n;
    float lr, beta1, beta2, eps, weight_decay;
    int step;
    float grad_scale;
} HowlAdamW;

int howl_res8_fwd_xent(const HowlRes8Params* prm, const float* feat, long sb, long st, long sm, int B, int T, int M, int C,
                       const HowlRes8Saved* saved, const long long* labels, float* logits, float* nll, float* dlogits,
                       void* ws, size_t ws_bytes, hipStream_t stream);
int howl_res8_bwd_xent(const HowlRes8Params* prm, const float* feat, long sb, long st, long sm, int B, int T, int M, int C,
                       const HowlRes8Saved* saved, const float* dlogits, const float* nll, float* loss,
                       const HowlRes8Grads* grads, void* ws, size_t ws_bytes, int part,
                       const HowlAdamW* adamw , hipStream_t stream);

int howl_xent_fwd_bwd(const float* logits, const long long* labels, int B, int C, float* loss, float* dlogits,
                      hipStream_t stream);

int howl_ctc_supported(int T, int C, int max_target_length);
size_t howl_ctc_workspace_floats(int T, int B);
int howl_ctc_loss(const float* logits, long st_t, long st_b, int T, int B, int C, const long long* targets, long tgt_stride,
                  int max_target_length, const long long* input_lengths, const long long* target_lengths, int blank,
                  float* nll, float* loss, float* dlogits, long dst_t, long dst_b, float* workspace, size_t workspace_floats,
                  hipStream_t stream);

int howl_adamw_step(float* p, const float* g, float* m, float* v, size_t n, float lr, float beta1, float beta2,
                    float eps, float weight_decay, int step, float grad_scale, hipStream_t stream);

typedef struct {
    const float* w_ih;
    const float* w_hh;
    const float* b_ih;
    const float* b_hh;
} HowlLstmParams;

typedef struct {
    float* w_ih;
    float* w_hh;
    float* b_ih;
    float* b_hh;
} HowlLstmGrads;

typedef struct {
    float* gx;
    float* gates;
    float* c;
    float* hseq;
    float* dgates;
    int t_out;
    int x_frames;
} HowlLstmSaved;

size_t howl_lstm_workspace_bytes(int B, int T);
size_t howl_lstm_needs_gx(const HowlLstmParams* p, int B, int T, int M, int x_frames);
int howl_lstm_fwd(const HowlLstmParams* p, const float* x, int B, int T, int M, const long long* lengths,
                  const float* h0, const float* c0, const HowlLstmSaved* saved, float* hT, float* cT, void* ws,
                  size_t ws_bytes, hipStream_t stream);
typedef struct {
    const float* pcm;
    int B, L;
    long ld;
    const float* fbp;
    int M;
    float log_eps;
    const float* zmuv;
    float* out;
    int layout;
} HowlLogmelArgs;
int howl_lstm_fwd_next(const HowlLstmParams* p, const float* x, int B, int T, int M, const long long* lengths,
                       const float* h0, const float* c0, const HowlLstmSaved* saved, float* hT, float* cT, void* ws,
                       size_t ws_bytes, const HowlLogmelArgs* next, hipStream_t stream);
int howl_lstm_bwd(const HowlLstmParams* p, const float* x, int B, int T, int M, const long long* lengths,
                  const float* c0, const HowlLstmSaved* saved, const float* dy, const float* dhT, const float* dcT,
                  const HowlLstmGrads* grads, void* ws, size_t ws_bytes, hipStream_t stream);

typedef struct {
    const float* w1;
    const float* b1;
    const float* w2;
    const float* b2;
} HowlHeadParams;
typedef struct {
    float* w1;
    float* b1;
    float* w2;
    float* b2;
} HowlHeadGrads;
typedef struct {
    const float* nll;
    const long long* target_lengths;
    int B;
    float* loss;
} HowlCtcMean;
size_t howl_head_workspace_bytes(int n_in, int n_hid, int n_out);
int howl_head_fwd(const HowlHeadParams* p, const float* x, int rows_inner, long s_outer, long s_inner, int rows, int n_in,
                  int n_hid, int n_out, float* y1, float* y2, hipStream_t stream);
int howl_head_bwd(const HowlHeadParams* p, const float* x, int rows_inner, long s_outer, long s_inner, int rows, int n_in,
                  int n_hid, int n_out, const float* y1, const float* dy2, float* dz1, float* dx, const HowlHeadGrads* grads,
                  const HowlCtcMean* ctc_mean , void* ws, size_t ws_bytes, hipStream_t stream);
int howl_seq_head_ctc_supported(int B, int T, int n_in, int n_hid, int n_out, int max_target_length);
int howl_seq_head_ctc(const HowlHeadParams* p, const float* x, long s_outer, long s_inner, int B, int T, int n_in, int n_hid, int n_out,
                      const long long* targets, long tgt_stride, int max_target_length, const long long* input_lengths,
                      const long long* target_lengths, int blank, float* y2, float* nll, float* dz1, float* dhs, void* head_ws,
                      size_t head_ws_bytes, hipStream_t stream);
int howl_seq_lstm_bwd(const HowlHeadParams* head, int n_hid, int n_out, const float* y1, const float* dy2, float* dz1, float* dhs,
                      const HowlHeadGrads* head_grads, const HowlCtcMean* ctc_mean , void* head_ws,
                      size_t head_ws_bytes, const HowlLstmParams* p, const float* x, int B, int T, int M,
                      const long long* lengths, const float* c0, const HowlLstmSaved* saved, const HowlLstmGrads* grads, void* ws,
                      size_t ws_bytes, const HowlAdamW* adamw , hipStream_t stream);

typedef struct {
    int kind;
    int cin, cout, stride, pad_h, pad_w;
    int act;
    int bias;
    int pool;
    int res_src;
    int feat, sub, wrapped;
    long long w_off, b_off, gamma_off, beta_off;
    long long rmean_off, rvar_off;
} HowlMbLayer;
size_t howl_mobilenet_num_layers(void);
int howl_mobilenet_layer(int i, HowlMbLayer* out);
size_t howl_mobilenet_param_floats(int num_labels);
size_t howl_mobilenet_buffer_floats(void);
size_t howl_mobilenet_workspace_bytes(int B, int M, int T, int num_labels);
typedef struct {
    long long z, g, y, ss, bc, b_ss, f_yout;
    long long pooled, pooled_d, dz1, total_floats;
    int hin, win, ho, wo, hy, wy;
    int f_tile, f_cx, f_ry, d_tile, d_ry, d_chunks, nslab, group_rows;
} HowlMbWsLayer;
// ... 15 lines not shown
```

Measured before the change: 463,800 utterances/sec.

## Replace per-iteration block barriers with LDS counter waits in conv and wgrad loops

Replaces the __syncthreads calls inside the double-buffered conv and weight-gradient main loops with per-wave LDS atomic counters. Each wave signals when it has finished writing or reading a tile buffer, and waits only for the specific producer or consumer it depends on. This lets waves drift relative to one another instead of stalling at full-workgroup barriers. In exchange it adds atomic and polling overhead, a timeout fallback that writes NaN and a status word on failure, a few extra LDS words, and a workspace status slot; it can be disabled through an environment variable.

New measurement: 466,600 utterances/sec, median of 6. Within noise of the previous version (+0.6%).

```diff
diff --git a/howl_amd/csrc/howl_common.hip.h b/howl_amd/csrc/howl_common.hip.h
--- a/howl_amd/csrc/howl_common.hip.h
+++ b/howl_amd/csrc/howl_common.hip.h
@@ -96,6 +96,44 @@
     __builtin_amdgcn_fence(__ATOMIC_ACQUIRE, "wavefront");
 }
 
+typedef __attribute__((address_space(3))) unsigned lds_u32;
+constexpr long long HOWL_WAIT_TICKS = 4ll << 20;
+__device__ __forceinline__ void lds_arrive(lds_u32* counter, int lane) {
+#if !defined(HIPEMU)
+    asm volatile("" ::: "memory");
+    if (lane == 0) __hip_atomic_fetch_add(counter, 1u, __ATOMIC_RELAXED, __HIP_MEMORY_SCOPE_WORKGROUP);
+    asm volatile("" ::: "memory");
+#endif
+}
+__device__ __forceinline__ unsigned lds_poll(lds_u32* counter, int lane) {
+#if !defined(HIPEMU)
+    unsigned v = 0u;
+    if (lane == 0) v = __hip_atomic_load(counter, __ATOMIC_RELAXED, __HIP_MEMORY_SCOPE_WORKGROUP);
+    return (unsigned)__builtin_amdgcn_readfirstlane((int)v);
+#else
+    return 0u;
+#endif
+}
+__device__ __forceinline__ bool lds_wait(lds_u32* counter, unsigned target, int lane) {
+    bool ok = true;
+#if !defined(HIPEMU)
+    asm volatile("" ::: "memory");
+    if ((int)(lds_poll(counter, lane) - target) < 0) {
+        const long long t0 = (long long)__builtin_amdgcn_s_memtime();
+        for (;;) {
+            __builtin_amdgcn_s_sleep(1);
+            if ((int)(lds_poll(counter, lane) - target) >= 0) break;
+            if ((long long)__builtin_amdgcn_s_memtime() - t0 > HOWL_WAIT_TICKS) {
+                ok = false;
+                break;
+            }
+        }
+    }
+    asm volatile("s_waitcnt lgkmcnt(0)" ::: "memory");
+#endif
+    return ok;
+}
+
 __device__ __forceinline__ float wave_sum(float v) {
     for (int m = 32; m >= 1; m >>= 1) v += __shfl_xor(v, m);
     return v;
diff --git a/howl_amd/csrc/res8.hip b/howl_amd/csrc/res8.hip
--- a/howl_amd/csrc/res8.hip
+++ b/howl_amd/csrc/res8.hip
@@ -194,7 +194,29 @@
     bool fused;
     bool even;
     bool affine;
-};
+    bool waits;
+    int* wstat;
+};
+
+#if defined(HIPEMU)
+#define HOWL_WAITS_ON(cfg_) false
+#else
+#define HOWL_WAITS_ON(cfg_) ((cfg_).waits)
+#endif
+constexpr int LW_WRITTEN = 0, LW_READ = 2;
+struct LoopWaits {
+    lds_u32* cnt;
+    int* wstat;
+    int lane, role;
+    bool gave_up;
+};
+__device__ __forceinline__ void loop_wait(LoopWaits& w, int idx, unsigned target) {
+    if (!lds_wait(w.cnt + idx, target, w.lane)) {
+        w.gave_up = true;
+        if (w.lane == 0 && w.wstat != nullptr) *w.wstat = 16 * w.role + 1 + idx;
+    }
+}
+__device__ __forceinline__ void loop_arrive(const LoopWaits& w, int idx) { lds_arrive(w.cnt + idx, w.lane); }
 
 struct SlotVal {
     float2 a, s, k;
@@ -517,6 +539,7 @@
     const float* lm;
     int B, CS, t0, lane, tid;
     int nblk;
+    lds_u32* cnt;
 };
 
 
@@ -537,7 +560,10 @@
         dl[s3] = (tap / 3) * WP + tap % 3 - (lane >> 4) * c.CS;
     }
     const int gcol = (b & 1) ? PW - 1 : 0, lcol = (b & 1) ? 0 : WP - 1;
-    for (; b < c.B; b += c.nblk) {
+    const bool waits = HOWL_WAITS_ON(cfg);
+    LoopWaits lw{c.cnt, cfg.wstat, lane, MODE, false};
+    unsigned done = 0;
+    for (; b < c.B; b += c.nblk, done += CONV_THREADS / 64) {
         const size_t ubase = (size_t)b * NMAP * P;
         const int bn = b + c.nblk;
         const bool more = bn < c.B;
@@ -554,6 +580,7 @@
         f32x4 acc[NTV];
         KCursor<NTV> k;
         if constexpr (NTW > 0) k_begin<NTW, TS>(k, acc, c.ltile, c.wnt, c.CS, P, c.t0, lane);
+        if (waits) loop_wait(lw, LW_WRITTEN + 0, done);
         if constexpr (NTW > 0) k_prime<NTW>(k);
         constexpr bool STAGE = true;
         const int a0 = 2, a1 = 2, a2 = KG_A - 4, b0 = 2, b1 = 2, b2 = KG_B - 4;
@@ -569,6 +596,7 @@
         HOWL_WINO_CHUNK();
         if constexpr (NTW > 0) k_run<NTW>(k, acc, c.CS, a0);
         HOWL_WINO_BAR();
+        if (waits) loop_wait(lw, LW_READ + 1, done);
         if constexpr (STAGE) {
             slot_write<MODE>(v[0], cfg, ubase + r1, tid, pk1[0], c.tile, c.lm, HALO == 2 && zb && ((gx.pad[1] >> 0) & 1));
             slot_write<MODE>(v[1], cfg, ubase + r1, tid + CONV_THREADS, pk1[1], c.tile, c.lm, HALO == 2 && zb && ((gx.pad[1] >> 1) & 1));
@@ -585,12 +613,18 @@
             slot_write<MODE>(v[0], cfg, ubase + r1, tid + 2 * CONV_THREADS, pk1[2], c.tile, c.lm, HALO == 2 && zb && ((gx.pad[1] >> 2) & 1));
             slot_write<MODE>(v[1], cfg, ubase + r1, tid + 3 * CONV_THREADS, pk1[3], c.tile, c.lm, HALO == 2 && zb && ((gx.pad[1] >> 3) & 1));
         }
+        if (waits) loop_arrive(lw, LW_WRITTEN + 1);
         HOWL_STAIR(1);
         HOWL_WINO_CHUNK();
         if constexpr (NTW > 0) k_run<NTW>(k, acc, c.CS, a2);
         HOWL_WINO_BAR();
         HOWL_STAIR(0);
-        __syncthreads();
+        if (waits) {
+            loop_arrive(lw, LW_READ + 0);
+            loop_wait(lw, LW_WRITTEN + 1, done + CONV_THREADS / 64);
+        } else {
+            __syncthreads();
+        }
         if constexpr (NTW > 0) k_prime<NTW>(k);
         if (STAGE && more) {
             slot_load<MODE, HALO>(v[0], cfg, nbase, tid, pk0[0], bnsl);
@@ -602,6 +636,7 @@
         HOWL_WINO_CHUNK();
         if constexpr (NTW > 0) k_run<NTW>(k, acc, c.CS, b0);
         HOWL_WINO_BAR();
+        if (waits && more) loop_wait(lw, LW_READ + 0, done + CONV_THREADS / 64);
         if (STAGE && more) {
             slot_write<MODE>(v[0], cfg, nbase, tid, pk0[0], c.tile, c.lm, HALO == 2 && zn && ((gx.pad[0] >> 0) & 1));
             slot_write<MODE>(v[1], cfg, nbase, tid + CONV_THREADS, pk0[1], c.tile, c.lm, HALO == 2 && zn && ((gx.pad[0] >> 1) & 1));
@@ -620,6 +655,7 @@
             slot_write<MODE>(v[1], cfg, nbase, tid + 4 * CONV_THREADS, pk0[4], c.tile, c.lm, HALO == 2 && zn && ((gx.pad[0] >> 4) & 1));
             if constexpr (HALO == 1) halo_write<MODE>(v[2], cfg, hs[0], lcol, c.tile, c.lm);
         }
+        if (waits) loop_arrive(lw, LW_WRITTEN + 0);
         float2 ev[NTV][2];
         if constexpr (NTW > 0) {
             if (eop != nullptr) {
@@ -635,8 +671,13 @@
             k_tail<NTW>(k, acc, dl);
             HOWL_STAIR(0);
         }
+        if (waits) loop_arrive(lw, LW_READ + 1);
         if constexpr (NTW > 0) conv_epilogue<MODE, NTW, TS, HALO>(acc, ev, epi, ubase, c.t0, lane, st0, st1, b, pv);
+        if (!waits) __syncthreads();
+    }
+    if (waits) {
         __syncthreads();
+        if (lw.gave_up) st0 = st1 = __builtin_nanf("");
     }
 }
 
@@ -700,6 +741,7 @@
     float* tile = lds + 3 * KSTEPS * 64;
     float* lm = tile + TF;
     float* red = lm + 4 * CP;
+    lds_u32* cnt = (lds_u32*)(red + 12 * 2 * 16);
 
     const int tid = threadIdx.x;
     const int lane = tid & 63;
@@ -805,6 +847,7 @@
     float st0 = 0.0f, st1 = 0.0f;
     const ConvEpilogue epi{res, out, xs, xshift, xrstd, cout, P, cvalid, MODE == 1 && xs != nullptr && xs_stats == nullptr,
                            pool, 4 * slices, t0};
+    if (tid < 4) cnt[tid] = 0u;
     __syncthreads();
     if (b < B) {
 #pragma unroll
@@ -816,7 +859,7 @@
     }
     __syncthreads();
 
-    const ConvLoop cl{(const lds_f32*)tile, (const lds_f32*)wl + nt * KSTEPS * 64, tile, lm, B, CS, t0, lane, tid, nblk};
+    const ConvLoop cl{(const lds_f32*)tile, (const lds_f32*)wl + nt * KSTEPS * 64, tile, lm, B, CS, t0, lane, tid, nblk, cnt};
     switch (ntw) {
         case 5: conv_loop<MODE, 5, ts, HALO>(cl, epi, cfg, pk0, pk1, b, st0, st1, hs, gx); break;
         case 4: conv_loop<MODE, 4, ts, HALO>(cl, epi, cfg, pk0, pk1, b, st0, st1, hs, gx); break;
@@ -1149,6 +1192,7 @@
     int bid, nblk;
     int gw;
     int qe, mte;
+    lds_u32* cnt;
 };
 
 __device__ __forceinline__ int wgrad_boff(int q, int n, int g, int CSX) {
@@ -1178,7 +1222,10 @@
     const int aoff = n * a.CSZ + g * WPZ;
     const int R1 = a.R1, R2 = a.R - a.R1;
     const int gcol = (b & 1) ? PW - 1 : 0, lcol = (b & 1) ? 0 : PW + 1;
-    for (; b < a.B; b += a.nblk) {
+    const bool waits = HOWL_WAITS_ON(a.st.z);
+    LoopWaits lw{a.cnt, a.st.z.wstat, lane, 2, false};
+    unsigned done = 0;
+    for (; b < a.B; b += a.nblk, done += CONV_THREADS / 64) {
         const size_t ubase = (size_t)b * NMAP * a.P;
         const int bn = b + a.nblk;
         const bool more = bn < a.B;
@@ -1200,6 +1247,7 @@
             bsl = pb.bu, bnsl = pn.bu, hvb = pb.hv, hvn = pn.hv;
             zb_ = pb.hv < Hs, zn_ = pn.hv < Hs;
         }
+        if (waits) loop_wait(lw, LW_WRITTEN + 0, done);
 #pragma unroll
         for (int mt = 0; mt < 3; ++mt) az[mt] = c.ap[mt][0];
 #pragma unroll
@@ -1226,6 +1274,7 @@
         if constexpr (HALO == 2) xr = wrow_load(a.st.x, gx, b, a.P / PW, a.P, true);
         HOWL_STAIR(3);
         if (R1 > 0) wgrad_k_run<NB, EX>(c, acc, acce, az, bx, aze, bxe, 1);
+        if (waits) loop_wait(lw, LW_READ + 1, done);
         HOWL_W_WRITE(0, 0, zb, xb, cb, zb_, gx.pzb, gx.pxb);
         HOWL_W_WRITE(1, 1, zb, xb, cb, zb_, gx.pzb, gx.pxb);
         if constexpr (HALO != 0) whalo_write(xh, a.st.xaffine, wh[1], lcol, a.tx, a.lm, hvb);
@@ -1240,8 +1289,14 @@
         HOWL_STAIR(1);
         if (R1 > 2) wgrad_k_run<NB, EX>(c, acc, acce, az, bx, aze, bxe, R1 - 2);
         HOWL_STAIR(0);
+        if (waits) loop_arrive(lw, LW_READ + 0);
         HOWL_W_WRITE(0, 4, zb, xb, cb, zb_, gx.pzb, gx.pxb);
-        __syncthreads();
+        if (waits) {
+            loop_arrive(lw, LW_WRITTEN + 1);
+            loop_wait(lw, LW_WRITTEN + 1, done + CONV_THREADS / 64);
+        } else {
+            __syncthreads();
+        }
 #pragma unroll
         for (int i = 0; i < NB; ++i) c.bp[i] += 2 * WPW;
         c.bpe += 2 * WPW;
@@ -1261,6 +1316,7 @@
         }
         HOWL_STAIR(3);
         wgrad_k_run<NB, EX>(c, acc, acce, az, bx, aze, bxe, 1);
+        if (waits && more) loop_wait(lw, LW_READ + 0, done + CONV_THREADS / 64);
         if (more) {
             HOWL_W_WRITE(0, 0, zt, xt, ct, zn_, gx.pzt, gx.pxt);
             HOWL_W_WRITE(1, 1, zt, xt, ct, zn_, gx.pzt, gx.pxt);
@@ -1275,12 +1331,22 @@
             HOWL_W_WRITE(0, 2, zt, xt, ct, zn_, gx.pzt, gx.pxt);
             HOWL_W_WRITE(1, 3, zt, xt, ct, zn_, gx.pzt, gx.pxt);
         }
+        if (waits) loop_arrive(lw, LW_WRITTEN + 0);
         HOWL_STAIR(1);
         if (R2 > 2) wgrad_k_run<NB, EX>(c, acc, acce, az, bx, aze, bxe, R2 - 2);
         HOWL_STAIR(0);
 #undef HOWL_W_LOAD
 #undef HOWL_W_WRITE
-        __syncthreads();
+        if (waits)
+            loop_arrive(lw, LW_READ + 1);
+        else
+            __syncthreads();
+    }
+    if (waits && lw.gave_up) {
+#pragma unroll
+        for (int i = 0; i < NB; ++i)
+#pragma unroll
+            for (int mt = 0; mt < 3; ++mt) acc[i][mt][0] = __builtin_nanf("");
     }
     float* dst = a.part + (size_t)a.bid * CP * WNCOL;
 #pragma unroll
@@ -1308,6 +1374,7 @@
     float* tz = lds;
     float* tx = lds + tile_floats_z(H);
     float* lm = tx + tile_floats_x(H);
+    lds_u32* cnt = (lds_u32*)(lm + 6 * CP);
 
     const int tid = threadIdx.x;
     const int lane = tid & 63;
@@ -1363,6 +1430,7 @@
         lm[4 * CP + tid] = st.xaffine ? -in_stats[tid] * in_stats[CP + tid] : 0.0f;
         lm[5 * CP + tid] = st.xaffine ? in_stats[CP + tid] : 1.0f;
     }
+    if (tid < 4) cnt[tid] = 0u;
     __syncthreads();
     if (b < B) {
 #pragma unroll
@@ -1389,7 +1457,7 @@
             case 3: qe = 25, mte = 2; break;
             default: ex = false; break;
         }
-        const WgradArgs a{st, part, tz, tx, lm, B, P, CSZ, CSX, R, R1, tid, lane, wave, bid, nblk, gw, qe, mte};
+        const WgradArgs a{st, part, tz, tx, lm, B, P, CSZ, CSX, R, R1, tid, lane, wave, bid, nblk, gw, qe, mte, cnt};
         if (ex)
             wgrad_loop<2, true, GWS, HALO>(a, zt, xt, ct, zb, xb, cb, b, wh, gx);
         else
@@ -1397,7 +1465,7 @@
     } else {
         static_assert(SLICES == 2, "the weight gradient is sliced two ways");
         const bool ex = wave < 3;
-        const WgradArgs a{st, part, tz, tx, lm, B, P, CSZ, CSX, R, R1, tid, lane, wave, bid, nblk, gw, 24 + slice, ex ? wave : 0};
+        const WgradArgs a{st, part, tz, tx, lm, B, P, CSZ, CSX, R, R1, tid, lane, wave, bid, nblk, gw, 24 + slice, ex ? wave : 0, cnt};
         if (ex)
             wgrad_loop<1, true, GWS, HALO>(a, zt, xt, ct, zb, xb, cb, b, wh, gx);
         else
@@ -1629,8 +1697,10 @@
                                                                     float* __restrict__ s0, unsigned short* __restrict__ mask0,
                                                                     int B, int T, int M, int H, int nconv, HowlPtrs6 cw,
                                                                     float* __restrict__ wp_fwd, float* __restrict__ wp_bwd,
-                                                                    int nwin, int win_step, int win_last, int slices) {
+                                                                    int nwin, int win_step, int win_last, int slices,
+                                                                    int* __restrict__ wstat) {
     if ((int)blockIdx.x >= nconv) {
+        if ((int)blockIdx.x == nconv && threadIdx.x == 0) *wstat = 0;
         const int e = ((int)blockIdx.x - nconv) * C0M_THREADS + (int)threadIdx.x;
         if (e < 2 * 6 * PACK_ELEMS) pack_weights_one(cw, wp_fwd, wp_bwd, (e / PACK_ELEMS) % 6, e / (6 * PACK_ELEMS), e % PACK_ELEMS);
         return;
@@ -2109,9 +2179,9 @@
 
 size_t conv0_tile_floats(int T, int M) { return (size_t)(T + 2) * (M + 4) + 3 * (M + 4) + 16; }
 size_t conv_lds_bytes(int H, bool own_rows) {
-    return (size_t)(3 * KSTEPS * 64 + tile_floats(H, own_rows) + 4 * CP + 12 * 2 * 16) * sizeof(float);
-}
-size_t wgrad_lds_bytes(int H) { return (size_t)(tile_floats_z(H) + tile_floats_x(H) + 6 * CP) * sizeof(float); }
+    return (size_t)(3 * KSTEPS * 64 + tile_floats(H, own_rows) + 4 * CP + 12 * 2 * 16 + 4 ) * sizeof(float);
+}
+size_t wgrad_lds_bytes(int H) { return (size_t)(tile_floats_z(H) + tile_floats_x(H) + 6 * CP + 4 ) * sizeof(float); }
 
 struct Ws {
     float* wp_fwd;
@@ -2122,6 +2192,7 @@
     float* m12;
     float* dpool;
     float* pool;
+    int* wstat;
     float* bufa;
     float* bufb;
     float* dz;
@@ -2149,6 +2220,7 @@
     w->m12 = take(2 * CP);
     w->dpool = take((size_t)B * CP);
     w->pool = take((size_t)B * 16 * CP);
+    w->wstat = reinterpret_cast<int*>(take(1));
     *fwd_eval_bytes = off;
     w->bufa = take(act);
     w->bufb = take(act);
@@ -2197,7 +2269,7 @@
     int B, T, M, ns, nr, Hs, hv_last, Bv, halo;
     StripGeom sg;
     int P, Pt;
-    bool slicing, merged, fused;
+    bool slicing, merged, fused, waits;
     int G, SL;
     size_t lds_conv;
     int Bw, Tw, S0, G0, c0_nwin, c0_step, c0_last;
@@ -2221,6 +2293,7 @@
     p.slicing = !env_off("HOWL_RES8_SLICES");
     p.merged = !env_off("HOWL_RES8_BWD_PAIR");
     p.fused = p.halo != 0 || !env_off("HOWL_RES8_BWD_FUSED");
+    p.waits = !env_off("HOWL_RES8_WAITS");
 
     p.G = even_grid(p.Bv < cus ? p.Bv : cus, p.ns);
     p.SL = p.halo == 0 && p.slicing ? conv_slices(p.G, H, cus) : 1;
@@ -2298,7 +2371,12 @@
     for (int i = 0; i < 6; ++i) r.p[i] = const_cast<float*>(a[i]);
     return r;
 }
-StageCfg plain_tile(const float* t) { return StageCfg{t, nullptr, nullptr, nullptr, nullptr, 0.0f, false, false, false}; }
+StageCfg plain_tile(const float* t) { return StageCfg{t, nullptr, nullptr, nullptr, nullptr, 0.0f, false, false, false, false, nullptr}; }
+StageCfg with_waits(StageCfg c, const Res8Plan& p) {
+    c.waits = p.waits;
+    c.wstat = p.ws.wstat;
+    return c;
+}
 
 template <auto Kernel>
 void raise_lds_limit(size_t lds) {
@@ -2327,7 +2405,7 @@
     const int nblk = MODE == 0 ? p.G : p.Gh;
     raise_lds_limit<conv3x3_mfma_kernel<MODE, SLICES, HALO>>(p.lds_conv);
     hipLaunchKernelGGL((conv3x3_mfma_kernel<MODE, SLICES, HALO>), dim3(launch_blocks(nblk, SLICES)), dim3(CONV_THREADS), p.lds_conv,
-                       stream, a.in, a.in_stats, a.wp, a.res, a.out, a.xs, a.xs_stats, a.part, a.pool, p.Bv, p.Hs, nblk, a.fold,
+                       stream, with_waits(a.in, p), a.in_stats, a.wp, a.res, a.out, a.xs, a.xs_stats, a.part, a.pool, p.Bv, p.Hs, nblk, a.fold,
                        a.bfold, a.wf, geom_arg<HALO>(p));
 }
 template <int MODE>
@@ -2361,7 +2439,8 @@
 template <int SD, int SW, int HALO>
 void launch_pair_inst(const Res8Plan& p, hipStream_t stream, const BwdLayerLaunch& a) {
     raise_lds_limit<bwd_pair_kernel<SD, SW, HALO>>(p.lds_pair);
-    hipLaunchKernelGGL((bwd_pair_kernel<SD, SW, HALO>), dim3(launch_blocks(p.Gh, SD + SW)), dim3(CONV_THREADS), p.lds_pair, stream, a.zc,
+    hipLaunchKernelGGL((bwd_pair_kernel<SD, SW, HALO>), dim3(launch_blocks(p.Gh, SD + SW)), dim3(CONV_THREADS), p.lds_pair, stream,
+                       with_waits(a.zc, p),
                        a.bfold, a.wp, a.dx, a.xs, a.xs_stats, a.spart, a.s_prev, a.in_stats, a.wpart, p.Bv, p.Hs, p.Gh, a.wf,
                        geom_arg<HALO>(p));
 }
@@ -2381,7 +2460,7 @@
 }
 template <int SW, int HALO>
 void launch_wgrad_inst(const Res8Plan& p, hipStream_t stream, const BwdLayerLaunch& a) {
-    StageCfg zw = a.zc;
+    StageCfg zw = with_waits(a.zc, p);
     zw.ds = nullptr;
     raise_lds_limit<wgrad_mfma_kernel<SW, HALO>>(p.lds_wgrad);
     hipLaunchKernelGGL((wgrad_mfma_kernel<SW, HALO>), dim3(launch_blocks(p.Gh, SW)), dim3(CONV_THREADS), p.lds_wgrad, stream,
@@ -2408,7 +2487,7 @@
     const int npack = (2 * 6 * PACK_ELEMS + C0M_THREADS - 1) / C0M_THREADS;
     hipLaunchKernelGGL((conv0_fwd_mfma_kernel<NS, EXACT>), dim3(p.G0 + npack), dim3(C0M_THREADS), p.lds_conv0, stream, f.x, f.sb, f.st,
                        f.sm, prm->conv0_w, s0, mask0, p.Bw, p.Tw, p.M, p.Hs, p.G0, ptrs6(prm->conv_w), p.ws.wp_fwd, p.ws.wp_bwd,
-                       p.c0_nwin, p.c0_step, p.c0_last, p.S0);
+                       p.c0_nwin, p.c0_step, p.c0_last, p.S0, p.ws.wstat);
 }
 void launch_conv0_fwd(const Res8Plan& p, hipStream_t stream, const Feat& f, const HowlRes8Params* prm, float* s0,
                       unsigned short* mask0) {
@@ -2525,7 +2604,7 @@
         a.zc = plain_tile(dz);
         if (p.fused)
             a.zc = StageCfg{dx_cur, sv->s[i], even ? (const float*)ds_prev : (const float*)nullptr, ds_out, w.dpool,
-                            1.0f / (float)p.Pt, true, even, false};
+                            1.0f / (float)p.Pt, true, even, false, false, nullptr};
         else if (run_layers)
             hipLaunchKernelGGL(bn_relu_bwd_kernel, dim3(p.ew_grid), dim3(BRB_THREADS), 0, stream, (const float*)dx_cur, w.dpool, sv->s[i],
                                stats_i, w.m12, a.bfold.part, p.Gh * p.SD, count, even ? (const float*)ds_prev : (const float*)nullptr,
@@ -2616,6 +2695,10 @@
 size_t howl_res8_workspace_bytes(int B, int T) { return res8_plan(B, T, 40).train_bytes; }
 size_t howl_res8_workspace_bytes_mels(int B, int T, int M) { return res8_plan(B, T, M).train_bytes; }
 size_t howl_res8_saved_floats(int B, int T, int M) { return res8_plan(B, T, M).saved_floats; }
+size_t howl_res8_wait_status_offset(int B, int T, int M) {
+    char base[1];
+    return (size_t)(reinterpret_cast<char*>(res8_plan(B, T, M, base).ws.wstat) - base);
+}
 size_t howl_res8_eval_workspace_bytes_mels(int B, int T, int M) { return res8_plan(B, T, M).eval_bytes; }
 int howl_res8_row_strips(int T) { return res8_plan(1, T, 40).nr; }
 
diff --git a/howl_amd/lib.py b/howl_amd/lib.py
--- a/howl_amd/lib.py
+++ b/howl_amd/lib.py
@@ -146,7 +146,7 @@
 }
 SIZE_FUNCS = {"howl_fb_packed_floats": [c_int], "howl_res8_workspace_bytes": [c_int, c_int], "howl_res8_long_workspace_bytes": [c_int, c_int],
               "howl_res8_workspace_bytes_mels": [c_int, c_int, c_int], "howl_res8_saved_floats": [c_int, c_int, c_int],
-              "howl_res8_eval_workspace_bytes_mels": [c_int, c_int, c_int], "howl_res8_row_strips": [c_int], "howl_res8_long_workspace_bytes_mels": [c_int, c_int, c_int], "howl_lstm_workspace_bytes": [c_int, c_int],
+              "howl_res8_eval_workspace_bytes_mels": [c_int, c_int, c_int], "howl_res8_row_strips": [c_int], "howl_res8_wait_status_offset": [c_int, c_int, c_int], "howl_res8_long_workspace_bytes_mels": [c_int, c_int, c_int], "howl_lstm_workspace_bytes": [c_int, c_int],
               "howl_lstm_needs_gx": [POINTER(HowlLstmParams), c_int, c_int, c_int, c_int],
               "howl_head_workspace_bytes": [c_int, c_int, c_int],
               "howl_mobilenet_num_layers": [],
diff --git a/howl_amd/model/cnn.py b/howl_amd/model/cnn.py
--- a/howl_amd/model/cnn.py
+++ b/howl_amd/model/cnn.py
@@ -302,6 +302,13 @@
                         self.num_labels, ctypes.byref(buf.saved), ctypes.c_void_p(dlogits.data_ptr()), ctypes.byref(gr),
                         ctypes.c_void_p(buf.ws.data_ptr()), buf.ws.numel(), int(part), ops._stream())
         return grads
+
+    def wait_status(self):
+        if not self._buffers_cache:
+            return 0
+        (B, T, M, _, _), buf = next(reversed(self._buffers_cache.items()))
+        off = _lib.get().cdll.howl_res8_wait_status_offset(B, T, M)
+        return int(buf.ws[off:off + 4].view(torch.int32).item())
 
     def forward(self, x, lengths=None):
         if torch.is_grad_enabled() and any(p.requires_grad for p in self.hot_parameters()):
diff --git a/include/howl_hip.h b/include/howl_hip.h
--- a/include/howl_hip.h
+++ b/include/howl_hip.h
@@ -93,6 +93,7 @@
 size_t howl_res8_saved_floats(int B, int T, int M);
 size_t howl_res8_eval_workspace_bytes_mels(int B, int T, int M);
 int howl_res8_row_strips(int T);
+size_t howl_res8_wait_status_offset(int B, int T, int M);
 
 int howl_res8_fwd(const HowlRes8Params* prm, const float* feat, long sb, long st, long sm, int B, int T, int M, int C,
                   int training, const HowlRes8Saved* saved, float* logits, void* ws, size_t ws_bytes,
```
